# liupei101/VLSA

Measured on AMD Instinct MI355X. Metric: patches/sec per slide (50k x 512 CONCH bag), higher is better.
Workload: dtype bf16

## Files before the change

include/vlsa_hip.h:

```cpp
#ifndef VLSA_HIP_H
#define VLSA_HIP_H

#include <stddef.h>
#include <stdint.h>

#ifdef __cplusplus
extern "C" {
#endif

#define VLSA_ABI_VERSION 1
#define VLSA_MAX_P 16
#define VLSA_MAX_K 64
#define VLSA_MAX_D 1024

#define VLSA_DT_F32 0
#define VLSA_DT_BF16 1

#define VLSA_OK 0
#define VLSA_EINVAL (-1)
#define VLSA_EUNSUPPORTED (-2)
#define VLSA_ELAUNCH (-3)

#define VLSA_KERNEL_AUTO 0
#define VLSA_KERNEL_GENERIC 1
#define VLSA_KERNEL_MFMA 2
#define VLSA_KERNEL_DMA 3

#define VLSA_POOL_MEAN 0
#define VLSA_POOL_MAX 1
#define VLSA_POOL_WEIGHT 2
#define VLSA_POOL_GIVEN 3

int vlsa_abi_version(void);
const char* vlsa_error_string(int code);

int vlsa_num_partials(int64_t N);

size_t vlsa_qprep_bytes(int D);

int vlsa_prepare_queries(const float* Q, int nq, int D, int gated, float coattn_scale, void* qprep, void* stream);
int vlsa_prepare_queries_and_text(const float* Q, int nq, int D, int gated, float coattn_scale, void* qprep,
                                  const float* T, int K, float* That, float* tnorm, void* stream);
const float* vlsa_qprep_qeff(const void* qprep, int D);
const float* vlsa_qprep_qhat(const void* qprep, int D);
const float* vlsa_qprep_qnorm(const void* qprep, int D);

int vlsa_vlfan_partial(const void* X, int x_dtype, int64_t N, int64_t ldx, int D, const void* qprep, int P,
                       int kernel, float* pm, float* pl, float* pacc, float* scores, void* stream);

int vlsa_vlfan_merge(const float* pm, const float* pl, const float* pacc, int G, int P, int D, int normalise,
                     float* m2, float* l, float* out, void* stream);
int vlsa_vlfan_merge_strided(const float* pm, int64_t pm_stride, const float* pl, int64_t pl_stride, const float* pacc,
                             int64_t pacc_stride, int G, int P, int D, int normalise, float* m2, float* l, float* out,
                             void* stream);

size_t vlsa_bwd_prep_bytes(int D);
int vlsa_vlfan_backward(const void* X, int x_dtype, int64_t N, int64_t ldx, int D, const void* qprep, int P,
                        float coattn_scale, const float* dout, const float* out, const float* m2, const float* l,
                        void* bwd_prep, float* pm, float* pl, float* pacc, void* stream);

int vlsa_attn_normalise(const float* scores, int P, int64_t N, const float* m2, const float* l, float* A,
                        void* stream);

int vlsa_normalize_rows(const float* in, int rows, int D, float* out, float* norms, void* stream);

int vlsa_vlfan_merge_head(const float* pm, const float* pl, const float* pacc, int G, int P, int D, int pool_mode,
                          const float* pool_w, const float* W, const float* b, const float* That, int K,
                          const float* logit_scale, void* head_ws, float* m2, float* l, float* out, float* pooled, float* v,
                          float* vhat, float* vnorm, float* logits, float* incidence, void* stream);

size_t vlsa_head_workspace_bytes(int D);

int vlsa_head_forward(const float* rows, int P, int D, int pool_mode, const float* pool_w, const float* W,
                      const float* b, const float* That, int K, const float* logit_scale, void* workspace,
                      float* pooled, float* v, float* vhat, float* vnorm, float* logits, float* incidence,
                      void* stream);

int vlsa_vlfan_forward_bag(const void* X, int x_dtype, int64_t N, int64_t ldx, int D, const float* Q, int nq, int gated,
                           float coattn_scale, const float* T, int K, const float* logit_scale, int pool_mode, const float* pool_w,
                           const float* W, const float* b, int kernel, void* qprep, float* That, float* tnorm, float* pm, float* pl,
                           float* pacc, int G, float* m2, float* l, float* out, float* scores, float* A, void* head_ws,
                           float* pooled, float* v, float* vhat, float* vnorm, float* logits, float* incidence, void* stream);

int vlsa_query_chain(const float* dE, const void* qprep, int nq, int gated, int D, float* dQ, void* stream);

int vlsa_vlfan_backward_bag(const void* X, int x_dtype, int64_t N, int64_t ldx, int D, const void* qprep, int nq, int gated,
                            float coattn_scale, const float* dlogits, const float* g_vhat, const float* g_That,
                            const float* pooled, const float* vhat, const float* vnorm, const float* That, const float* tnorm,
                            const float* logits, const float* W, const float* logit_scale, const float* out, const float* m2,
                            const float* l, int K, float* head_ws, float* drows, float* dW, float* db, float* dT, float* dls,
                            void* bwd_prep, float* pm, float* pl, float* pacc, int G, float* dE, float* dQ, void* stream);


typedef struct vlsa_bag_desc {
    const void* X;
    int64_t N;
    int64_t ldx;
} vlsa_bag_desc;

typedef struct vlsa_rows_desc {
    float* ptr;
    int64_t ld;
} vlsa_rows_desc;

int vlsa_batch_max_bags(void);
int vlsa_batch_forward_max_bags(void);
int vlsa_batch_partials_per_bag(int B);
size_t vlsa_batch_workspace_bytes(int B, int P, int D);

int vlsa_vlfan_partial_batch(const void* bag_desc, int B, int x_dtype, int D, const void* qprep, int P, void* workspace,
                             void* stream);
int vlsa_batch_groups(const int64_t* rows_host, int B, int reserved_cus);
int vlsa_batch_partials_per_bag_ex(int B, int reserved_cus, int groups);
int vlsa_vlfan_partial_batch_ex(const void* bag_desc, int B, int x_dtype, int D, const void* qprep, int P, void* workspace,
                                int reserved_cus, int groups, void* stream);
int vlsa_vlfan_forward_batch(const void* bag_desc, int B, int x_dtype, int D, const void* qprep, int P, int pool_mode,
                             const float* pool_w, const float* W, const float* b, const float* That, int K,
                             const float* logit_scale, void* workspace, float* m2, float* l, float* out, float* pooled,
                             float* v, float* vhat, float* vnorm, float* logits, float* incidence, int reserved_cus,
                             int groups, void* stream);
int vlsa_vlfan_partial_batch_scores(const void* bag_desc, int B, int x_dtype, int D, const void* qprep, int P, void* workspace,
                                    int reserved_cus, int groups, const void* scores_desc, void* stream);
int vlsa_attn_normalise_batch(const void* bag_desc, int B, int P, int64_t max_N, const void* scores_desc, const float* m2,
                              const float* l, const void* attn_desc, void* stream);
int vlsa_vlfan_forward_batch_attn(const void* bag_desc, int B, int x_dtype, int D, const void* qprep, int P, int pool_mode,
                                  const float* pool_w, const float* W, const float* b, const float* That, int K,
                                  const float* logit_scale, void* workspace, float* m2, float* l, float* out, float* pooled,
                                  float* v, float* vhat, float* vnorm, float* logits, float* incidence, int reserved_cus,
                                  int groups, const void* scores_desc, const void* attn_desc, int64_t max_N, void* stream);

int vlsa_bwd_batch_partials(void);
size_t vlsa_bwd_batch_prep_bytes(int B, int D);
int vlsa_vlfan_backward_batch(const void* bag_desc, int B, int x_dtype, int D, const void* qprep, int P,
                              float coattn_scale, const float* dout, const float* out, const float* m2, const float* l,
                              void* bwd_prep, float* pm, float* pl, float* pacc, int groups, void* stream);

int vlsa_vlfan_backward_bags(const void* bag_desc, int B, int x_dtype, int D, const void* qprep, int P, float coattn_scale,
                             const float* dout, const float* out, const float* m2, const float* l, void* bwd_prep, float* pm,
                             float* pl, float* pacc, int G, void* stream);

int vlsa_vlfan_merge_batch_strided(const float* pm, const float* pl, const float* pacc, int B, int G, int P, int D,
                                   int normalise, const int64_t* strides9, float* m2, float* l, float* out, void* stream);

int vlsa_vlfan_merge_head_batch_strided(const float* pm, const float* pl, const float* pacc, int B, int G, int P, int D,
                                        const int64_t* strides9, int pool_mode, const float* pool_w, const float* W,
                                        const float* b, const float* That, int K, const float* logit_scale, float* m2,
                                        float* l, float* out, float* pooled, float* v, float* vhat, float* vnorm,
                                        float* logits, float* incidence, void* stream);

int vlsa_head_forward_batch(const float* rows, int B, int P, int D, int pool_mode, const float* pool_w, const float* W,
                            const float* b, const float* That, int K, const float* logit_scale, void* counters,
                            float* pooled, float* v, float* vhat, float* vnorm, float* logits, float* incidence,
                            void* stream);

int vlsa_head_forward_batch_text(const float* rows, int B, int P, int D, int pool_mode, const float* pool_w, const float* W,
                                 const float* b, const float* T, int K, const float* logit_scale, float* That, float* tnorm,
                                 float* pooled, float* v, float* vhat, float* vnorm, float* logits, float* incidence, void* stream);

int vlsa_head_backward_batch(const float* dlogits, const float* g_vhat, const float* g_That, const float* pooled, const float* vhat,
                             const float* vnorm, const float* That, const float* tnorm, const float* logits, const float* W,
                             const float* logit_scale, int B, int P, int D, int K, float* workspace, float* drows, float* dW,
                             float* db, float* dT, float* dls, void* stream);


int vlsa_pool_num_partials(int64_t N);

int vlsa_scored_pool_partial(const void* X, int x_dtype, int64_t N, int64_t ldx, int D, const float* scores,
                             float* pm, float* pl, float* pacc, void* stream);

int vlsa_colmax(const void* X, int x_dtype, int64_t N, int64_t ldx, int D, float* partials, float* out, void* stream);

int vlsa_colmax_part_rows(void);
int vlsa_colmax_parts(int64_t N);
size_t vlsa_colmax_workspace_bytes(int n_parts);
int vlsa_colmax_batch(const void* bag_desc, int B, int x_dtype, int D, const int* part_start, int n_parts, void* workspace, float* out,
                      int* idx, void* stream);
int vlsa_pool_dx_tile_rows(void);
int vlsa_pool_dx_batch(const void* dx_desc, const void* bag_desc, int B, int mode, const int* idx, const float* dpooled,
                       const int* tile_start, int n_tiles, void* stream);
int vlsa_gather_rows_batch(const void* bag_desc, int B, int x_dtype, const int* idx, float* out, void* stream);

int vlsa_attn_scores(const float* H, const float* Hg, int64_t N, int hid, const float* b1, const float* bg,
                     const float* w2, const float* b2, float* a, void* stream);

int vlsa_gated_scores_tiling(int x_dtype, int gated, int* max_rows, int* round_tiles);
int vlsa_gated_scores_big_tile(int x_dtype, int gated, int* rows, int64_t* min_total_rows);
int64_t vlsa_gated_scores_pool_ws_floats(int64_t N);
int vlsa_gated_scores_pool(const void* X, int x_dtype, int64_t N, int64_t ldx, int D, const void* prep, int gated, float* a, float* ws,
                           float* pooled, void* stream);
int vlsa_gated_scores_pool_adapter(const void* X, int x_dtype, int64_t N, int64_t ldx, int D, const void* prep, int gated, float* a,
                                   float* ws, float* pooled, const float* W1, int R, const float* W2, float keep_ratio, float* logit,
                                   void* stream);
int vlsa_gated_scores_pool_batch(const void* bag_desc, int B, int x_dtype, int D, const void* prep, int gated, const int* tile_start,
                                 int n_tiles, int rows_per_tile, float* a, const int64_t* a_off, float* ws, float* pooled,
                                 void* stream);
int vlsa_gated_scores_batch(const void* bag_desc, int B, int x_dtype, int D, const void* prep, int gated, const int* tile_start,
                            int n_tiles, int rows_per_tile, float* a, const int64_t* a_off, int64_t a_floats, void* stream);
int vlsa_scored_pool_partial_batch(const void* bag_desc, int B, int x_dtype, int D, const float* scores, const int64_t* a_off,
                                   int G, float* pm, float* pl, float* pacc, void* stream);

int vlsa_prompt_sentences(const float* templ, const float* context, int ctx_per_rank, const float* rank, const float* interp,
                          int n_base, const int* order, int R, int L, int S, int C, int T, int dim, float* out, void* stream);
int vlsa_prompt_sentences_backward(const float* dout, const int* pos, int ctx_per_rank, const float* interp, int n_base,
                                   int n_rank_rows, int R, int L, int S, int C, int T, int dim, float* dcontext, float* drank,
                                   void* stream);

int vlsa_prototype_shapley(const float* sim, int P, int K, float logit_scale, float* values, float* shap, void* stream);

size_t vlsa_featproj_prep_bytes(void);
int vlsa_prepare_featproj(const float* W, const float* b, const float* gamma, const float* beta, int dim_in, int dim_out,
                          void* prep, void* stream);
int vlsa_feat_project(const void* X, int x_dtype, int64_t N, int64_t ldx, int D, const void* prep, float eps, float* Y,
                      int64_t ldy, void* stream);

int vlsa_query_pool_attention(const float* rows, int B, int P, int D, const float* Wa, const float* ba, const float* Wg,
                              const float* bg, const float* w2, const float* c, int hid, int want_raw, void* workspace,
                              float* pooled, float* scores, void* stream);

int vlsa_rowdot(const void* X, int x_dtype, int64_t N, int64_t ldx, int D, const float* v, float* out, void* stream);
int vlsa_scored_pool_backward(const void* X, int x_dtype, int64_t N, int64_t ldx, int D, const float* a, const float* m2,
                              const float* l, const float* pooled, const float* dpooled, float* da, void* stream);

int vlsa_topk_mean(const float* S, int C, int64_t N, int k, float out_scale, float* out, void* stream);
int vlsa_topk_chunks(int64_t N);
size_t vlsa_topk_workspace_bytes(int C, int64_t N, int k);
int vlsa_topk_mean_ws(const float* S, int C, int64_t N, int k, float out_scale, void* workspace, float* out, void* stream);

int vlsa_topk_values(const float* S, int C, int64_t N, int k, void* workspace, float* vals, void* stream);

int vlsa_topk_mean_batch(const void* bag_desc, const void* scores_desc, int B, int C, int k, const float* logit_scale, float* out,
                         void* stream);

int vlsa_topk_select_batch(const void* bag_desc, const void* scores_desc, int B, int C, int k, const float* logit_scale, float* out,
                           int* idx, void* stream);

size_t vlsa_unit_mean_workspace_bytes(int B);
int vlsa_unit_mean_batch(const void* bag_desc, int B, int x_dtype, int D, void* workspace, float* u, void* stream);

int vlsa_zeroshot_backward_batch(const void* bag_desc, int B, int x_dtype, int D, int C, int k, const int* idx, const float* u,
                                 const float* G, const float* logits, const float* That, const float* tnorm, const float* logit_scale,
                                 float* dT, float* dls, void* stream);

int vlsa_normalize_many(const void* X, int x_dtype, int64_t N, int64_t ldx, int D, float* out, void* stream);

size_t vlsa_gated_prep_bytes(int gated);
int vlsa_prepare_gated_weights(const float* Wa, const float* ba, const float* Wg, const float* bg, const float* w2,
                               const float* c, int dim_in, int dim_hid, int gated, void* prep, void* stream);
int vlsa_gated_scores(const void* X, int x_dtype, int64_t N, int64_t ldx, int D, const void* prep, int gated, float* a,
                      void* stream);

int vlsa_adapter_head(const float* f, int D, const float* W1, int R, const float* W2, float keep_ratio, float* hidden,
                      float* out, void* stream);

int vlsa_pack_rows_bf16(const void* src, int src_dtype, int64_t N, int64_t lds, int D, void* dst, int64_t ldd,
                        void* stream);

int vlsa_surv_loss(const float* x, const int64_t* t, const float* e, int B, int K, int from_logits,
                   const float* logit_scale_exp, float alpha, float eps, int p, int raw_distance, float w_ifmle,
                   float w_emd, float* out_ifmle, float* out_emd, float* grad, void* stream);
int vlsa_surv_objective(const float* x, const int64_t* t, const float* e, int B, int K, int from_logits, const float* logit_scale,
                        int ls_is_log, float alpha, float eps, int p, int raw_distance, float w_ifmle, float w_emd,
                        float* objective, float* grad, void* stream);

#define VLSA_EVAL_INCIDENCE 0
#define VLSA_EVAL_HAZARD 1
#define VLSA_EVAL_RAW 0
#define VLSA_EVAL_CONVERTED 1
#define VLSA_EVAL_MAX_M 65536
#define VLSA_EVAL_RESULT_WORDS 16
#define VLSA_EVAL_SUM_MLE 0
#define VLSA_EVAL_SUM_MLE_ORG 1
#define VLSA_EVAL_SUM_IFMLE 2
#define VLSA_EVAL_SUM_EMD 3
#define VLSA_EVAL_EVENTS 4
#define VLSA_EVAL_NONFINITE 5
#define VLSA_EVAL_M 6
#define VLSA_EVAL_CONCORDANT 8
#define VLSA_EVAL_DISCORDANT 9
#define VLSA_EVAL_TIED_RISK 10
#define VLSA_EVAL_TIED_TIME 11
#define VLSA_EVAL_COMPARABLE 12
int vlsa_surv_eval_rows(const float* x, int x_kind, int pred_type, const int64_t* t, const float* e, int M, int K, double alpha,
                        double eps, const float* logit_scale, double logit_scale_value, int ls_is_log, int ext_mask, double ext_alpha,
                        double ext_eps, int p, int raw_distance, double w_ifmle, double w_emd, double* est, double* time, float* surv,
                        double* result, void* stream);
int vlsa_concordance_pairs(const double* time, const float* e, const double* est, int M, double tied_tol, uint64_t* counters,
                           int zero_first, void* stream);

// ... 168 lines not shown
```

vlsa_amd/csrc/launch.h:

```cpp
#pragma once
#include "vlsa_common.h"

namespace vlsa {

inline int launch_status() { return hipGetLastError() == hipSuccess ? VLSA_OK : VLSA_ELAUNCH; }

struct LdsGrant {
    int granted[64];
    LdsGrant() { for (int& g : granted) g = -1; }
    bool covers(int bytes) {
        int d = 0;
        if (hipGetDevice(&d) != hipSuccess || d < 0 || d >= 64) return false;
        if (granted[d] >= bytes) return true;
        granted[d] = bytes;
        return false;
    }
};

template <auto Kernel>
inline LdsGrant& lds_grant() {
    static LdsGrant grant;
    return grant;
}
template <auto Kernel, typename... Args>
inline void launch_lds(dim3 grid, dim3 block, size_t lds_bytes, hipStream_t stream, Args... args) {
    if (!lds_grant<Kernel>().covers((int)lds_bytes))
        (void)hipFuncSetAttribute(reinterpret_cast<const void*>(Kernel), hipFuncAttributeMaxDynamicSharedMemorySize, (int)lds_bytes);
    hipLaunchKernelGGL(Kernel, grid, block, lds_bytes, stream, args...);
}

struct DropSpec {
    unsigned int thr = 0u;
    float scale = 1.f;
};
inline bool drop_spec(float p, DropSpec* out) {
    *out = DropSpec{};
    if (p <= 0.f) return true;
    if (!(p < 1.f)) return false;
    out->thr = (unsigned int)((double)p * 4294967296.0);
    if (out->thr == 0u) out->thr = 1u;
    out->scale = 1.f / (1.f - p);
    return true;
}

inline bool bag_table_ok(const void* bag_desc, int B, const void* table, long long n_table) {
    return bag_desc && table && B >= 1 && B <= 64 && n_table >= B;
}

}
```

vlsa_amd/csrc/vlfan_backward_batch.hip:

```cpp
#ifndef VLSA_DMA_NT
#define VLSA_DMA_NT "nt"
#endif
#define VLSA_STREAM_NT VLSA_DMA_NT
#include "vlfan_stream.h"
#include "launch.h"

namespace vlsa {

namespace bb {
constexpr int kTile = 32;
constexpr int kSlot = kTile * 256;
constexpr int kWaveRing = 2 * kSlot;
constexpr int kRingBytes = 4 * kWaveRing;
constexpr int kMaxP = 12;
constexpr int kTileBytes = 2 * 4 * kMaxP * 16;
constexpr int kExchWave = 2 * kTileBytes + 128;
constexpr int kExchGroup = 4 * kExchWave;
constexpr int kTabOff = kRingBytes + kExchGroup;
constexpr int kTabInts = 8;
constexpr int kMaxBags = 64;
constexpr int kLdsBytes = kTabOff + kMaxBags * kTabInts * 4;
}

__global__ __launch_bounds__(256) void k_prepare_backward_batch(const float* __restrict__ dout, const float* __restrict__ out,
                                                                 int P, int D, __bf16* __restrict__ dsplit,
                                                                 float* __restrict__ delta) {
    __shared__ float red[4];
    const int p = blockIdx.x, bag = blockIdx.y, tid = threadIdx.x;
    dout += (size_t)bag * P * D;
    out += (size_t)bag * P * D;
    dsplit += (size_t)bag * 3 * 16 * D;
    float acc = 0.f;
    for (int d = tid; d < D; d += 256) {
        const float x = p < P ? dout[(size_t)p * D + d] : 0.f;
        if (p < P) acc += x * out[(size_t)p * D + d];
        const __bf16 h0 = (__bf16)x;
        const float r1 = x - (float)h0;
        const __bf16 h1 = (__bf16)r1;
        dsplit[((size_t)0 * 16 + p) * D + d] = h0;
        dsplit[((size_t)1 * 16 + p) * D + d] = h1;
        dsplit[((size_t)2 * 16 + p) * D + d] = (__bf16)(r1 - (float)h1);
    }
    acc = block_sum_256(acc, red);
    if (tid == 0) delta[(size_t)bag * kPStride + p] = acc;
}

__global__ __launch_bounds__(256, 2) void k_vlfan_backward_dma_batch(const vlsa_bag_desc* __restrict__ bags, int B,
                                                                     const __bf16* __restrict__ qsplit,
                                                                     const __bf16* __restrict__ dsplit, int P,
                                                                     const float* __restrict__ m2, const float* __restrict__ l,
                                                                     const float* __restrict__ delta, float scale,
                                                                     float* __restrict__ pm, float* __restrict__ pl,
                                                                     float* __restrict__ pacc, int S) {
    using namespace bb;
    constexpr int D = 512;
    extern __shared__ __attribute__((aligned(16))) unsigned char smem[];
    const int tid = threadIdx.x, lane = tid & 63;
    const int w = __builtin_amdgcn_readfirstlane(tid >> 6);
    const int cw = w;
    const int g = lane >> 4, i16 = lane & 15;
    const int Gb = gridDim.x / S;
    const int grp = blockIdx.x / Gb, b = blockIdx.x % Gb, G = Gb;

    unsigned char* ring = smem + w * kWaveRing;
    unsigned char* exch = smem + kRingBytes;
    const StreamTab<kTabInts> tab{reinterpret_cast<int_ma*>(smem + kTabOff)};
    const bool pok = i16 < P;
    const int xslot = i16 < bb::kMaxP ? (i16 + 4 * g) % bb::kMaxP : (4 * g) % bb::kMaxP;

    if (tid < B) {
        const vlsa_bag_desc d = bags[tid];
        const unsigned int vb = (unsigned int)((b + (tid / S) * 37) % G);
        stream_split<5, 2, kTile>(d, G, vb, (tid % S) == grp, tab.entry(tid));
    }
    bf16x8 qf[3][4];
#pragma unroll
    for (int t = 0; t < 3; ++t)
#pragma unroll
        for (int kk = 0; kk < 4; ++kk)
            qf[t][kk] = *reinterpret_cast<const bf16x8*>(qsplit + ((size_t)t * 16 + i16) * D + cw * 128 + kk * 32 + g * 8);
#pragma unroll
    for (int t = 0; t < 3; ++t)
#pragma unroll
        for (int kk = 0; kk < 4; ++kk) asm volatile("" : "+v"(qf[t][kk]));
    asm volatile("s_waitcnt vmcnt(0)" ::: "memory");
    __syncthreads();

    DmaRingBf16 dma(ring, lane, cw);

    int kown = 0;
    {
        const int fb = stream_first_bag(tab, 0, B, 0);
        if (fb < B) {
            dma.bind(tab.entry(fb), fb);
            dma.issue(0, 0);
        }
    }

    
    f32x4 acc[8];
#pragma unroll
    for (int ct = 0; ct < 8; ++ct) acc[ct] = f32x4{0.f, 0.f, 0.f, 0.f};

    for (int bag = 0; bag < B; ++bag) {
        if (tab.get(bag, kEntMine) == 0) continue;
        const int nrows = tab.get(bag, kEntRows), ntiles = tab.get(bag, kEntTiles);
        const int niter = ntiles;
        if (niter == 0) continue;
        bf16x8 df[2][4];
#pragma unroll
        for (int t = 0; t < 2; ++t)
#pragma unroll
            for (int kk = 0; kk < 4; ++kk)
                df[t][kk] = *reinterpret_cast<const bf16x8*>(dsplit + (((size_t)bag * 3 + t) * 16 + i16) * D + cw * 128 + kk * 32 + g * 8);
        float m2p = pok ? m2[(size_t)bag * kPStride + i16] : 0.f;
        float rlp = pok ? 1.f / l[(size_t)bag * kPStride + i16] : 0.f;
        float dlt = pok ? delta[(size_t)bag * kPStride + i16] : 0.f;
#pragma unroll
        for (int t = 0; t < 2; ++t)
#pragma unroll
            for (int kk = 0; kk < 4; ++kk) asm volatile("" : "+v"(df[t][kk]));
        asm volatile("" : "+v"(m2p), "+v"(rlp), "+v"(dlt));

        for (int it = 0; it < niter; ++it) {
            const int tile = it;
            constexpr bool have = true;
            const int slot = kown & 1;
            const unsigned char* xs = ring + slot * kSlot;
            const int row0 = tile * kTile;
            f32x4 S[2], Nd[2], Dd[2];
#pragma unroll
            for (int h = 0; h < 2; ++h) {
                S[h] = f32x4{0.f, 0.f, 0.f, 0.f};
                Nd[h] = f32x4{0.f, 0.f, 0.f, 0.f};
                Dd[h] = f32x4{0.f, 0.f, 0.f, 0.f};
            }
            if (have) {
                int nb, nt;
                stream_next<1>(tab, bag, tile, ntiles, B, 0, nb, nt);
                asm volatile("s_waitcnt lgkmcnt(0)" ::: "memory");
                if (nb < B) {
                    dma.bind(tab.entry(nb), nb);
                    dma.issue(nt, slot ^ 1);
                    asm volatile("s_waitcnt vmcnt(8)" ::: "memory");
                } else {
                    asm volatile("s_waitcnt vmcnt(0)" ::: "memory");
                }
                bf16x8 xa[2][4];
#pragma unroll
                for (int h = 0; h < 2; ++h)
#pragma unroll
                    for (int kk = 0; kk < 4; ++kk)
                        xa[h][kk] = *reinterpret_cast<const bf16x8_ma*>(xs + swz(16 * h + i16, kk * 64 + g * 16));
                __builtin_amdgcn_sched_barrier(0);
                f32x4 Sb[2], Db[2];
                Sb[0] = f32x4{0.f, 0.f, 0.f, 0.f};
                Sb[1] = Sb[0];
                Db[0] = Sb[0];
                Db[1] = Sb[0];
#pragma unroll
                for (int kk = 0; kk < 4; ++kk)
#pragma unroll
                    for (int h = 0; h < 2; ++h) {
                        S[h] = __builtin_amdgcn_mfma_f32_16x16x32_bf16(xa[h][kk], qf[0][kk], S[h], 0, 0, 0);
                        Sb[h] = __builtin_amdgcn_mfma_f32_16x16x32_bf16(xa[h][kk], qf[1][kk], Sb[h], 0, 0, 0);
                        Nd[h] = __builtin_amdgcn_mfma_f32_16x16x32_bf16(xa[h][kk], xa[h][kk], Nd[h], 0, 0, 0);
                        Sb[h] = __builtin_amdgcn_mfma_f32_16x16x32_bf16(xa[h][kk], qf[2][kk], Sb[h], 0, 0, 0);
                        Dd[h] = __builtin_amdgcn_mfma_f32_16x16x32_bf16(xa[h][kk], df[0][kk], Dd[h], 0, 0, 0);
                        Db[h] = __builtin_amdgcn_mfma_f32_16x16x32_bf16(xa[h][kk], df[1][kk], Db[h], 0, 0, 0);
                    }
                S[0] += Sb[0];
                S[1] += Sb[1];
                Dd[0] += Db[0];
                Dd[1] += Db[1];
            }

            VLSA_LDS_BARRIER();
            {
                unsigned char* mine = exch + cw * kExchWave;
                if (i16 < kMaxP) {
                    *reinterpret_cast<f32x4_ma*>(mine + ((0 * 4 + g) * kMaxP + xslot) * 16) = S[0];
                    *reinterpret_cast<f32x4_ma*>(mine + ((1 * 4 + g) * kMaxP + xslot) * 16) = S[1];
                    *reinterpret_cast<f32x4_ma*>(mine + kTileBytes + ((0 * 4 + g) * kMaxP + xslot) * 16) = Dd[0];
                    *reinterpret_cast<f32x4_ma*>(mine + kTileBytes + ((1 * 4 + g) * kMaxP + xslot) * 16) = Dd[1];
                }
                if (g == (i16 >> 2)) {
                    const int r = i16 & 3;
                    const float d0 = r == 0 ? Nd[0][0] : r == 1 ? Nd[0][1] : r == 2 ? Nd[0][2] : Nd[0][3];
                    const float d1 = r == 0 ? Nd[1][0] : r == 1 ? Nd[1][1] : r == 2 ? Nd[1][2] : Nd[1][3];
                    reinterpret_cast<float_ma*>(mine + 2 * kTileBytes)[i16] = d0;
                    reinterpret_cast<float_ma*>(mine + 2 * kTileBytes)[16 + i16] = d1;
                }
            }
            VLSA_LDS_BARRIER();
            if (have) {
                f32x4 T[2], DA[2], R2[2];
                {
                    f32x4 tv[2][4], dv[2][4], rv[2][4];
                    const int pidx = xslot;
#pragma unroll
                    for (int h = 0; h < 2; ++h)
#pragma unroll
                        for (int ww = 0; ww < 4; ++ww) {
                            const unsigned char* o = exch + ww * kExchWave;
                            tv[h][ww] = *reinterpret_cast<const f32x4_ma*>(o + ((h * 4 + g) * kMaxP + pidx) * 16);
                            dv[h][ww] = *reinterpret_cast<const f32x4_ma*>(o + kTileBytes + ((h * 4 + g) * kMaxP + pidx) * 16);
                            rv[h][ww] = *reinterpret_cast<const f32x4_ma*>(o + 2 * kTileBytes + (16 * h + 4 * g) * 4);
                        }
#pragma unroll
                    for (int h = 0; h < 2; ++h) {
                        T[h] = (tv[h][0] + tv[h][1]) + (tv[h][2] + tv[h][3]);
                        DA[h] = (dv[h][0] + dv[h][1]) + (dv[h][2] + dv[h][3]);
                        R2[h] = (rv[h][0] + rv[h][1]) + (rv[h][2] + rv[h][3]);
                    }
                }
                bf16x8 ahi, alo;
#pragma unroll
                for (int h = 0; h < 2; ++h)
#pragma unroll
                    for (int r = 0; r < 4; ++r) {
                        const bool valid = pok && (row0 + 16 * h + 4 * g + r < nrows);
                        const float inv = fminf(__builtin_amdgcn_rsqf(R2[h][r]), 1e12f);
                        const float A = fast_exp2(T[h][r] * inv - m2p) * rlp;
                        const float u = valid ? A * (DA[h][r] - dlt) * (scale * inv) : 0.f;
                        const __bf16 hi = (__bf16)u;
                        ahi[4 * h + r] = hi;
                        alo[4 * h + r] = (__bf16)(u - (float)hi);
                    }
#pragma unroll
                for (int ct = 0; ct < 8; ++ct) {
                    const int c_off = ct * 32 + (i16 & 3) * 8;
                    const int rr = 4 * g + (i16 >> 2);
                    const bf16x4 b0 = __builtin_amdgcn_ds_read_tr16_b64_v4bf16((lds_bf16x4_ptr)(xs + swz(rr, c_off)));
                    const bf16x4 b1 = __builtin_amdgcn_ds_read_tr16_b64_v4bf16((lds_bf16x4_ptr)(xs + swz(16 + rr, c_off)));
                    const bf16x8 bh = __builtin_shufflevector(b0, b1, 0, 1, 2, 3, 4, 5, 6, 7);
                    acc[ct] = __builtin_amdgcn_mfma_f32_16x16x32_bf16(ahi, bh, acc[ct], 0, 0, 0);
                    acc[ct] = __builtin_amdgcn_mfma_f32_16x16x32_bf16(alo, bh, acc[ct], 0, 0, 0);
                }
                ++kown;
            }
        }
    }

    asm volatile("s_waitcnt vmcnt(0)" ::: "memory");
    {
        const size_t slotg = blockIdx.x;
        if (cw == 0 && g == 0 && i16 < P) {
            pm[slotg * kPStride + i16] = 0.f;
            pl[slotg * kPStride + i16] = 1.f;
        }
#pragma unroll
        for (int ct = 0; ct < 8; ++ct)
#pragma unroll
            for (int r = 0; r < 4; ++r) {
                const int p = 4 * g + r;
                if (p < P) pacc[(slotg * P + p) * D + cw * 128 + ct * 16 + i16] = acc[ct][r];
            }
    }
}

}

using namespace vlsa;

static inline int bwd_groups(int B) { return B >= 8 ? 8 : (B >= 4 ? 4 : (B >= 2 ? 2 : 1)); }

int vlsa_launch_backward_f32_batch(const void* bag_desc, int B, const __bf16* qsplit, const __bf16* dsplit, int P,
                                   const float* m2, const float* l, const float* delta, float scale, float* pm, float* pl,
                                   float* pacc, int S, hipStream_t s);

extern "C" int vlsa_bwd_batch_partials(void) { return 512; }

extern "C" size_t vlsa_bwd_batch_prep_bytes(int B, int D) { return (size_t)B * 3 * 16 * D * 2 + (size_t)B * kPStride * 4; }

static int backward_prepare(const void* bag_desc, int B, int x_dtype, int D, const void* qprep, int P, int bf16_max_p, const float* dout,
                            const float* out, const float* m2, const float* l, void* bwd_prep, const float* pm, const float* pl,
                            const float* pacc, hipStream_t s, const __bf16** qsplit, const __bf16** dsplit, const float** delta) {
    if (!bag_desc || !qprep || !dout || !out || !m2 || !l || !bwd_prep || !pm || !pl || !pacc) return VLSA_EINVAL;
    if (B < 1 || B > bb::kMaxBags || P < 1 || P > VLSA_MAX_P) return VLSA_EINVAL;
    if (D != 512 || (x_dtype != VLSA_DT_BF16 && x_dtype != VLSA_DT_F32)) return VLSA_EUNSUPPORTED;
    if (x_dtype == VLSA_DT_BF16 && P > bf16_max_p) return VLSA_EUNSUPPORTED;
    __bf16* ds = static_cast<__bf16*>(bwd_prep);
    float* dl = reinterpret_cast<float*>(static_cast<unsigned char*>(bwd_prep) + (size_t)B * 3 * 16 * D * 2);
    hipLaunchKernelGGL(k_prepare_backward_batch, dim3(16, B), dim3(256), 0, s, dout, out, P, D, ds, dl);
    *qsplit = reinterpret_cast<const __bf16*>(static_cast<const unsigned char*>(qprep) + QPrepLayout(D).qsplit);
    *dsplit = ds;
    *delta = dl;
    return VLSA_OK;
}

extern "C" int vlsa_vlfan_backward_batch(const void* bag_desc, int B, int x_dtype, int D, const void* qprep, int P,
                                         float coattn_scale, const float* dout, const float* out, const float* m2,
                                         const float* l, void* bwd_prep, float* pm, float* pl, float* pacc, int groups,
                                         void* stream) {
    hipStream_t s = (hipStream_t)stream;
    const __bf16 *qsplit, *dsplit;
    const float* delta;
    const int rc = backward_prepare(bag_desc, B, x_dtype, D, qprep, P, bb::kMaxP, dout, out, m2, l, bwd_prep, pm, pl, pacc, s, &qsplit, &dsplit,
                                    &delta);
    if (rc != VLSA_OK) return rc;
    int S = groups > 0 ? groups : bwd_groups(B);
    {
        int p2 = 1;
        while (p2 * 2 <= S && p2 * 2 <= B && p2 * 2 <= 64) p2 *= 2;
        S = p2;
    }
    if (x_dtype == VLSA_DT_F32)
        return vlsa_launch_backward_f32_batch(bag_desc, B, qsplit, dsplit, P, m2, l, delta, coattn_scale, pm, pl, pacc, S, s);
    launch_lds<k_vlfan_backward_dma_batch>(dim3(512), dim3(256), bb::kLdsBytes, s, static_cast<const vlsa_bag_desc*>(bag_desc), B,
                                           qsplit, dsplit, P, m2, l, delta, coattn_scale, pm, pl, pacc, S);
    return launch_status();
}

int vlsa_launch_backward_mfma_bags(const void* bag_desc, int B, int x_dtype, const __bf16* qsplit, const __bf16* dsplit, int P,
                                   const float* m2, const float* l, const float* delta, float scale, float* pm, float* pl,
                                   float* pacc, int G, hipStream_t s);

extern "C" int vlsa_vlfan_backward_bags(const void* bag_desc, int B, int x_dtype, int D, const void* qprep, int P,
                                        float coattn_scale, const float* dout, const float* out, const float* m2, const float* l,
                                        void* bwd_prep, float* pm, float* pl, float* pacc, int G, void* stream) {
    if (G < 1) return VLSA_EINVAL;
    hipStream_t s = (hipStream_t)stream;
    const __bf16 *qsplit, *dsplit;
    const float* delta;
    const int rc = backward_prepare(bag_desc, B, x_dtype, D, qprep, P, VLSA_MAX_P, dout, out, m2, l, bwd_prep, pm, pl, pacc, s, &qsplit, &dsplit,
                                    &delta);
    if (rc != VLSA_OK) return rc;
    return vlsa_launch_backward_mfma_bags(bag_desc, B, x_dtype, qsplit, dsplit, P, m2, l, delta, coattn_scale, pm, pl, pacc, G, s);
}
```

vlsa_amd/csrc/vlfan_backward_batch_f32.hip:

```cpp
#define VLSA_STREAM_NT "nt"
#include "vlfan_stream.h"
#include "launch.h"

namespace vlsa {

namespace bbf {
constexpr int kTile = 16;
constexpr int kSlot = kTile * 512;
constexpr int kWaveRing = 2 * kSlot;
constexpr int kRingBytes = 4 * kWaveRing;
constexpr int kExchWave = 2 * 1024 + 64;
constexpr int kExchBytes = 4 * kExchWave;
constexpr int kTabOff = kRingBytes + kExchBytes;
constexpr int kTabInts = 8;
constexpr int kMaxBags = 64;
constexpr int kLdsBytes = kTabOff + kMaxBags * kTabInts * 4;
}

__global__ __launch_bounds__(256, 2) void k_vlfan_backward_f32_batch(const vlsa_bag_desc* __restrict__ bags, int B,
                                                                     const __bf16* __restrict__ qsplit,
                                                                     const __bf16* __restrict__ dsplit, int P,
                                                                     const float* __restrict__ m2, const float* __restrict__ l,
                                                                     const float* __restrict__ delta, float scale,
                                                                     float* __restrict__ pm, float* __restrict__ pl,
                                                                     float* __restrict__ pacc, int S) {
    using namespace bbf;
    constexpr int D = 512;
    extern __shared__ __attribute__((aligned(16))) unsigned char smem[];
    const int tid = threadIdx.x, lane = tid & 63;
    const int cw = __builtin_amdgcn_readfirstlane(tid >> 6);
    const int g = lane >> 4, i16 = lane & 15;
    const int Gb = gridDim.x / S;
    const int grp = blockIdx.x / Gb, b = blockIdx.x % Gb, G = Gb;

    unsigned char* ring = smem + cw * kWaveRing;
    unsigned char* exch = smem + kRingBytes;
    const StreamTab<kTabInts> tab{reinterpret_cast<int_ma*>(smem + kTabOff)};
    const bool pok = i16 < P;

    if (tid < B) {
        const vlsa_bag_desc d = bags[tid];
        const unsigned int vb = (unsigned int)((b + (tid / S) * 37) % G);
        stream_split<4, 4, kTile>(d, G, vb, (tid % S) == grp, tab.entry(tid));
    }
    bf16x8 qs[3][4];
#pragma unroll
    for (int t = 0; t < 3; ++t)
#pragma unroll
        for (int s4 = 0; s4 < 4; ++s4) {
            const __bf16* src = qsplit + ((size_t)t * 16 + i16) * D + cw * 128 + 32 * s4 + 4 * g;
            const bf16x4 lo4 = *reinterpret_cast<const bf16x4*>(src), hi4 = *reinterpret_cast<const bf16x4*>(src + 16);
            qs[t][s4] = __builtin_shufflevector(lo4, hi4, 0, 1, 2, 3, 4, 5, 6, 7);
        }
#pragma unroll
    for (int t = 0; t < 3; ++t)
#pragma unroll
        for (int s4 = 0; s4 < 4; ++s4) asm volatile("" : "+v"(qs[t][s4]));
    asm volatile("s_waitcnt vmcnt(0)" ::: "memory");
    __syncthreads();

    DmaRingF32 dma(ring, lane, cw);

    int kown = 0;
    {
        const int fb = stream_first_bag(tab, 0, B, 0);
        if (fb < B) {
            dma.bind(tab.entry(fb), fb);
            dma.issue(0, 0);
        }
    }

    f32x4 acc[8];
#pragma unroll
    for (int ct = 0; ct < 8; ++ct) acc[ct] = f32x4{0.f, 0.f, 0.f, 0.f};

    for (int bag = 0; bag < B; ++bag) {
        if (tab.get(bag, kEntMine) == 0) continue;
        const int nrows = tab.get(bag, kEntRows), ntiles = tab.get(bag, kEntTiles);
        if (ntiles == 0) continue;
        bf16x8 df[2][4];
#pragma unroll
        for (int t = 0; t < 2; ++t)
#pragma unroll
            for (int s4 = 0; s4 < 4; ++s4) {
                const __bf16* src = dsplit + (((size_t)bag * 3 + t) * 16 + i16) * D + cw * 128 + 32 * s4 + 4 * g;
                const bf16x4 lo4 = *reinterpret_cast<const bf16x4*>(src), hi4 = *reinterpret_cast<const bf16x4*>(src + 16);
                df[t][s4] = __builtin_shufflevector(lo4, hi4, 0, 1, 2, 3, 4, 5, 6, 7);
            }
        float m2p = pok ? m2[(size_t)bag * kPStride + i16] : 0.f;
        float rlp = pok ? 1.f / l[(size_t)bag * kPStride + i16] : 0.f;
        float dlt = pok ? delta[(size_t)bag * kPStride + i16] : 0.f;
#pragma unroll
        for (int t = 0; t < 2; ++t)
#pragma unroll
            for (int s4 = 0; s4 < 4; ++s4) asm volatile("" : "+v"(df[t][s4]));
        asm volatile("" : "+v"(m2p), "+v"(rlp), "+v"(dlt));

        for (int tile = 0; tile < ntiles; ++tile) {
            const int slot = kown & 1;
            const unsigned char* xs = ring + slot * kSlot;
            const int row0 = tile * kTile;
            f32x4 Sv = {0.f, 0.f, 0.f, 0.f}, Dv = {0.f, 0.f, 0.f, 0.f};
            float ss = 0.f;
            {
                int nb, nt;
                stream_next<1>(tab, bag, tile, ntiles, B, 0, nb, nt);
                asm volatile("s_waitcnt lgkmcnt(0)" ::: "memory");
                if (nb < B) {
                    dma.bind(tab.entry(nb), nb);
                    dma.issue(nt, slot ^ 1);
                    asm volatile("s_waitcnt vmcnt(8)" ::: "memory");
                } else {
                    asm volatile("s_waitcnt vmcnt(0)" ::: "memory");
                }
                float xa[32];
#pragma unroll
                for (int j = 0; j < 8; ++j) {
                    const f32x4 v = *reinterpret_cast<const f32x4_ma*>(xs + fswz(i16, 16 * j + 4 * g));
                    xa[4 * j] = v[0];
                    xa[4 * j + 1] = v[1];
                    xa[4 * j + 2] = v[2];
                    xa[4 * j + 3] = v[3];
                }
                float s0 = 0.f, s1 = 0.f;
#pragma unroll
                for (int kk = 0; kk < 32; kk += 2) {
                    s0 = fmaf(xa[kk], xa[kk], s0);
                    s1 = fmaf(xa[kk + 1], xa[kk + 1], s1);
                }
                ss = quad_rows_sum(s0 + s1);
                f32x4 Db = {0.f, 0.f, 0.f, 0.f}, Sb = {0.f, 0.f, 0.f, 0.f};
#pragma unroll
                for (int s4 = 0; s4 < 4; ++s4) {
                    bf16x8 xh, xl;
#pragma unroll
                    for (int e = 0; e < 8; ++e) {
                        const float v = xa[8 * s4 + e];
                        const __bf16 h = (__bf16)v;
                        xh[e] = h;
                        xl[e] = (__bf16)(v - (float)h);
                    }
                    Sv = __builtin_amdgcn_mfma_f32_16x16x32_bf16(xh, qs[0][s4], Sv, 0, 0, 0);
                    Dv = __builtin_amdgcn_mfma_f32_16x16x32_bf16(xh, df[0][s4], Dv, 0, 0, 0);
                    Sb = __builtin_amdgcn_mfma_f32_16x16x32_bf16(xh, qs[1][s4], Sb, 0, 0, 0);
                    Db = __builtin_amdgcn_mfma_f32_16x16x32_bf16(xh, df[1][s4], Db, 0, 0, 0);
                    Sb = __builtin_amdgcn_mfma_f32_16x16x32_bf16(xl, qs[0][s4], Sb, 0, 0, 0);
                    Db = __builtin_amdgcn_mfma_f32_16x16x32_bf16(xl, df[0][s4], Db, 0, 0, 0);
                    Sb = __builtin_amdgcn_mfma_f32_16x16x32_bf16(xh, qs[2][s4], Sb, 0, 0, 0);
                    Sb = __builtin_amdgcn_mfma_f32_16x16x32_bf16(xl, qs[1][s4], Sb, 0, 0, 0);
                }
                Sv += Sb;
                Dv += Db;
            }

            VLSA_LDS_BARRIER();
            {
                unsigned char* mine = exch + cw * kExchWave;
                *reinterpret_cast<f32x4_ma*>(mine + lane * 16) = Sv;
                *reinterpret_cast<f32x4_ma*>(mine + 1024 + lane * 16) = Dv;
                if (g == 0) reinterpret_cast<float_ma*>(mine + 2048)[i16] = ss;
            }
            VLSA_LDS_BARRIER();
            {
                f32x4 T, DA, R2;
                {
                    f32x4 tv[4], dv[4], rv[4];
#pragma unroll
                    for (int ww = 0; ww < 4; ++ww) {
                        const unsigned char* o = exch + ww * kExchWave;
                        tv[ww] = *reinterpret_cast<const f32x4_ma*>(o + lane * 16);
                        dv[ww] = *reinterpret_cast<const f32x4_ma*>(o + 1024 + lane * 16);
                        rv[ww] = *reinterpret_cast<const f32x4_ma*>(o + 2048 + 16 * g);
                    }
                    T = (tv[0] + tv[1]) + (tv[2] + tv[3]);
                    DA = (dv[0] + dv[1]) + (dv[2] + dv[3]);
                    R2 = (rv[0] + rv[1]) + (rv[2] + rv[3]);
                }
                float uv[4];
#pragma unroll
                for (int r = 0; r < 4; ++r) {
                    const bool valid = pok && (row0 + 4 * g + r < nrows);
                    const float inv = fminf(__builtin_amdgcn_rsqf(R2[r]), 1e12f);
                    const float A = fast_exp2(T[r] * inv - m2p) * rlp;
                    uv[r] = valid ? A * (DA[r] - dlt) * (scale * inv) : 0.f;
                }
                float xb[4][8];
#pragma unroll
                for (int rs = 0; rs < 4; ++rs)
#pragma unroll
                    for (int ct = 0; ct < 8; ++ct) xb[rs][ct] = *reinterpret_cast<const float_ma*>(xs + fswz(4 * g + rs, 16 * ct + i16));
                bf16x4 uhi, ulo;
#pragma unroll
                for (int r = 0; r < 4; ++r) {
                    uhi[r] = (__bf16)uv[r];
                    ulo[r] = (__bf16)(uv[r] - (float)uhi[r]);
                }
#pragma unroll
                for (int ct = 0; ct < 8; ++ct) {
                    bf16x4 xh, xl;
#pragma unroll
                    for (int r = 0; r < 4; ++r) {
                        xh[r] = (__bf16)xb[r][ct];
                        xl[r] = (__bf16)(xb[r][ct] - (float)xh[r]);
                    }
                    acc[ct] = __builtin_amdgcn_mfma_f32_16x16x16bf16_1k(uhi, xh, acc[ct], 0, 0, 0);
                    acc[ct] = __builtin_amdgcn_mfma_f32_16x16x16bf16_1k(ulo, xh, acc[ct], 0, 0, 0);
                    acc[ct] = __builtin_amdgcn_mfma_f32_16x16x16bf16_1k(uhi, xl, acc[ct], 0, 0, 0);
                }
                ++kown;
            }
        }
    }

    asm volatile("s_waitcnt vmcnt(0)" ::: "memory");
    {
        const size_t slotg = blockIdx.x;
        if (cw == 0 && g == 0 && i16 < P) {
            pm[slotg * kPStride + i16] = 0.f;
            pl[slotg * kPStride + i16] = 1.f;
        }
#pragma unroll
        for (int ct = 0; ct < 8; ++ct)
#pragma unroll
            for (int r = 0; r < 4; ++r) {
                const int p = 4 * g + r;
                if (p < P) pacc[(slotg * P + p) * D + cw * 128 + ct * 16 + i16] = acc[ct][r];
            }
    }
}

}

using namespace vlsa;

int vlsa_launch_backward_f32_batch(const void* bag_desc, int B, const __bf16* qsplit, const __bf16* dsplit, int P,
                                   const float* m2, const float* l, const float* delta, float scale, float* pm, float* pl,
                                   float* pacc, int S, hipStream_t s) {
    launch_lds<k_vlfan_backward_f32_batch>(dim3(512), dim3(256), bbf::kLdsBytes, s, static_cast<const vlsa_bag_desc*>(bag_desc), B,
                                           qsplit, dsplit, P, m2, l, delta, scale, pm, pl, pacc, S);
    return launch_status();
}
```

vlsa_amd/csrc/vlfan_batch.hip:

```cpp
#ifndef VLSA_DMA_NT
#define VLSA_DMA_NT "nt"
#endif
#define VLSA_STREAM_NT VLSA_DMA_NT
#include "vlfan_stream.h"
#include "launch.h"

namespace vlsa {

#ifdef VLSA_TIMING
__device__ long long vlsa_dbg_batch[64];
#define BSTAMP(k)                                                                                            \
    do {                                                                                                     \
        const int k_ = (k);                                                                                  \
        if (blockIdx.x == 3 && threadIdx.x == 0 && k_ < 40) vlsa_dbg_batch[k_] = __builtin_readcyclecounter(); \
        if (blockIdx.x == 3 && threadIdx.x == 0 && (k_ == 1 || k_ == 39)) vlsa_dbg_batch[k_ == 1 ? 62 : 63] = __builtin_amdgcn_s_memrealtime(); \
    } while (0)
#define ISTAMP(k, dep)                                                                                                   \
    do {                                                                                                                 \
        if (kown == 12) {                                                                                                 \
            float sink_ = (dep);                                                                                          \
            asm volatile("v_mov_b32 %0, %0" : "+v"(sink_));                                                              \
            if (blockIdx.x == 3 && (threadIdx.x & 255) == 0)                                                             \
                vlsa_dbg_batch[40 + 8 * rg + (k)] = __builtin_readcyclecounter();                                        \
        }                                                                                                                \
    } while (0)
#else
#define BSTAMP(k) do {} while (0)
#define ISTAMP(k, dep) do {} while (0)
#endif

namespace bt {
constexpr int kTile = 32;
constexpr int kSlot = kTile * 256;
constexpr int kWaveRing = 2 * kSlot;
constexpr int kRingBytes = 8 * kWaveRing;
constexpr int kExchWave = 2048 + 128;
constexpr int kExchGroup = 4 * kExchWave;
constexpr int kTabOff = kRingBytes + 2 * kExchGroup;
constexpr int kTabInts = 12;
constexpr int kMaxLocal = 64;
constexpr int kMaxBags = 256;
constexpr int kMlOff = kTabOff + kMaxLocal * kTabInts * 4;
constexpr int kLdsBytes = kMlOff + 8 * 32 * 4;
constexpr float kThr = 16.0f;
}

template <bool kScores>
__global__ __launch_bounds__(512, 2) void k_vlfan_partial_dma_batch(const vlsa_bag_desc* __restrict__ bags, int B,
                                                                     const __bf16* __restrict__ qsplit, int P,
                                                                     float* __restrict__ pm, float* __restrict__ pl,
                                                                     float* __restrict__ pacc, int S,
                                                                     const vlsa_rows_desc* __restrict__ sdesc) {
    using namespace bt;
    constexpr int D = 512;
    extern __shared__ __attribute__((aligned(16))) unsigned char smem[];
    const int tid = threadIdx.x, lane = tid & 63;
    const int w = __builtin_amdgcn_readfirstlane(tid >> 6);
    const int rg = w >> 2, cw = w & 3;
    const int g = lane >> 4, i16 = lane & 15;
#ifdef VLSA_TIMING
    const int xmode = S >> 8;
    S &= 255;
#else
    constexpr int xmode = 0;
#endif
    const int Gb = gridDim.x / S;
    const int grp = blockIdx.x / Gb, b = blockIdx.x % Gb, G = Gb;

    unsigned char* ring = smem + w * kWaveRing;
    unsigned char* exch = smem + kRingBytes + rg * kExchGroup;
    const StreamTab<kTabInts> tab{reinterpret_cast<int_ma*>(smem + kTabOff)};

    const int nloc = grp < B ? (B - grp + S - 1) / S : 0;
    if (tid < nloc) {
        const int bag_id = grp + tid * S;
        const vlsa_bag_desc d = bags[bag_id];
        const unsigned int vb = (unsigned int)((b + tid * 37) % G);
        int_ma* e = tab.entry(tid);
        const long long rbeg = stream_split<6, 2, kTile>(d, G, vb, true, e);
        if constexpr (kScores) {
            const vlsa_rows_desc sd = sdesc[bag_id];
            const unsigned long long sp = sd.ptr ? reinterpret_cast<unsigned long long>(sd.ptr + rbeg) : 0ull;
            e[kEntScoreLo] = (int)(unsigned int)sp;
            e[kEntScoreHi] = (int)(sp >> 32);
            e[kEntScorePitch] = (int)sd.ld;
        }
    }
    bf16x8 qf[3][4];
#pragma unroll
    for (int t = 0; t < 3; ++t)
#pragma unroll
        for (int kk = 0; kk < 4; ++kk)
            qf[t][kk] = *reinterpret_cast<const bf16x8*>(qsplit + ((size_t)t * 16 + i16) * D + cw * 128 + kk * 32 + g * 8);
#pragma unroll
    for (int t = 0; t < 3; ++t)
#pragma unroll
        for (int kk = 0; kk < 4; ++kk) asm volatile("" : "+v"(qf[t][kk]));
    asm volatile("s_waitcnt vmcnt(0)" ::: "memory");
    __syncthreads();

    DmaRingBf16 dma(ring, lane, cw);

    int kown = 0;
    int k0 = 0, k1 = 0;
    {
        const int fb = stream_first_bag(tab, 0, nloc, rg);
        if (fb < nloc) {
            dma.bind(tab.entry(fb), fb);
            dma.issue(rg, 0);
        }
    }

    int stamp = 0;
    BSTAMP(stamp++);
    for (int bag = 0; bag < nloc; ++bag) {
        const int nrows = tab.get(bag, kEntRows), ntiles = tab.get(bag, kEntTiles);
        const int niter = (ntiles + 1) >> 1;
        f32x4 acc[8];
#pragma unroll
        for (int ct = 0; ct < 8; ++ct) acc[ct] = f32x4{0.f, 0.f, 0.f, 0.f};
        float M = -INFINITY, lsum = 0.f;
        float* srow = nullptr;
        bool has_scores = false;
        if constexpr (kScores) {
            const unsigned long long sp = (unsigned long long)(unsigned int)tab.get(bag, kEntScoreLo) |
                                          ((unsigned long long)(unsigned int)tab.get(bag, kEntScoreHi) << 32);
            const int sp_q = 8 * cw + (lane >> 3);
            has_scores = sp != 0 && cw < 2 && 8 * cw < P;
            if (has_scores && sp_q < P) srow = reinterpret_cast<float*>(sp) + (size_t)sp_q * tab.get(bag, kEntScorePitch) + 4 * (lane & 7);
        }

        if (rg == 1 && !(xmode & 2)) VLSA_LDS_BARRIER();
        for (int it = 0; it < niter; ++it) {
            const int tile = 2 * it + rg;
            const bool have = tile < ntiles;
            const int slot = kown & 1;
            const unsigned char* xs = ring + slot * kSlot;
            const int row0 = tile * kTile;
            f32x4 S[2], Nd[2];
#pragma unroll
            for (int h = 0; h < 2; ++h) {
                S[h] = f32x4{0.f, 0.f, 0.f, 0.f};
                Nd[h] = f32x4{0.f, 0.f, 0.f, 0.f};
            }
            if (!(xmode & 2)) VLSA_LDS_BARRIER();
            if (have) {
                int nb, nt;
                stream_next<2>(tab, bag, tile, ntiles, nloc, rg, nb, nt);
                ISTAMP(0, 0.f);
                asm volatile("s_waitcnt lgkmcnt(0)" ::: "memory");
                if (nb < nloc) {
                    dma.bind(tab.entry(nb), nb);
                    dma.issue(nt, slot ^ 1);
                    asm volatile("s_waitcnt vmcnt(8)" ::: "memory");
                } else {
                    asm volatile("s_waitcnt vmcnt(0)" ::: "memory");
                }
                ISTAMP(1, 0.f);
                bf16x8 xa[2][4];
#pragma unroll
                for (int h = 0; h < 2; ++h)
#pragma unroll
                    for (int kk = 0; kk < 4; ++kk)
                        xa[h][kk] = *reinterpret_cast<const bf16x8_ma*>(xs + swz(16 * h + i16, kk * 64 + g * 16));
                __builtin_amdgcn_sched_barrier(0);
                f32x4 Sb[2];
                Sb[0] = f32x4{0.f, 0.f, 0.f, 0.f};
                Sb[1] = Sb[0];
                if (!(xmode & 1))
#pragma unroll
                for (int kk = 0; kk < 4; ++kk)
#pragma unroll
                    for (int h = 0; h < 2; ++h) {
                        S[h] = __builtin_amdgcn_mfma_f32_16x16x32_bf16(xa[h][kk], qf[0][kk], S[h], 0, 0, 0);
                        Sb[h] = __builtin_amdgcn_mfma_f32_16x16x32_bf16(xa[h][kk], qf[1][kk], Sb[h], 0, 0, 0);
                        Nd[h] = __builtin_amdgcn_mfma_f32_16x16x32_bf16(xa[h][kk], xa[h][kk], Nd[h], 0, 0, 0);
                        Sb[h] = __builtin_amdgcn_mfma_f32_16x16x32_bf16(xa[h][kk], qf[2][kk], Sb[h], 0, 0, 0);
                    }
                S[0] += Sb[0];
                S[1] += Sb[1];
                ISTAMP(2, S[0][0] + S[1][0] + Nd[0][0] + Nd[1][0]);
            }

            {
                unsigned char* mine = exch + cw * kExchWave;
                *reinterpret_cast<f32x4_ma*>(mine + (0 * 64 + lane) * 16) = S[0];
                *reinterpret_cast<f32x4_ma*>(mine + (1 * 64 + lane) * 16) = S[1];
                if (g == (i16 >> 2)) {
                    const int r = i16 & 3;
                    const float d0 = r == 0 ? Nd[0][0] : r == 1 ? Nd[0][1] : r == 2 ? Nd[0][2] : Nd[0][3];
                    const float d1 = r == 0 ? Nd[1][0] : r == 1 ? Nd[1][1] : r == 2 ? Nd[1][2] : Nd[1][3];
                    reinterpret_cast<float_ma*>(mine + 2048)[i16] = d0;
                    reinterpret_cast<float_ma*>(mine + 2048)[16 + i16] = d1;
                }
            }
            if (have) ISTAMP(3, 0.f);
            if (!(xmode & 2)) VLSA_LDS_BARRIER();
            if (have) {
                ISTAMP(4, 0.f);
                f32x4 T[2], R2[2];
                {
                    f32x4 tv[2][4], rv[2][4];
#pragma unroll
                    for (int h = 0; h < 2; ++h)
#pragma unroll
                        for (int ww = 0; ww < 4; ++ww) {
                            const unsigned char* o = exch + ww * kExchWave;
                            tv[h][ww] = *reinterpret_cast<const f32x4_ma*>(o + (h * 64 + lane) * 16);
                            rv[h][ww] = *reinterpret_cast<const f32x4_ma*>(o + 2048 + (16 * h + 4 * g) * 4);
                        }
#pragma unroll
                    for (int h = 0; h < 2; ++h) {
                        T[h] = (tv[h][0] + tv[h][1]) + (tv[h][2] + tv[h][3]);
                        R2[h] = (rv[h][0] + rv[h][1]) + (rv[h][2] + rv[h][3]);
                    }
                }
#pragma unroll
                for (int h = 0; h < 2; ++h)
#pragma unroll
                    for (int r = 0; r < 4; ++r) T[h][r] *= fminf(__builtin_amdgcn_rsqf(R2[h][r]), 1e12f);
                if (row0 + kTile > nrows) {
#pragma unroll
                    for (int h = 0; h < 2; ++h)
#pragma unroll
                        for (int r = 0; r < 4; ++r)
                            if (row0 + 16 * h + 4 * g + r >= nrows) T[h][r] = -INFINITY;
                }
                if constexpr (kScores) {
                    if (has_scores) {
                        const int c = lane & 7;
                        const int src = (16 * (c & 3) + ((8 * cw + (lane >> 3)) & 15)) << 2;
                        f32x4 v;
#pragma unroll
                        for (int r = 0; r < 4; ++r) {
                            const float t0 = T[0][r], t1 = T[1][r];
                            const float a0 = __int_as_float(__builtin_amdgcn_ds_bpermute(src, __float_as_int(t0)));
                            const float a1 = __int_as_float(__builtin_amdgcn_ds_bpermute(src, __float_as_int(t1)));
                            v[r] = (c & 4) ? a1 : a0;
                        }
                        if (srow != nullptr) *reinterpret_cast<f32x4*>(srow + row0) = v;
                    }
                }
                ISTAMP(5, T[0][0] + T[1][0]);
                const float tmax = fmaxf(fmaxf(fmaxf(T[0][0], T[0][1]), fmaxf(T[0][2], T[0][3])),
                                         fmaxf(fmaxf(T[1][0], T[1][1]), fmaxf(T[1][2], T[1][3])));
                if (__builtin_amdgcn_ballot_w64(tmax > M + kThr) != 0) {
                    const float newM = fmaxf(M, quad_rows_max(tmax));
                    const float f = (M == -INFINITY) ? 0.f : fast_exp2(M - newM);
                    lsum *= f;
#pragma unroll
                    for (int r = 0; r < 4; ++r) {
                        const float fr = __shfl(f, 4 * g + r);
#pragma unroll
                        for (int ct = 0; ct < 8; ++ct) acc[ct][r] *= fr;
                    }
                    M = newM;
                }
                bf16x8 ahi, alo;
#pragma unroll
                for (int h = 0; h < 2; ++h)
#pragma unroll
                    for (int r = 0; r < 4; ++r) {
                        const float wv = (xmode & 4) ? T[h][r] : fast_exp2(T[h][r] - M);
                        lsum += wv;
                        const __bf16 hi = (__bf16)wv;
                        ahi[4 * h + r] = hi;
                        alo[4 * h + r] = (__bf16)(wv - (float)hi);
                    }
                ISTAMP(6, lsum);
                if (!(xmode & 8))
#pragma unroll
                for (int ct = 0; ct < 8; ++ct) {
                    const int c_off = ct * 32 + (i16 & 3) * 8;
                    const int rr = 4 * g + (i16 >> 2);
                    const bf16x4 b0 = __builtin_amdgcn_ds_read_tr16_b64_v4bf16((lds_bf16x4_ptr)(xs + swz(rr, c_off)));
                    const bf16x4 b1 = __builtin_amdgcn_ds_read_tr16_b64_v4bf16((lds_bf16x4_ptr)(xs + swz(16 + rr, c_off)));
                    const bf16x8 bh = __builtin_shufflevector(b0, b1, 0, 1, 2, 3, 4, 5, 6, 7);
                    acc[ct] = __builtin_amdgcn_mfma_f32_16x16x32_bf16(ahi, bh, acc[ct], 0, 0, 0);
                    acc[ct] = __builtin_amdgcn_mfma_f32_16x16x32_bf16(alo, bh, acc[ct], 0, 0, 0);
                }
                ISTAMP(7, acc[0][0] + acc[7][0]);
                ++kown;
            }
            BSTAMP(stamp++);
        }
        if (rg == 0 && !(xmode & 2)) VLSA_LDS_BARRIER();
        k0 += (ntiles + 1) >> 1;
        k1 += ntiles >> 1;

        lsum = quad_rows_sum(lsum);
        const int kmine = rg == 0 ? k0 : k1, kother = rg == 0 ? k1 : k0;
        unsigned char* myslot = ring + (((kmine - 1) & 1) * kSlot);
        const unsigned char* otherslot = smem + ((rg ^ 1) * 4 + cw) * kWaveRing + (((kother - 1) & 1) * kSlot);
        float_ma* mlw = reinterpret_cast<float_ma*>(smem + kMlOff);
#pragma unroll
        for (int j = 0; j < 4; ++j) *reinterpret_cast<f32x4_ma*>(myslot + (j * 64 + lane) * 16) = rg == 0 ? acc[4 + j] : acc[j];
        if (g == 0) {
            mlw[w * 32 + i16] = M;
            mlw[w * 32 + 16 + i16] = lsum;
        }
        VLSA_LDS_BARRIER();
        {
            const int wo = (rg ^ 1) * 4 + cw;
            const f32x4 Mm4 = *reinterpret_cast<const f32x4_ma*>(&mlw[w * 32 + 4 * g]);
            const f32x4 Mo4 = *reinterpret_cast<const f32x4_ma*>(&mlw[wo * 32 + 4 * g]);
            const float Mo = mlw[wo * 32 + i16], lo = mlw[wo * 32 + 16 + i16];
            f32x4 oth[4];
#pragma unroll
            for (int j = 0; j < 4; ++j) oth[j] = *reinterpret_cast<const f32x4_ma*>(otherslot + (j * 64 + lane) * 16);
            float am[4], ao[4];
#pragma unroll
            for (int r = 0; r < 4; ++r) {
                const float mn = fmaxf(Mm4[r], Mo4[r]);
                am[r] = (Mm4[r] == -INFINITY) ? 0.f : fast_exp2(Mm4[r] - mn);
                ao[r] = (Mo4[r] == -INFINITY) ? 0.f : fast_exp2(Mo4[r] - mn);
            }
            const size_t slotg = (size_t)(grp + bag * S) * G + tab.get(bag, kEntSlot);
            if (w == 0 && g == 0 && i16 < P) {
                const float Mn = fmaxf(M, Mo);
                const float fm = (M == -INFINITY) ? 0.f : fast_exp2(M - Mn);
                const float fo = (Mo == -INFINITY) ? 0.f : fast_exp2(Mo - Mn);
                pm[slotg * kPStride + i16] = Mn;
                pl[slotg * kPStride + i16] = lsum * fm + lo * fo;
            }
            float_ma* tp = reinterpret_cast<float_ma*>(myslot + 4096);
#pragma unroll
            for (int j = 0; j < 4; ++j) {
                const f32x4 mine = rg == 0 ? acc[j] : acc[4 + j];
#pragma unroll
                for (int r = 0; r < 4; ++r) tp[(4 * g + r) * 64 + j * 16 + i16] = mine[r] * am[r] + oth[j][r] * ao[r];
            }
            asm volatile("s_waitcnt lgkmcnt(0)" ::: "memory");
            float* dstp = pacc + slotg * P * D + cw * 128 + rg * 64 + (lane & 15) * 4;
#pragma unroll
            for (int k = 0; k < 4; ++k) {
                const int p = 4 * k + (lane >> 4);
                const f32x4 v = *reinterpret_cast<const f32x4_ma*>(reinterpret_cast<unsigned char*>(tp) + (p * 64 + (lane & 15) * 4) * 4);
                if (p < P) *reinterpret_cast<f32x4*>(dstp + (size_t)p * D) = v;
            }
        }
        VLSA_LDS_BARRIER();
        BSTAMP(stamp++);
    }
}

struct MergeStrides {
    int64_t sm, sl, sa;
    int64_t bm, bl, ba;
    int64_t om, ol, oo;
};

__global__ __launch_bounds__(256, 5) void k_vlfan_merge_batch(const float* __restrict__ pm, const float* __restrict__ pl,
                                                            const float* __restrict__ pacc, int G, int P, int D,
                                                            int normalise, float* __restrict__ m2, float* __restrict__ l,
                                                            float* __restrict__ out, MergeStrides st) {
    __shared__ float red[4];
    __shared__ __attribute__((aligned(16))) float4 sacc[128];
    __shared__ float sl;
    __builtin_amdgcn_s_setprio(VLSA_TAIL_PRIO);
    const int tid = threadIdx.x, lane = tid & 63, wv = tid >> 6;
    const int p = blockIdx.y, c0 = blockIdx.x * 512, bag = blockIdx.z;
    pm += (size_t)bag * st.bm;
    pl += (size_t)bag * st.bl;
    pacc += (size_t)bag * st.ba;
    const int c4 = tid & 127, gs = __builtin_amdgcn_readfirstlane(tid >> 7);
    const int col = c0 + c4 * 4;
    const bool incol = col < D;
    constexpr int U = 16;
    float mx = -INFINITY;
    for (int gI = tid; gI < G; gI += 256) mx = fmaxf(mx, pm[(size_t)gI * st.sm + p]);
    mx = wave_max(mx);
    if (lane == 0) red[wv] = mx;
    __syncthreads();
    mx = fmaxf(fmaxf(red[0], red[1]), fmaxf(red[2], red[3]));
    float4 a = make_float4(0.f, 0.f, 0.f, 0.f);
    float lt = 0.f;
    for (int g0 = gs; g0 < G; g0 += 2 * U) {
        float mg[U], lg[U];
        float4 v[U];
#pragma unroll
        for (int u = 0; u < U; ++u) {
            const int gI = g0 + 2 * u;
            const bool ok = gI < G;
            mg[u] = ok ? pm[(size_t)gI * st.sm + p] : -INFINITY;
            lg[u] = ok ? pl[(size_t)gI * st.sl + p] : 0.f;
            v[u] = (ok && incol) ? *reinterpret_cast<const float4*>(pacc + (size_t)gI * st.sa + (size_t)p * D + col)
                                 : make_float4(0.f, 0.f, 0.f, 0.f);
        }
#pragma unroll
        for (int u = 0; u < U; ++u) {
            const float f = (mg[u] == -INFINITY) ? 0.f : fast_exp2(mg[u] - mx);
            lt += lg[u] * f;
            a.x += v[u].x * f; a.y += v[u].y * f; a.z += v[u].z * f; a.w += v[u].w * f;
        }
    }
    if (gs == 1) {
        sacc[c4] = a;
        if (c4 == 0) sl = lt;
    }
    __syncthreads();
    if (gs == 0) {
        const float4 o = sacc[c4];
        a.x += o.x; a.y += o.y; a.z += o.z; a.w += o.w;
        const float ls = lt + sl;
        if (normalise) {
            const float inv = 1.f / ls;
            a.x *= inv; a.y *= inv; a.z *= inv; a.w *= inv;
        }
        if (incol) *reinterpret_cast<float4*>(out + (size_t)bag * st.oo + (size_t)p * D + col) = a;
        if (c4 == 0 && blockIdx.x == 0) {
            m2[(size_t)bag * st.om + p] = mx;
            l[(size_t)bag * st.ol + p] = ls;
        }
    }
}

__global__ __launch_bounds__(512, 4) void k_vlfan_merge_pool_batch(const float* __restrict__ pm, const float* __restrict__ pl,
                                                                    const float* __restrict__ pacc, int G, int P, int D,
                                                                    float* __restrict__ m2, float* __restrict__ l,
                                                                    float* __restrict__ out, MergeStrides st, int pool_mode,
                                                                    const float* __restrict__ pool_w,
                                                                    float* __restrict__ pooled) {
    __shared__ __attribute__((aligned(16))) float4 sacc[VLSA_MAX_P][16];
    __shared__ float slt[VLSA_MAX_P][16];
    __shared__ float spw[VLSA_MAX_P];
    __builtin_amdgcn_s_setprio(VLSA_TAIL_PRIO);
    const int tid = threadIdx.x;
    const int gs = tid >> 8, p = (tid >> 4) & 15, c4 = tid & 15, bag = blockIdx.y;
    const int col = blockIdx.x * 64 + c4 * 4;
    const bool live = p < P && col < D;
    pm += (size_t)bag * st.bm + p;
    pl += (size_t)bag * st.bl + p;
    pacc += (size_t)bag * st.ba + (size_t)p * D + col;
    if (pool_mode == VLSA_POOL_WEIGHT && tid == 0) {
        float mx = -INFINITY, sum = 0.f;
        for (int q = 0; q < P; ++q) mx = fmaxf(mx, pool_w[q]);
        for (int q = 0; q < P; ++q) { spw[q] = expf(pool_w[q] - mx); sum += spw[q]; }
        for (int q = 0; q < P; ++q) spw[q] /= sum;
    }
    constexpr int U = 8;
    float mx = -INFINITY;
    if (p < P)
        for (int g = 0; g < G; ++g) mx = fmaxf(mx, pm[(size_t)g * st.sm]);
    float4 a = make_float4(0.f, 0.f, 0.f, 0.f);
    float lt = 0.f;
    for (int g0 = gs; g0 < G; g0 += 2 * U) {
        float mg[U], lg[U];
        float4 v[U];
#pragma unroll
        for (int u = 0; u < U; ++u) {
            const int g = g0 + 2 * u;
            const bool ok = live && g < G;
            mg[u] = ok ? pm[(size_t)g * st.sm] : -INFINITY;
            lg[u] = ok ? pl[(size_t)g * st.sl] : 0.f;
            v[u] = ok ? *reinterpret_cast<const float4*>(pacc + (size_t)g * st.sa) : make_float4(0.f, 0.f, 0.f, 0.f);
        }
#pragma unroll
        for (int u = 0; u < U; ++u) {
            const float f = (mg[u] == -INFINITY) ? 0.f : fast_exp2(mg[u] - mx);
            lt += lg[u] * f;
            a.x += v[u].x * f; a.y += v[u].y * f; a.z += v[u].z * f; a.w += v[u].w * f;
        }
    }
    if (gs == 1) {
        sacc[p][c4] = a;
        slt[p][c4] = lt;
    }
    __syncthreads();
    if (gs == 0) {
        const float4 o = sacc[p][c4];
// ... 56 lines not shown
    if (tid < 8 * VLSA_MAX_P) {
        const int g = tid >> 4, p = tid & 15;
        const bool ok = g < G && p < P;
        sm_[g][p] = ok ? pm[(size_t)g * st.sm + p] : -INFINITY;
        sl_[g][p] = ok ? pl[(size_t)g * st.sl + p] : 0.f;
    }
    if (pool_mode == VLSA_POOL_WEIGHT && tid == 255) {
        float mx = -INFINITY, sum = 0.f;
        for (int q = 0; q < P; ++q) mx = fmaxf(mx, pool_w[q]);
        for (int q = 0; q < P; ++q) { spw[q] = expf(pool_w[q] - mx); sum += spw[q]; }
        for (int q = 0; q < P; ++q) spw[q] /= sum;
    }
    __syncthreads();
    if (tid < VLSA_MAX_P) {
        const int p = tid;
        float mx = -INFINITY;
#pragma unroll
        for (int g = 0; g < 8; ++g) mx = fmaxf(mx, sm_[g][p]);
        float ls = 0.f;
#pragma unroll
        for (int g = 0; g < 8; ++g) {
            const float f = sm_[g][p] == -INFINITY ? 0.f : fast_exp2(sm_[g][p] - mx);
            ls += sl_[g][p] * f;
            sm_[g][p] = f;
        }
        sinv[p] = 1.f / ls;
        if (p < P) {
            m2[(size_t)bag * st.om + p] = mx;
            l[(size_t)bag * st.ol + p] = ls;
        }
    }
    __syncthreads();
    for (int c = tid; c < D; c += 256) {
        float acc[VLSA_MAX_P];
#pragma unroll
        for (int p = 0; p < VLSA_MAX_P; ++p) acc[p] = 0.f;
        for (int g = 0; g < G; ++g) {
            float x[VLSA_MAX_P];
#pragma unroll
            for (int p = 0; p < VLSA_MAX_P; ++p) x[p] = p < P ? pacc[(size_t)g * st.sa + (size_t)p * D + c] : 0.f;
#pragma unroll
            for (int p = 0; p < VLSA_MAX_P; ++p) acc[p] += x[p] * sm_[g][p];
        }
        float r = pool_mode == VLSA_POOL_MAX ? -INFINITY : 0.f;
#pragma unroll
        for (int p = 0; p < VLSA_MAX_P; ++p)
            if (p < P) {
                const float o = acc[p] * sinv[p];
                out[(size_t)bag * st.oo + (size_t)p * D + c] = o;
                if (pool_mode == VLSA_POOL_MAX) r = fmaxf(r, o);
                else if (pool_mode == VLSA_POOL_WEIGHT) r += spw[p] * o;
                else r += o;
            }
        if (pool_mode == VLSA_POOL_MEAN) r /= (float)P;
        if (pooled != nullptr) pooled[(size_t)bag * D + c] = r;
    }
}

__global__ __launch_bounds__(256) void k_attn_normalise_batch(const vlsa_bag_desc* __restrict__ bags, const vlsa_rows_desc* __restrict__ sdesc,
                                                             const vlsa_rows_desc* __restrict__ adesc, const float* __restrict__ m2,
                                                             const float* __restrict__ l, int m_stride) {
    const int bag = blockIdx.z, p = blockIdx.y;
    const int64_t n = ((int64_t)blockIdx.x * 256 + threadIdx.x) * 4;
    const int64_t N = bags[bag].N;
    const vlsa_rows_desc sd = sdesc[bag], ad = adesc[bag];
    if (n >= N || sd.ptr == nullptr || ad.ptr == nullptr) return;
    const float m = m2[(size_t)bag * m_stride + p], inv = 1.f / l[(size_t)bag * m_stride + p];
    const f32x4 t = *reinterpret_cast<const f32x4*>(sd.ptr + (size_t)p * sd.ld + n);
    f32x4 a;
#pragma unroll
    for (int r = 0; r < 4; ++r) a[r] = fast_exp2(t[r] - m) * inv;
    *reinterpret_cast<f32x4*>(ad.ptr + (size_t)p * ad.ld + n) = a;
}

}

using namespace vlsa;

int vlsa_launch_head_batch(const float* rows, int B, int P, int D, int pool_mode, const float* pool_w, const float* W,
                           const float* b, const float* That, int K, const float* logit_scale, unsigned int* counters,
                           float* pooled, float* v, float* vhat, float* vnorm, float* logits, float* incidence,
                           hipStream_t s);
int vlsa_launch_head_pooled_batch(const float* pooled, int B, int D, const float* W, const float* b, const float* That, int K,
                                  const float* logit_scale, float* v, float* vhat, float* vnorm, float* logits,
                                  float* incidence, hipStream_t s);
int vlsa_launch_head_rows_batch(const float* rows, int B, int P, int D, int pool_mode, const float* pool_w, const float* W,
                                const float* b, const float* That, int K, const float* logit_scale, float* pooled, float* v,
                                float* vhat, float* vnorm, float* logits, float* incidence, hipStream_t s);

static int launch_merge_pool(const float* pm, const float* pl, const float* pacc, int B, int G, int P, int D, float* m2, float* l,
                             float* out, const MergeStrides& st, int pool_mode, const float* pool_w, float* pooled, hipStream_t s) {
    if (G <= 8)
        hipLaunchKernelGGL(k_vlfan_merge_pool_small, dim3(B), dim3(256), 0, s, pm, pl, pacc, G, P, D, m2, l, out, st, pool_mode, pool_w,
                           pooled);
    else
        hipLaunchKernelGGL(k_vlfan_merge_pool_batch, dim3((D + 63) / 64, B), dim3(512), 0, s, pm, pl, pacc, G, P, D, m2, l, out, st,
                           pool_mode, pool_w, pooled);
    return launch_status();
}

#ifdef VLSA_TIMING
extern "C" int vlsa_debug_read_batch_cycles(long long* host_out) {
    return hipMemcpyFromSymbol(host_out, HIP_SYMBOL(vlsa::vlsa_dbg_batch), sizeof(long long) * 64) == hipSuccess ? 0 : -3;
}
#endif

static inline int batch_groups(int B) { return B >= 8 ? 8 : (B >= 4 ? 4 : (B >= 2 ? 2 : 1)); }
static inline int min_groups(int B) {
    int m = 1;
    while (m * bt::kMaxLocal < B) m *= 2;
    return m;
}
static inline int resolve_groups(int B, int groups) {
    int S = groups > 0 ? groups : batch_groups(B);
    int p2 = 1;
    while (p2 * 2 <= S && p2 * 2 <= B && p2 * 2 <= 256) p2 *= 2;
    const int m = min_groups(B);
    return p2 < m ? m : p2;
}
static inline int batch_workgroups(int S, int reserved_cus) {
    int r = reserved_cus < 0 ? 0 : reserved_cus;
    r = (r + S - 1) / S * S;
    if (r > 256 - S) r = 256 - S;
    return 256 - r;
}
extern "C" int vlsa_batch_partials_per_bag(int B) { return 256 / batch_groups(B); }
extern "C" int vlsa_batch_partials_per_bag_ex(int B, int reserved_cus, int groups) {
    const int S = resolve_groups(B, groups);
    return batch_workgroups(S, reserved_cus) / S;
}
extern "C" int vlsa_batch_groups(const int64_t* rows_host, int B, int reserved_cus) {
    if (!rows_host || B < 1) return 1;
    int best = 1;
    double best_cost = 1e300;
    for (int S = min_groups(B); S <= 256 && S <= B; S *= 2) {
        const int Gb = batch_workgroups(S, reserved_cus) / S;
        double worst = 0.0;
        for (int g = 0; g < S; ++g) {
            double c = 0.0;
            for (int t = g; t < B; t += S) {
                const int64_t units = (rows_host[t] + 63) / 64;
                c += (double)((units + Gb - 1) / Gb) + 0.7;
            }
            if (c > worst) worst = c;
        }
        if (worst < best_cost * 0.999) {
            best_cost = worst;
            best = S;
        }
    }
    return best;
}

extern "C" int vlsa_batch_max_bags(void) { return 64; }
extern "C" int vlsa_batch_forward_max_bags(void) { return bt::kMaxBags; }

extern "C" size_t vlsa_batch_workspace_bytes(int B, int P, int D) {
    const size_t recs = (size_t)(B < bt::kMaxLocal ? B : bt::kMaxLocal) * 256;
    return (recs * kPStride * 2 + recs * P * D) * sizeof(float) + (size_t)B * 64;
}

int vlsa_launch_partial_f32_batch(const void* bag_desc, int B, const float* qeff, const float* qmeta, int P, float* pm,
                                  float* pl, float* pacc, int S, int workgroups, const void* scores_desc, hipStream_t s);

extern "C" int vlsa_vlfan_partial_batch_scores(const void* bag_desc, int B, int x_dtype, int D, const void* qprep, int P,
                                               void* workspace, int reserved_cus, int groups, const void* scores_desc,
                                               void* stream) {
    if (!bag_desc || !qprep || !workspace) return VLSA_EINVAL;
    if (B < 1 || B > bt::kMaxBags || P < 1 || P > VLSA_MAX_P) return VLSA_EINVAL;
    if (x_dtype != VLSA_DT_BF16 && x_dtype != VLSA_DT_F32) return VLSA_EINVAL;
    if (D != 512) return VLSA_EUNSUPPORTED;
    const int S = resolve_groups(B, groups);
    const int WG = batch_workgroups(S, reserved_cus);
    const int G = WG / S;
    float* pm = static_cast<float*>(workspace);
    float* pl = pm + (size_t)B * G * kPStride;
    float* pacc = pl + (size_t)B * G * kPStride;
    const QPrepLayout L(D);
    if (x_dtype == VLSA_DT_F32) {
        const unsigned char* qp = static_cast<const unsigned char*>(qprep);
        return vlsa_launch_partial_f32_batch(bag_desc, B, reinterpret_cast<const float*>(qp + L.qeff),
                                             reinterpret_cast<const float*>(qp + L.qnorm), P, pm, pl, pacc, S, WG, scores_desc,
                                             (hipStream_t)stream);
    }
    const __bf16* qsplit = reinterpret_cast<const __bf16*>(static_cast<const unsigned char*>(qprep) + L.qsplit);
#ifdef VLSA_TIMING
    static const int xm = VLSA_ENV("VLSA_EXP") ? atoi(VLSA_ENV("VLSA_EXP")) : 0;
#else
    constexpr int xm = 0;
#endif
    if (!scores_desc)
        launch_lds<k_vlfan_partial_dma_batch<false>>(dim3(WG), dim3(512), bt::kLdsBytes, (hipStream_t)stream,
                                                     static_cast<const vlsa_bag_desc*>(bag_desc), B, qsplit, P, pm, pl, pacc, S | (xm << 8),
                                                     static_cast<const vlsa_rows_desc*>(nullptr));
    else
        launch_lds<k_vlfan_partial_dma_batch<true>>(dim3(WG), dim3(512), bt::kLdsBytes, (hipStream_t)stream,
                                                    static_cast<const vlsa_bag_desc*>(bag_desc), B, qsplit, P, pm, pl, pacc, S,
                                                    static_cast<const vlsa_rows_desc*>(scores_desc));
    return launch_status();
}

extern "C" int vlsa_vlfan_partial_batch_ex(const void* bag_desc, int B, int x_dtype, int D, const void* qprep, int P,
                                           void* workspace, int reserved_cus, int groups, void* stream) {
    return vlsa_vlfan_partial_batch_scores(bag_desc, B, x_dtype, D, qprep, P, workspace, reserved_cus, groups, nullptr, stream);
}

extern "C" int vlsa_attn_normalise_batch(const void* bag_desc, int B, int P, int64_t max_N, const void* scores_desc,
                                         const float* m2, const float* l, const void* attn_desc, void* stream) {
    if (!bag_desc || !scores_desc || !attn_desc || !m2 || !l) return VLSA_EINVAL;
    if (B < 1 || B > bt::kMaxBags || P < 1 || P > VLSA_MAX_P || max_N < 0) return VLSA_EINVAL;
    if (max_N == 0) return VLSA_OK;
    const unsigned int chunks = (unsigned int)((max_N + 1023) / 1024);
    hipLaunchKernelGGL(k_attn_normalise_batch, dim3(chunks, P, B), dim3(256), 0, (hipStream_t)stream,
                       static_cast<const vlsa_bag_desc*>(bag_desc), static_cast<const vlsa_rows_desc*>(scores_desc),
                       static_cast<const vlsa_rows_desc*>(attn_desc), m2, l, (int)kPStride);
    return launch_status();
}

extern "C" int vlsa_vlfan_partial_batch(const void* bag_desc, int B, int x_dtype, int D, const void* qprep, int P,
                                        void* workspace, void* stream) {
    return vlsa_vlfan_partial_batch_ex(bag_desc, B, x_dtype, D, qprep, P, workspace, 0, 0, stream);
}

extern "C" int vlsa_vlfan_forward_batch_attn(const void* bag_desc, int B, int x_dtype, int D, const void* qprep, int P,
                                             int pool_mode, const float* pool_w, const float* W, const float* b,
                                             const float* That, int K, const float* logit_scale, void* workspace, float* m2,
                                             float* l, float* out, float* pooled, float* v, float* vhat, float* vnorm,
                                             float* logits, float* incidence, int reserved_cus, int groups,
                                             const void* scores_desc, const void* attn_desc, int64_t max_N, void* stream) {
    if (!That || !logit_scale || !m2 || !l || !out || !pooled || !v || !vhat || !vnorm || !logits) return VLSA_EINVAL;
    if (K < 1 || K > VLSA_MAX_K) return VLSA_EINVAL;
    if ((scores_desc == nullptr) != (attn_desc == nullptr)) return VLSA_EINVAL;
    if (pool_mode < VLSA_POOL_MEAN || pool_mode > VLSA_POOL_WEIGHT) return VLSA_EINVAL;
    if (pool_mode == VLSA_POOL_WEIGHT && !pool_w) return VLSA_EINVAL;
    const int rc = vlsa_vlfan_partial_batch_scores(bag_desc, B, x_dtype, D, qprep, P, workspace, reserved_cus, groups, scores_desc,
                                                   stream);
    if (rc != VLSA_OK) return rc;
    hipStream_t s = (hipStream_t)stream;
    const int G = vlsa_batch_partials_per_bag_ex(B, reserved_cus, groups);
    float* pm = static_cast<float*>(workspace);
    float* pl = pm + (size_t)B * G * kPStride;
    float* pacc = pl + (size_t)B * G * kPStride;
    unsigned int* counters = reinterpret_cast<unsigned int*>(static_cast<unsigned char*>(workspace) +
                                                             vlsa_batch_workspace_bytes(B, P, D) - (size_t)B * 64);
    const MergeStrides st{kPStride, kPStride, (int64_t)P * D, (int64_t)G * kPStride, (int64_t)G * kPStride,
                          (int64_t)G * P * D, kPStride, kPStride, (int64_t)P * D};
    if (launch_merge_pool(pm, pl, pacc, B, G, P, D, m2, l, out, st, pool_mode, pool_w, pooled, s) != VLSA_OK) return VLSA_ELAUNCH;
    (void)counters;
    const int rh = vlsa_launch_head_pooled_batch(pooled, B, D, W, b, That, K, logit_scale, v, vhat, vnorm, logits, incidence, s);
    if (rh != VLSA_OK || !scores_desc) return rh;
    return vlsa_attn_normalise_batch(bag_desc, B, P, max_N, scores_desc, m2, l, attn_desc, stream);
}

extern "C" int vlsa_vlfan_forward_batch(const void* bag_desc, int B, int x_dtype, int D, const void* qprep, int P,
                                        int pool_mode, const float* pool_w, const float* W, const float* b,
                                        const float* That, int K, const float* logit_scale, void* workspace, float* m2,
                                        float* l, float* out, float* pooled, float* v, float* vhat, float* vnorm,
                                        float* logits, float* incidence, int reserved_cus, int groups, void* stream) {
    return vlsa_vlfan_forward_batch_attn(bag_desc, B, x_dtype, D, qprep, P, pool_mode, pool_w, W, b, That, K, logit_scale,
                                         workspace, m2, l, out, pooled, v, vhat, vnorm, logits, incidence, reserved_cus, groups,
                                         nullptr, nullptr, 0, stream);
}

extern "C" int vlsa_vlfan_merge_batch_strided(const float* pm, const float* pl, const float* pacc, int B, int G, int P, int D,
                                              int normalise, const int64_t* strides9, float* m2, float* l, float* out,
                                              void* stream) {
    if (!pm || !pl || !pacc || !strides9 || !m2 || !l || !out) return VLSA_EINVAL;
    if (B < 1 || G < 1 || P < 1 || P > VLSA_MAX_P || D < 4 || (D % 4) != 0 || D > VLSA_MAX_D) return VLSA_EINVAL;
    MergeStrides st{strides9[0], strides9[1], strides9[2], strides9[3], strides9[4], strides9[5], strides9[6], strides9[7], strides9[8]};
    if ((st.sa % 4) || (st.ba % 4) || (st.oo % 4) || (reinterpret_cast<uintptr_t>(pacc) & 15) || (reinterpret_cast<uintptr_t>(out) & 15))
        return VLSA_EINVAL;
    hipLaunchKernelGGL(k_vlfan_merge_batch, dim3((D + 511) / 512, P, B), dim3(256), 0, (hipStream_t)stream, pm, pl, pacc, G, P, D,
                       normalise, m2, l, out, st);
    return launch_status();
}

extern "C" int vlsa_vlfan_merge_head_batch_strided(const float* pm, const float* pl, const float* pacc, int B, int G, int P, int D,
                                                   const int64_t* strides9, int pool_mode, const float* pool_w, const float* W,
                                                   const float* b, const float* That, int K, const float* logit_scale, float* m2,
                                                   float* l, float* out, float* pooled, float* v, float* vhat, float* vnorm,
                                                   float* logits, float* incidence, void* stream) {
    if (!pm || !pl || !pacc || !strides9 || !m2 || !l || !out || !pooled || !v || !vhat || !vnorm || !logits || !That || !logit_scale)
        return VLSA_EINVAL;
    if (B < 1 || G < 1 || P < 1 || P > VLSA_MAX_P || D < 4 || (D % 4) != 0 || D > VLSA_MAX_D || K < 1 || K > VLSA_MAX_K) return VLSA_EINVAL;
    if (pool_mode < VLSA_POOL_MEAN || pool_mode > VLSA_POOL_WEIGHT || (pool_mode == VLSA_POOL_WEIGHT && !pool_w)) return VLSA_EINVAL;
    MergeStrides st{strides9[0], strides9[1], strides9[2], strides9[3], strides9[4], strides9[5], strides9[6], strides9[7], strides9[8]};
    if ((st.sa % 4) || (st.ba % 4) || (st.oo % 4) || (reinterpret_cast<uintptr_t>(pacc) & 15) || (reinterpret_cast<uintptr_t>(out) & 15))
        return VLSA_EINVAL;
    hipStream_t s = (hipStream_t)stream;
    if (launch_merge_pool(pm, pl, pacc, B, G, P, D, m2, l, out, st, pool_mode, pool_w, pooled, s) != VLSA_OK) return VLSA_ELAUNCH;
    return vlsa_launch_head_pooled_batch(pooled, B, D, W, b, That, K, logit_scale, v, vhat, vnorm, logits, incidence, s);
}

extern "C" int vlsa_head_forward_batch(const float* rows, int B, int P, int D, int pool_mode, const float* pool_w, const float* W,
                                       const float* b, const float* That, int K, const float* logit_scale, void* counters,
                                       float* pooled, float* v, float* vhat, float* vnorm, float* logits, float* incidence,
                                       void* stream) {
    if (!rows || !That || !logit_scale || !counters || !pooled || !v || !vhat || !vnorm || !logits) return VLSA_EINVAL;
    if (B < 1 || P < 1 || P > VLSA_MAX_P || K < 1 || K > VLSA_MAX_K || D <= 0 || D > VLSA_MAX_D || (D % 4) != 0) return VLSA_EINVAL;
    if (B > 1 && pool_mode >= VLSA_POOL_MEAN && pool_mode <= VLSA_POOL_WEIGHT && pooled != rows)
        return vlsa_launch_head_rows_batch(rows, B, P, D, pool_mode, pool_w, W, b, That, K, logit_scale, pooled, v, vhat, vnorm, logits,
                                           incidence, (hipStream_t)stream);
    return vlsa_launch_head_batch(rows, B, P, D, pool_mode, pool_w, W, b, That, K, logit_scale, static_cast<unsigned int*>(counters),
                                  pooled, v, vhat, vnorm, logits, incidence, (hipStream_t)stream);
}
```

vlsa_amd/csrc/vlfan_batch_f32.hip:

```cpp
#define VLSA_STREAM_NT "nt"
#include "vlfan_stream.h"
#include "launch.h"
#ifndef VLSA_F32_ABL
#define VLSA_F32_ABL 0
#endif

namespace vlsa {

namespace bf {
constexpr int kTile = 16;
constexpr int kSlot = kTile * 512;
constexpr int kWaveRing = 2 * kSlot;
constexpr int kRingBytes = 8 * kWaveRing;
constexpr int kExchWave = 1024 + 64;
constexpr int kExchGroup = 4 * kExchWave;
constexpr int kTabOff = kRingBytes + 2 * kExchGroup;
constexpr int kTabInts = 12;
constexpr int kMaxLocal = 64;
constexpr int kMlOff = kTabOff + kMaxLocal * kTabInts * 4;
constexpr int kLdsBytes = kMlOff + 8 * 32 * 4;
constexpr float kThr = 16.0f;
}

template <bool kScores>
__global__ __launch_bounds__(512, 2) void k_vlfan_partial_f32_batch(const vlsa_bag_desc* __restrict__ bags, int B,
                                                                     const float* __restrict__ qeff, const float* __restrict__ qmeta, int P,
                                                                     float* __restrict__ pm, float* __restrict__ pl,
                                                                     float* __restrict__ pacc, int S,
                                                                     const vlsa_rows_desc* __restrict__ sdesc, const vlsa_bag_desc one) {
    using namespace bf;
    constexpr int D = 512;
    extern __shared__ __attribute__((aligned(16))) unsigned char smem[];
    const int tid = threadIdx.x, lane = tid & 63;
    const int w = __builtin_amdgcn_readfirstlane(tid >> 6);
    const int rg = w >> 2, cw = w & 3;
    const int g = lane >> 4, i16 = lane & 15;
    const int Gb = gridDim.x / S;
    const int grp = blockIdx.x / Gb, b = blockIdx.x % Gb, G = Gb;

    unsigned char* ring = smem + w * kWaveRing;
    unsigned char* exch = smem + kRingBytes + rg * kExchGroup;
    const StreamTab<kTabInts> tab{reinterpret_cast<int_ma*>(smem + kTabOff)};

    const int nloc = grp < B ? (B - grp + S - 1) / S : 0;
    if (tid < nloc) {
        const int bag_id = grp + tid * S;
        const vlsa_bag_desc d = bags ? bags[bag_id] : one;
        const unsigned int vb = (unsigned int)((b + tid * 37) % G);
        int_ma* e = tab.entry(tid);
        const long long rbeg = stream_split<5, 4, kTile>(d, G, vb, true, e);
        if constexpr (kScores) {
            const vlsa_rows_desc sd = sdesc[bag_id];
            const unsigned long long sp = sd.ptr ? reinterpret_cast<unsigned long long>(sd.ptr + rbeg) : 0ull;
            e[kEntScoreLo] = (int)(unsigned int)sp;
            e[kEntScoreHi] = (int)(sp >> 32);
            e[kEntScorePitch] = (int)sd.ld;
        }
    }
    float qf[32];
    {
        const float sc = qmeta[31];
#pragma unroll
        for (int kk = 0; kk < 32; ++kk)
            qf[kk] = qeff[(size_t)i16 * D + cw * 128 + 16 * (kk >> 2) + 4 * g + (kk & 3)] * sc;
#pragma unroll
        for (int kk = 0; kk < 32; ++kk) asm volatile("" : "+v"(qf[kk]));
    }
    asm volatile("s_waitcnt vmcnt(0)" ::: "memory");
    __syncthreads();

    DmaRingF32 dma(ring, lane, cw);

    int kown = 0;
    int k0 = 0, k1 = 0;
    {
        const int fb = stream_first_bag(tab, 0, nloc, rg);
        if (fb < nloc) {
            dma.bind(tab.entry(fb), fb);
            dma.issue(rg, 0);
        }
    }

    
    for (int bag = 0; bag < nloc; ++bag) {
        const int nrows = tab.get(bag, kEntRows), ntiles = tab.get(bag, kEntTiles);
        const int niter = (ntiles + 1) >> 1;
        f32x4 acc[8];
#pragma unroll
        for (int ct = 0; ct < 8; ++ct) acc[ct] = f32x4{0.f, 0.f, 0.f, 0.f};
        float M = -INFINITY, lsum = 0.f;
        float* srow = nullptr;
        if constexpr (kScores) {
            const unsigned long long sp = (unsigned long long)(unsigned int)tab.get(bag, kEntScoreLo) |
                                          ((unsigned long long)(unsigned int)tab.get(bag, kEntScoreHi) << 32);
            if (sp != 0 && cw == 0 && i16 < P) srow = reinterpret_cast<float*>(sp) + (size_t)i16 * tab.get(bag, kEntScorePitch) + 4 * g;
        }

        for (int it = 0; it < niter; ++it) {
            const int tile = 2 * it + rg;
            const bool have = tile < ntiles;
            const int slot = kown & 1;
            const unsigned char* xs = ring + slot * kSlot;
            const int row0 = tile * kTile;
            f32x4 S = {0.f, 0.f, 0.f, 0.f};
            float ss = 0.f;
            if (have) {
                int nb, nt;
                stream_next<2>(tab, bag, tile, ntiles, nloc, rg, nb, nt);
                asm volatile("s_waitcnt lgkmcnt(0)" ::: "memory");
                if (nb < nloc) {
                    dma.bind(tab.entry(nb), nb);
                    dma.issue(nt, slot ^ 1);
                    asm volatile("s_waitcnt vmcnt(8)" ::: "memory");
                } else {
                    asm volatile("s_waitcnt vmcnt(0)" ::: "memory");
                }
                float xa[32];
#pragma unroll
                for (int j = 0; j < 8; ++j) {
                    const f32x4 v = *reinterpret_cast<const f32x4_ma*>(xs + fswz(i16, 16 * j + 4 * g));
                    xa[4 * j] = v[0];
                    xa[4 * j + 1] = v[1];
                    xa[4 * j + 2] = v[2];
                    xa[4 * j + 3] = v[3];
                }
                f32x4 Sb = {0.f, 0.f, 0.f, 0.f};
#if (VLSA_F32_ABL & 4)
                S[0] = xa[0] + xa[31];
#elif (VLSA_F32_ABL & 32)
                f32x4 Sc = {0.f, 0.f, 0.f, 0.f}, Sd = {0.f, 0.f, 0.f, 0.f};
#pragma unroll
                for (int kk = 0; kk < 32; kk += 4) {
                    S = __builtin_amdgcn_mfma_f32_16x16x4f32(xa[kk], qf[kk], S, 0, 0, 0);
                    Sb = __builtin_amdgcn_mfma_f32_16x16x4f32(xa[kk + 1], qf[kk + 1], Sb, 0, 0, 0);
                    Sc = __builtin_amdgcn_mfma_f32_16x16x4f32(xa[kk + 2], qf[kk + 2], Sc, 0, 0, 0);
                    Sd = __builtin_amdgcn_mfma_f32_16x16x4f32(xa[kk + 3], qf[kk + 3], Sd, 0, 0, 0);
                }
                S = (S + Sb) + (Sc + Sd);
#else
#pragma unroll
                for (int kk = 0; kk < 32; kk += 2) {
                    S = __builtin_amdgcn_mfma_f32_16x16x4f32(xa[kk], qf[kk], S, 0, 0, 0);
                    Sb = __builtin_amdgcn_mfma_f32_16x16x4f32(xa[kk + 1], qf[kk + 1], Sb, 0, 0, 0);
                }
                S += Sb;
#endif
                float s0 = 0.f, s1 = 0.f;
#pragma unroll
                for (int kk = 0; kk < 32; kk += 2) {
                    s0 = fmaf(xa[kk], xa[kk], s0);
                    s1 = fmaf(xa[kk + 1], xa[kk + 1], s1);
                }
                ss = quad_rows_sum(s0 + s1);
            }

            VLSA_LDS_BARRIER();
            {
                unsigned char* mine = exch + cw * kExchWave;
                *reinterpret_cast<f32x4_ma*>(mine + lane * 16) = S;
                if (g == 0) reinterpret_cast<float_ma*>(mine + 1024)[i16] = ss;
            }
            VLSA_LDS_BARRIER();
            if (have) {
                f32x4 T, R2;
                {
                    f32x4 tv[4], rv[4];
#pragma unroll
                    for (int ww = 0; ww < 4; ++ww) {
                        const unsigned char* o = exch + ww * kExchWave;
                        tv[ww] = *reinterpret_cast<const f32x4_ma*>(o + lane * 16);
                        rv[ww] = *reinterpret_cast<const f32x4_ma*>(o + 1024 + 16 * g);
                    }
                    T = (tv[0] + tv[1]) + (tv[2] + tv[3]);
                    R2 = (rv[0] + rv[1]) + (rv[2] + rv[3]);
                }
#pragma unroll
                for (int r = 0; r < 4; ++r) T[r] *= fminf(__builtin_amdgcn_rsqf(R2[r]), 1e12f);
                if (row0 + kTile > nrows) {
#pragma unroll
                    for (int r = 0; r < 4; ++r)
                        if (row0 + 4 * g + r >= nrows) T[r] = -INFINITY;
                }
                if constexpr (kScores) {
                    if (srow != nullptr) *reinterpret_cast<f32x4*>(srow + row0) = T;
                }
                const float tmax = fmaxf(fmaxf(T[0], T[1]), fmaxf(T[2], T[3]));
                if (__builtin_amdgcn_ballot_w64(tmax > M + kThr) != 0) {
                    const float newM = fmaxf(M, quad_rows_max(tmax));
                    const float f = (M == -INFINITY) ? 0.f : fast_exp2(M - newM);
                    lsum *= f;
#pragma unroll
                    for (int r = 0; r < 4; ++r) {
                        const float fr = __shfl(f, 4 * g + r);
#pragma unroll
                        for (int ct = 0; ct < 8; ++ct) acc[ct][r] *= fr;
                    }
                    M = newM;
                }
                float wv[4];
#pragma unroll
                for (int r = 0; r < 4; ++r) {
                    wv[r] = fast_exp2(T[r] - M);
                    lsum += wv[r];
                }
                float xb[4][8];
#pragma unroll
                for (int rs = 0; rs < 4; ++rs)
#pragma unroll
                    for (int ct = 0; ct < 8; ++ct) xb[rs][ct] = *reinterpret_cast<const float_ma*>(xs + fswz(4 * g + rs, 16 * ct + i16));
                bf16x4 whi, wlo;
#pragma unroll
                for (int r = 0; r < 4; ++r) {
                    whi[r] = (__bf16)wv[r];
                    wlo[r] = (__bf16)(wv[r] - (float)whi[r]);
                }
#if (VLSA_F32_ABL & 2)
#pragma unroll
                for (int ct = 0; ct < 8; ++ct) acc[ct][0] += xb[0][ct] + xb[1][ct] + xb[2][ct] + xb[3][ct];
#elif (VLSA_F32_ABL & 16)
                bf16x4 xh[8], xl[8];
#pragma unroll
                for (int ct = 0; ct < 8; ++ct)
#pragma unroll
                    for (int r = 0; r < 4; ++r) {
                        xh[ct][r] = (__bf16)xb[r][ct];
                        xl[ct][r] = (__bf16)(xb[r][ct] - (float)xh[ct][r]);
                    }
#pragma unroll
                for (int ct = 0; ct < 8; ++ct) acc[ct] = __builtin_amdgcn_mfma_f32_16x16x16bf16_1k(whi, xh[ct], acc[ct], 0, 0, 0);
#pragma unroll
                for (int ct = 0; ct < 8; ++ct) acc[ct] = __builtin_amdgcn_mfma_f32_16x16x16bf16_1k(wlo, xh[ct], acc[ct], 0, 0, 0);
#pragma unroll
                for (int ct = 0; ct < 8; ++ct) acc[ct] = __builtin_amdgcn_mfma_f32_16x16x16bf16_1k(whi, xl[ct], acc[ct], 0, 0, 0);
#else
#pragma unroll
                for (int ct = 0; ct < 8; ++ct) {
                    bf16x4 xh, xl;
#pragma unroll
                    for (int r = 0; r < 4; ++r) {
                        xh[r] = (__bf16)xb[r][ct];
                        xl[r] = (__bf16)(xb[r][ct] - (float)xh[r]);
                    }
#if (VLSA_F32_ABL & 1)
                    acc[ct][0] += (float)xh[0] + (float)xl[1] + (float)xh[2] + (float)xl[3] + (float)xl[0] + (float)xh[1] + (float)xl[2] + (float)xh[3];
#else
                    acc[ct] = __builtin_amdgcn_mfma_f32_16x16x16bf16_1k(whi, xh, acc[ct], 0, 0, 0);
                    acc[ct] = __builtin_amdgcn_mfma_f32_16x16x16bf16_1k(wlo, xh, acc[ct], 0, 0, 0);
                    acc[ct] = __builtin_amdgcn_mfma_f32_16x16x16bf16_1k(whi, xl, acc[ct], 0, 0, 0);
#endif
                }
#endif
                ++kown;
            }
            
        }
        k0 += (ntiles + 1) >> 1;
        k1 += ntiles >> 1;

        lsum = quad_rows_sum(lsum);
        const int kmine = rg == 0 ? k0 : k1, kother = rg == 0 ? k1 : k0;
        unsigned char* myslot = ring + (((kmine - 1) & 1) * kSlot);
        const unsigned char* otherslot = smem + ((rg ^ 1) * 4 + cw) * kWaveRing + (((kother - 1) & 1) * kSlot);
        float_ma* mlw = reinterpret_cast<float_ma*>(smem + kMlOff);
#pragma unroll
        for (int j = 0; j < 4; ++j) *reinterpret_cast<f32x4_ma*>(myslot + (j * 64 + lane) * 16) = rg == 0 ? acc[4 + j] : acc[j];
        if (g == 0) {
            mlw[w * 32 + i16] = M;
            mlw[w * 32 + 16 + i16] = lsum;
        }
        VLSA_LDS_BARRIER();
        {
            const int wo = (rg ^ 1) * 4 + cw;
            const f32x4 Mm4 = *reinterpret_cast<const f32x4_ma*>(&mlw[w * 32 + 4 * g]);
            const f32x4 Mo4 = *reinterpret_cast<const f32x4_ma*>(&mlw[wo * 32 + 4 * g]);
            const float Mo = mlw[wo * 32 + i16], lo = mlw[wo * 32 + 16 + i16];
            f32x4 oth[4];
#pragma unroll
            for (int j = 0; j < 4; ++j) oth[j] = *reinterpret_cast<const f32x4_ma*>(otherslot + (j * 64 + lane) * 16);
            float am[4], ao[4];
#pragma unroll
            for (int r = 0; r < 4; ++r) {
                const float mn = fmaxf(Mm4[r], Mo4[r]);
                am[r] = (Mm4[r] == -INFINITY) ? 0.f : fast_exp2(Mm4[r] - mn);
                ao[r] = (Mo4[r] == -INFINITY) ? 0.f : fast_exp2(Mo4[r] - mn);
            }
            const size_t slotg = (size_t)(grp + bag * S) * G + tab.get(bag, kEntSlot);
            if (w == 0 && g == 0 && i16 < P) {
                const float Mn = fmaxf(M, Mo);
                const float fm = (M == -INFINITY) ? 0.f : fast_exp2(M - Mn);
                const float fo = (Mo == -INFINITY) ? 0.f : fast_exp2(Mo - Mn);
                pm[slotg * kPStride + i16] = Mn;
                pl[slotg * kPStride + i16] = lsum * fm + lo * fo;
            }
            float_ma* tp = reinterpret_cast<float_ma*>(myslot + 4096);
#pragma unroll
            for (int j = 0; j < 4; ++j) {
                const f32x4 mine = rg == 0 ? acc[j] : acc[4 + j];
#pragma unroll
                for (int r = 0; r < 4; ++r) tp[(4 * g + r) * 64 + j * 16 + i16] = mine[r] * am[r] + oth[j][r] * ao[r];
            }
            asm volatile("s_waitcnt lgkmcnt(0)" ::: "memory");
            float* dstp = pacc + slotg * P * D + cw * 128 + rg * 64 + (lane & 15) * 4;
#pragma unroll
            for (int k = 0; k < 4; ++k) {
                const int p = 4 * k + (lane >> 4);
                const f32x4 v = *reinterpret_cast<const f32x4_ma*>(reinterpret_cast<unsigned char*>(tp) + (p * 64 + (lane & 15) * 4) * 4);
                if (p < P) *reinterpret_cast<f32x4*>(dstp + (size_t)p * D) = v;
            }
        }
        VLSA_LDS_BARRIER();
        
    }
}
#ifdef VLSA_TIMING
extern "C" __global__ void k_dummy_batch_dbg() {}
#endif

}

using namespace vlsa;

int vlsa_launch_partial_f32_batch(const void* bag_desc, int B, const float* qeff, const float* qmeta, int P, float* pm,
                                  float* pl, float* pacc, int S, int workgroups, const void* scores_desc, hipStream_t s) {
    if (!scores_desc)
        launch_lds<k_vlfan_partial_f32_batch<false>>(dim3(workgroups), dim3(512), bf::kLdsBytes, s,
                                                     static_cast<const vlsa_bag_desc*>(bag_desc), B, qeff, qmeta, P, pm, pl, pacc, S,
                                                     static_cast<const vlsa_rows_desc*>(nullptr), vlsa_bag_desc{nullptr, 0, 0});
    else
        launch_lds<k_vlfan_partial_f32_batch<true>>(dim3(workgroups), dim3(512), bf::kLdsBytes, s,
                                                    static_cast<const vlsa_bag_desc*>(bag_desc), B, qeff, qmeta, P, pm, pl, pacc, S,
                                                    static_cast<const vlsa_rows_desc*>(scores_desc), vlsa_bag_desc{nullptr, 0, 0});
    return launch_status();
}

int vlsa_launch_partial_f32_one(const float* X, int64_t N, int64_t ldx, const float* qeff, const float* qmeta, int P, float* pm,
                                float* pl, float* pacc, int G, hipStream_t s) {
    launch_lds<k_vlfan_partial_f32_batch<false>>(dim3(G), dim3(512), bf::kLdsBytes, s, static_cast<const vlsa_bag_desc*>(nullptr), 1,
                                                 qeff, qmeta, P, pm, pl, pacc, 1, static_cast<const vlsa_rows_desc*>(nullptr), vlsa_bag_desc{X, N, ldx});
    return launch_status();
}
```

vlsa_amd/csrc/vlfan_stream.h:

```cpp
#pragma once
#include "vlsa_common.h"

#ifndef VLSA_STREAM_NT
#error "define VLSA_STREAM_NT (\"nt\" or \"\") before including vlfan_stream.h"
#endif

#define VLSA_LDS_BARRIER()                                   \
    do {                                                     \
        asm volatile("s_waitcnt lgkmcnt(0)" ::: "memory");   \
        __builtin_amdgcn_s_barrier();                        \
        asm volatile("" ::: "memory");                       \
    } while (0)

namespace vlsa {

constexpr int kStreamD = 512;

__device__ __forceinline__ int fswz(int row, int col) { return row * 512 + ((((col >> 2) ^ (row & 15))) << 4) + ((col & 3) << 2); }

enum StreamEntry : int {
    kEntAddrLo = 0,
    kEntAddrHi,
    kEntSpan,
    kEntPitch,
    kEntRows,
    kEntTiles,
    kEntSlot,
    kEntMine,
    kEntScoreLo,
    kEntScoreHi,
    kEntScorePitch,
};

template <int kInts>
struct StreamTab {
    int_ma* t;
    __device__ __forceinline__ int_ma* entry(int bag) const { return t + bag * kInts; }
    __device__ __forceinline__ int get(int bag, int k) const { return __builtin_amdgcn_readfirstlane(t[bag * kInts + k]); }
};

template <int kUnitShift, int kElemBytes, int kTile>
__device__ __forceinline__ long long stream_split(const vlsa_bag_desc& d, int G, unsigned int vb, bool mine, int_ma* e) {
    const unsigned long long units = (unsigned long long)((d.N + ((1 << kUnitShift) - 1)) >> kUnitShift);
    const unsigned int uq = (unsigned int)(units / (unsigned int)G), ur = (unsigned int)(units % (unsigned int)G);
    const unsigned long long ubeg = (unsigned long long)vb * uq + (vb < ur ? vb : ur);
    const long long rbeg = (long long)(ubeg << kUnitShift);
    long long rend = (long long)((ubeg + uq + (vb < ur ? 1u : 0u)) << kUnitShift);
    if (rend > d.N) rend = d.N;
    const int nrows = (mine && rend > rbeg) ? (int)(rend - rbeg) : 0;
    const unsigned long long addr = reinterpret_cast<unsigned long long>(d.X) + (unsigned long long)rbeg * d.ldx * (unsigned long long)kElemBytes;
    e[kEntAddrLo] = (int)(unsigned int)addr;
    e[kEntAddrHi] = (int)((addr >> 32) & 0xffffu);
    e[kEntSpan] = nrows > 0 ? (int)(((long long)(nrows - 1) * d.ldx + kStreamD) * kElemBytes) : 0;
    e[kEntPitch] = (int)(d.ldx * kElemBytes);
    e[kEntRows] = nrows;
    e[kEntTiles] = (nrows + kTile - 1) / kTile;
    e[kEntSlot] = (int)vb;
    e[kEntMine] = mine ? 1 : 0;
    return rbeg;
}

template <int kInts>
__device__ __forceinline__ int stream_first_bag(const StreamTab<kInts>& tab, int bag, int nbags, int start) {
    while (bag < nbags && tab.get(bag, kEntTiles) <= start) ++bag;
    return bag;
}
template <int kStride, int kInts>
__device__ __forceinline__ void stream_next(const StreamTab<kInts>& tab, int bag, int tile, int ntiles_bag, int nbags, int start,
                                            int& nb, int& nt) {
    if (tile + kStride < ntiles_bag) {
        nb = bag;
        nt = tile + kStride;
        return;
    }
    nb = bag + 1;
    while (nb < nbags && tab.get(nb, kEntTiles) <= start) ++nb;
    nt = start;
}

#define VLSA_DMA_PIECE(lds_dst, voff, rsrc, soff)                         \
    do {                                                                  \
        unsigned int keep_;                                               \
        asm volatile(                                                     \
            "s_mov_b32 %0, m0\n\t"                                        \
            "s_mov_b32 m0, %1\n\t"                                        \
            "s_nop 0\n\t"                                                 \
            "buffer_load_dwordx4 %2, %3, %4 offen " VLSA_STREAM_NT " lds\n\t" \
            "s_mov_b32 m0, %0"                                            \
            : "=&s"(keep_)                                                \
            : "s"(lds_dst), "v"(voff), "s"(rsrc), "s"(soff)               \
            : "memory");                                                  \
    } while (0)

constexpr int kDmaSlot = 8192;

struct DmaRingBase {
    i32x4 rsrc = {0, 0, 0, 0x00020000};
    int ldb = 0;
    int bag = -1;
    unsigned int lds;
    int cw;

    __device__ __forceinline__ DmaRingBase(unsigned char* ring, int cw_) : lds((unsigned int)(uintptr_t)(lds_void_ptr)ring), cw(cw_) {}
    __device__ __forceinline__ void load(const int_ma* e) {
        const int4 v = *reinterpret_cast<const int4*>(e);
        rsrc[0] = __builtin_amdgcn_readfirstlane(v.x);
        rsrc[1] = __builtin_amdgcn_readfirstlane(v.y);
        rsrc[2] = __builtin_amdgcn_readfirstlane(v.z);
        ldb = __builtin_amdgcn_readfirstlane(v.w);
    }
};

struct DmaRingBf16 : DmaRingBase {
    static constexpr int kTile = 32;
    int lr, chunk_e, chunk_o;
    int voff_e = 0, voff_o = 0;

    __device__ __forceinline__ DmaRingBf16(unsigned char* ring, int lane, int cw_) : DmaRingBase(ring, cw_), lr(lane >> 4) {
        chunk_e = ((lane & 15) ^ (lr << 1)) << 4;
        chunk_o = ((lane & 15) ^ (lr << 1) ^ 8) << 4;
    }
    __device__ __forceinline__ void offsets() {
        voff_e = lr * ldb + cw * 256 + chunk_e;
        voff_o = lr * ldb + cw * 256 + chunk_o;
    }
    __device__ __forceinline__ void bind(int addr_lo, int addr_hi, int span, int pitch) {
        rsrc[0] = addr_lo;
        rsrc[1] = addr_hi;
        rsrc[2] = span;
        ldb = pitch;
        offsets();
    }
    __device__ __forceinline__ void bind(const int_ma* e, int b) {
        if (b != bag) {
            load(e);
            offsets();
            bag = b;
        }
    }
    __device__ __forceinline__ void issue(int tile, int slot) const {
        const int sbase = tile * kTile * ldb;
        const unsigned int dst = lds + slot * kDmaSlot;
#pragma unroll
        for (int i = 0; i < 8; ++i) VLSA_DMA_PIECE(dst + i * 1024, (i & 1) ? voff_o : voff_e, rsrc, sbase + i * 4 * ldb);
    }
};

struct DmaRingF32 : DmaRingBase {
    static constexpr int kTile = 16;
    int lr, lc;
    int voff[8] = {0, 0, 0, 0, 0, 0, 0, 0};

    __device__ __forceinline__ DmaRingF32(unsigned char* ring, int lane, int cw_) : DmaRingBase(ring, cw_), lr(lane >> 5), lc(lane & 31) {}
    __device__ __forceinline__ void bind(const int_ma* e, int b) {
        if (b != bag) {
            load(e);
#pragma unroll
            for (int q = 0; q < 8; ++q) voff[q] = lr * ldb + cw * 512 + ((lc ^ (2 * q + lr)) << 4);
            bag = b;
        }
    }
    __device__ __forceinline__ void issue(int tile, int slot) const {
        const int sbase = tile * kTile * ldb;
        const unsigned int dst = lds + slot * kDmaSlot;
#pragma unroll
        for (int i = 0; i < 8; ++i) VLSA_DMA_PIECE(dst + i * 1024, voff[i], rsrc, sbase + i * 2 * ldb);
    }
};

}
```

vlsa_amd/csrc/vlsa_common.h:

```cpp
#pragma once
#include <hip/hip_runtime.h>
#include <stdint.h>

#include "../../include/vlsa_hip.h"

#ifdef VLSA_EXPERIMENT
#include <cstdlib>
#define VLSA_ENV(name) getenv(name)
#else
#define VLSA_ENV(name) (static_cast<const char*>(nullptr))
#endif

#ifndef VLSA_TAIL_PRIO
#define VLSA_TAIL_PRIO 3
#endif

namespace vlsa {

typedef __bf16 bf16x2 __attribute__((ext_vector_type(2)));
typedef __bf16 bf16x4 __attribute__((ext_vector_type(4)));
typedef __bf16 bf16x8 __attribute__((ext_vector_type(8)));
typedef float f32x4 __attribute__((ext_vector_type(4)));
typedef int i32x4 __attribute__((ext_vector_type(4)));
typedef unsigned int u32x4 __attribute__((ext_vector_type(4)));
typedef __attribute__((address_space(3))) bf16x4* lds_bf16x4_ptr;
typedef __attribute__((address_space(3))) void* lds_void_ptr;
typedef u32x4 __attribute__((may_alias)) u32x4_ma;
typedef bf16x8 __attribute__((may_alias)) bf16x8_ma;
typedef bf16x4 __attribute__((may_alias)) bf16x4_ma;
typedef f32x4 __attribute__((may_alias)) f32x4_ma;
typedef float __attribute__((may_alias)) float_ma;
typedef int __attribute__((may_alias)) int_ma;

static_assert(sizeof(vlsa_bag_desc) == 24, "vlsa_bag_desc is part of the ABI");
static_assert(sizeof(vlsa_rows_desc) == 16, "vlsa_rows_desc is part of the ABI");

constexpr float kLog2e = 1.4426950408889634f;
constexpr float kNormEps = 1e-12f;
constexpr int kPStride = 16;

__device__ __forceinline__ float wave_sum(float v) {
#pragma unroll
    for (int o = 32; o > 0; o >>= 1) v += __shfl_xor(v, o);
    return v;
}
__device__ __forceinline__ float wave_max(float v) {
#pragma unroll
    for (int o = 32; o > 0; o >>= 1) v = fmaxf(v, __shfl_xor(v, o));
    return v;
}
__device__ __forceinline__ float quad_rows_sum(float v) {
    v += __shfl_xor(v, 16);
    v += __shfl_xor(v, 32);
    return v;
}
__device__ __forceinline__ float quad_rows_max(float v) {
    v = fmaxf(v, __shfl_xor(v, 16));
    v = fmaxf(v, __shfl_xor(v, 32));
    return v;
}
__device__ __forceinline__ float row16_sum(float v) {
    v += __builtin_bit_cast(float, __builtin_amdgcn_update_dpp(0, __builtin_bit_cast(int, v), 0x128, 0xf, 0xf, false));
    v += __builtin_bit_cast(float, __builtin_amdgcn_update_dpp(0, __builtin_bit_cast(int, v), 0x124, 0xf, 0xf, false));
    v += __builtin_bit_cast(float, __builtin_amdgcn_update_dpp(0, __builtin_bit_cast(int, v), 0x122, 0xf, 0xf, false));
    v += __builtin_bit_cast(float, __builtin_amdgcn_update_dpp(0, __builtin_bit_cast(int, v), 0x121, 0xf, 0xf, false));
    return v;
}
__device__ __forceinline__ float fast_exp2(float x) { return __builtin_amdgcn_exp2f(x); }

__device__ __forceinline__ int swz(int row, int byte_off) { return row * 256 + (byte_off ^ ((row & 7) << 5)); }

__host__ __device__ __forceinline__ unsigned int dropout_bits(unsigned int seed, unsigned int row, unsigned int unit) {
    unsigned int h = seed ^ (row * 0x9E3779B1u) ^ (unit * 0x85EBCA6Bu);
    h ^= h >> 16;
    h *= 0x85EBCA6Bu;
    h ^= h >> 13;
    h *= 0xC2B2AE35u;
    h ^= h >> 16;
    return h;
}

__host__ __device__ __forceinline__ unsigned int bag_drop_seed(unsigned int s, int b) {
    return b == 0 ? s : dropout_bits(s ^ 0x5BD1E995u, (unsigned int)b, 0xFFFFFFFFu);
}

__device__ __forceinline__ float load_as_float(const float* p) { return *p; }
__device__ __forceinline__ float load_as_float(const __bf16* p) { return (float)*p; }

__device__ __forceinline__ float block_sum_256(float v, float* red) {
    v = wave_sum(v);
    __syncthreads();
    if ((threadIdx.x & 63) == 0) red[threadIdx.x >> 6] = v;
    __syncthreads();
    return red[0] + red[1] + red[2] + red[3];
}

struct QPrepLayout {
    size_t qeff, qsplit, qhat, qnorm, total;
    __host__ __device__ explicit QPrepLayout(int D) {
        qeff = 0;
        qsplit = qeff + (size_t)16 * D * 4;
        qhat = qsplit + (size_t)3 * 16 * D * 2;
        qnorm = qhat + (size_t)17 * D * 4;
        total = qnorm + 32 * 4;
    }
};

}
```

vlsa_amd/functional.py:

```python
from __future__ import annotations

import ctypes
import os
from dataclasses import dataclass
from typing import Optional, Tuple

import numpy as np
import torch
from torch.autograd.function import once_differentiable

from . import _native as nat
from ._native import VlsaNativeError
from .bag_tables import (ChunkTables, _bag2d, _dt, _need_gpu, _p, _stage_table, _stream, bag_rows, checked_bags,
                         merge_strides)

COATTN_SCALE = 100.0


def _f32c(t: torch.Tensor) -> torch.Tensor:
    t = t.detach()
    if t.dtype != torch.float32:
        t = t.float()
    return t.contiguous()

# ... 429 lines not shown
                if name == "That":
                    continue
                k[name] = _p(t)
        nq = self.P + 1 if self.gated else self.P
        dt = _dt(X)
        nat.check(lib.vlsa_vlfan_forward_bag(_p(X), dt, N_, X.stride(0), self.D, None if reuse else _p(Q), nq, int(self.gated), self.scale, _p(T),
                                             self.K, _p(logit_scale), -1 if query_pool_module is not None else self.pool, _p(pool_w),
                                             None if self.identity_head else _p(W), None if self.identity_head else _p(b),
                                             self.kernel, k["qprep"], k["That"], k["tnorm"], k["pm"], k["pl"], k["pacc"], G_,
                                             k["m2"], k["l"], k["out"], k["scores"], k["A"], k["ws"], k["pooled"], k["v"], k["vhat"],
                                             k["vnorm"], k["logits"], k["incidence"], s), "vlsa_vlfan_forward_bag")
        self._params_key = params_key
        if query_pool_module is not None:
            pooled, self.pool_scores = query_pool_attention(self.out[None], query_pool_module)
            nat.check(lib.vlsa_head_forward(_p(pooled), 1, self.D, nat.POOL_GIVEN, None, None if self.identity_head else _p(W),
                                            None if self.identity_head else _p(b), k["That"], self.K, _p(logit_scale), k["ws"],
                                            k["pooled"], k["v"], k["vhat"], k["vnorm"], k["logits"], k["incidence"], s), "vlsa_head_forward")
        if outs and "That" in outs:
            if not reuse or getattr(self, "_That_out", None) is None:
                self._That_out = self.That.clone()
            outs["That"] = self._That_out
        return outs["logits"] if outs and "logits" in outs else self.logits

    def hot_call(self, T, logit_scale, W, b, pool_w, That_out):
        lib, k = self.lib, self._c
        keep = (T, logit_scale, W, b, pool_w, That_out)
        fn_c = lib.vlsa_vlfan_forward_bag
        dt_code = {torch.float32: nat.DT_F32, torch.bfloat16: nat.DT_BF16}
        N, D, K = self.N, self.D, self.K
        any_n = N is None
        nq = self.P + 1 if self.gated else self.P
        args = [None, 0, N or 0, 0, D, None, nq, int(self.gated), self.scale, _p(T), K, _p(logit_scale), self.pool, _p(pool_w),
                None if self.identity_head else _p(W), None if self.identity_head else _p(b), self.kernel, k["qprep"], k["That"],
                k["tnorm"], k["pm"], k["pl"], k["pacc"], self.G, k["m2"], k["l"], k["out"], k["scores"], k["A"], k["ws"], k["pooled"],
                k["v"], None, k["vnorm"], None, k["incidence"], None]
        I_X, I_DT, I_N, I_LD, I_G, I_VHAT, I_LOGITS, I_STREAM = 0, 1, 2, 3, 23, 32, 34, 36
        empty, cur = torch.empty, torch.cuda.current_stream
        partials = _partials_of

        def fn(X):
            dev = X.device
            logits = empty((1, K), dtype=torch.float32, device=dev)
            vhat = empty((1, D), dtype=torch.float32, device=dev)
            a = args
            if any_n:
                n = X.shape[1]
                a[I_N], a[I_G] = n, partials(n)
            a[I_X], a[I_DT], a[I_LD] = X.data_ptr(), dt_code[X.dtype], X.stride(1)
            a[I_VHAT], a[I_LOGITS], a[I_STREAM] = vhat.data_ptr(), logits.data_ptr(), cur(dev).cuda_stream
            rc = fn_c(*a)
            if rc != 0:
                nat.check(rc, "vlsa_vlfan_forward_bag")
            return logits, vhat, That_out
        fn.keep = keep
        return fn

    def run_partial_only(self, X: torch.Tensor):
        dt = _dt(X)
        nat.check(self.lib.vlsa_vlfan_partial(_p(X), dt, self.N if self.N is not None else X.shape[0], X.stride(0), self.D, _p(self.qprep), self.P,
                                              self.kernel, _p(self.pm), _p(self.pl), _p(self.pacc),
                                              _p(self.scores), _stream()), "vlfan_partial")


def _vlfan_dx(bags, qbuf, P: int, scale: float, dout: torch.Tensor, out: torch.Tensor, m2: torch.Tensor, l: torch.Tensor):
    lib = nat.load()
    dev = bags[0].device
    for x in bags:
        if x.dtype != torch.float32 or x.shape[1] != 512:
            raise VlsaNativeError("the HIP aggregation produces dX for fp32 bags with D == 512 only (the output of a trainable "
                                  "Feat_Projecter); detach the bag or use such a bag")
    dxs = list(torch.empty(sum(x.shape[0] for x in bags), 512, dtype=torch.float32, device=dev).split([x.shape[0] for x in bags]))
    B = len(bags)
    tables = ChunkTables.of_list(bags, 64, "vlsa_vlfan_backward_dx", extra=dxs)
    ts, n_tiles = tables.p_tile_start(64)
    delta = torch.empty(B, nat.P_STRIDE, dtype=torch.float32, device=dev)
    nat.check(lib.vlsa_vlfan_backward_dx(tables.p_desc, tables.p_desc2, B, 512, _p(qbuf), P, float(scale), ts, n_tiles, _p(_f32c(dout)), _p(out), _p(m2),
                                         _p(l), _p(delta), _stream()), "vlsa_vlfan_backward_dx")
    return dxs


class _VlfanAggregateFn(torch.autograd.Function):
    @staticmethod
    def forward(ctx, X, Q, gated, coattn_scale, kernel, want_attn):
        X2 = _bag2d(X)
        qp = prepare_queries(Q, gated, coattn_scale)
        pm, pl, pacc, scores = vlfan_partial(X2, qp, kernel, want_scores=want_attn)
        m2, l, out = vlfan_merge(pm, pl, pacc, normalise=True)
        A = attn_normalise(scores, m2, l) if want_attn else torch.empty(0, device=X2.device)
        ctx.save_for_backward(X2, out, m2, l, qp.buf)
        ctx.meta = (qp.nq, qp.P, qp.D, bool(gated), float(coattn_scale))
        ctx.xshape = tuple(X.shape)
        ctx.mark_non_differentiable(A)
        return out, A

    @staticmethod
    def backward(ctx, dout, _dA):
        X2, out, m2, l, qbuf = ctx.saved_tensors
        nq, P, D, gated, scale = ctx.meta
        lib = nat.load()
        N = X2.shape[0]
        dev = X2.device
        dout = _f32c(dout)
        G = num_partials(N)
        pm = torch.empty(G, nat.P_STRIDE, dtype=torch.float32, device=dev)
        pl = torch.empty(G, nat.P_STRIDE, dtype=torch.float32, device=dev)
        pacc = torch.empty(G, P, D, dtype=torch.float32, device=dev)
        prep = torch.empty(lib.vlsa_bwd_prep_bytes(D), dtype=torch.uint8, device=dev)
        dt = _dt(X2)
        if N == 0:
            dE = torch.zeros(P, D, dtype=torch.float32, device=dev)
        else:
            nat.check(lib.vlsa_vlfan_backward(_p(X2), dt, N, X2.stride(0), D, _p(qbuf), P, scale, _p(dout), _p(out),
                                              _p(m2), _p(l), _p(prep), _p(pm), _p(pl), _p(pacc), _stream()),
                      "vlsa_vlfan_backward")
            _, _, dE = vlfan_merge(pm, pl, pacc, normalise=False)
        qp = PreparedQueries(qbuf, nq, P, D, gated)
        qhat, qnorm = qp.qhat, qp.qnorm
        dqh = torch.cat([dE, -dE.sum(dim=0, keepdim=True)], dim=0) if gated else dE
        dQ = (dqh - qhat * (dqh * qhat).sum(dim=-1, keepdim=True)) / qnorm[:, None]
        dX = None
        if ctx.needs_input_grad[0] and N > 0:
            dX = _vlfan_dx([X2], qbuf, P, scale, dout[None], out[None], m2[None], l[None])[0].reshape(ctx.xshape)
        return dX, dQ, None, None, None, None


def vlfan_cross_attention(X: torch.Tensor, Q: torch.Tensor, gated: bool = False, coattn_scale: float = COATTN_SCALE,
                          kernel: int = nat.KERNEL_AUTO, want_attn: bool = False):
    _need_gpu(X, Q)
    if torch.is_grad_enabled() and X.requires_grad and not (X.dtype == torch.float32 and X.shape[-1] == 512):
        _no_bag_grad(X)
    out, A = _VlfanAggregateFn.apply(X, Q.float(), bool(gated), float(coattn_scale), int(kernel), bool(want_attn))
    return out, (A if want_attn else None)


_GROUPS_CACHE: dict = {}


def forward_max_bags() -> int:
    return int(nat.load().vlsa_batch_forward_max_bags())


def choose_groups(sizes, reserved_cus: int = 0) -> int:
    key = (tuple(sizes), int(reserved_cus))
    g = _GROUPS_CACHE.get(key)
    if g is None:
        arr = (ctypes.c_int64 * len(sizes))(*[int(n) for n in sizes])
        g = int(nat.load().vlsa_batch_groups(arr, len(sizes), int(reserved_cus)))
        if len(_GROUPS_CACHE) > 4096:
            _GROUPS_CACHE.clear()
        _GROUPS_CACHE[key] = g
    return g


class AttnBuffers:

    @staticmethod
    def _layout(n, P: int):
        ld = (n + 63) // 64 * 64
        end = (P * ld).cumsum(0)
        return ld, end - P * ld, end

    def __init__(self, sizes, P: int, device, bag_desc: Optional[torch.Tensor] = None):
        self.sizes, self.P = [int(n) for n in sizes], int(P)
        B = len(self.sizes)
        n = np.asarray(self.sizes, dtype=np.int64)
        lds, start, end = self._layout(n, P)
        offs = np.concatenate([start, end[-1:]]) if B else np.zeros(1, dtype=np.int64)
        self.buf = torch.empty(max(int(offs[B]), 4), dtype=torch.float32, device=device)
        base = self.buf.data_ptr()
        if bag_desc is not None and torch.cuda.is_current_stream_capturing():
            dn = bag_desc[:, 1]
            dld, dstart, _ = self._layout(dn, P)
            self.desc = torch.stack([torch.where(dn > 0, dstart * 4 + base, torch.zeros_like(dn)), dld], 1).contiguous()
            self.ndesc = None
        else:
            host = np.zeros(5 * B, dtype=np.int64)
            host[0:2 * B:2] = np.where(n > 0, base + 4 * offs[:B], 0)
            host[1:2 * B:2] = lds
            host[2 * B + 1::3] = n
            dev = _stage_table(host, device, "AttnBuffers")
            self.desc, self.ndesc = dev[:2 * B].view(B, 2), dev[2 * B:].view(B, 3)
        self._offs, self._lds = offs, lds
        self._views = None
        self.max_n = max(self.sizes) if self.sizes else 0

    @property
    def views(self):
        if self._views is None:
            P = self.P
            self._views = [self.buf[int(o):int(o) + P * int(ld)].view(P, int(ld))[:, :n]
                           for o, ld, n in zip(self._offs[:-1], self._lds, self.sizes)]
        return self._views


class BagSet(list):

    def __init__(self, bags=(), D: int = 512, _rows=None):
        if _rows is not None:
            super().__init__(bags)
            self.rows, self.D = _rows, D
        else:
            super().__init__(checked_bags(bags, D, "a BagSet holds non-empty bags with D == 512, one dtype (bf16 or fp32) and one device",
                                          non_empty=True, no_grad="a BagSet holds bags without a gradient of their own (data, not activations)"))
            self.rows, self.D = bag_rows(self), D
        self.sizes = tuple(int(n) for n in self.rows[:, 1])
        self.dt = _dt(self[0]) if len(self) else nat.DT_BF16
        self._chunks, self._groups, self._desc = {}, {}, None

    def take(self, indices) -> "BagSet":
        idx = [int(i) for i in indices]
        return BagSet([self[i] for i in idx], self.D, _rows=self.rows[idx])

    def chunk(self, start: int, n: int) -> "BagSet":
        if start == 0 and n >= len(self):
            return self
        c = self._chunks.get((start, n))
        if c is None:
            c = self._chunks[(start, n)] = BagSet(list.__getitem__(self, slice(start, start + n)), self.D, _rows=self.rows[start:start + n])
        return c

    def groups(self, reserved_cus: int = 0) -> int:
        g = self._groups.get(reserved_cus)
        if g is None:
            g = self._groups[reserved_cus] = choose_groups(self.sizes, reserved_cus)
        return g

    def desc(self) -> torch.Tensor:
        if self._desc is None:
            self._desc = _stage_table(self.rows, self[0].device, "a BagSet's descriptor table (not yet uploaded)")
        return self._desc


class BagSlots(BagSet):

    def __init__(self, source: BagSet, batch: int, groups: Optional[int] = None, t_all: Optional[torch.Tensor] = None,
                 e_all: Optional[torch.Tensor] = None):
        if not isinstance(source, BagSet):
            raise ValueError(f"BagSlots takes a BagSet as its source (checked, resident bags), got {type(source).__name__}")
        batch, M = int(batch), len(source)
        max_bags = int(nat.load().vlsa_batch_max_bags())
        if batch > max_bags:
            raise ValueError(f"BagSlots: batch {batch} is above the {max_bags} bags a batched launch takes")
        if not (1 <= batch <= M):
            raise ValueError(f"BagSlots: batch {batch} outside [1, {M}] (the source holds {M} bags)")
        dev = source[0].device
        for name, lab, dtype in (("t_all", t_all, torch.int64), ("e_all", e_all, torch.float32)):
            if lab is None:
                continue
            if lab.dim() != 1 or lab.shape[0] != M:
                raise ValueError(f"BagSlots: {name} has shape {tuple(lab.shape)}, the source holds {M} bags")
            if lab.device != dev:
                raise ValueError(f"BagSlots: {name} is on {lab.device}, the source's bags are on {dev}")
            if lab.dtype != dtype or not lab.is_contiguous():
                raise ValueError(f"BagSlots: {name} must be a contiguous {dtype} tensor")
        if groups is None:
            rep = sorted(source.sizes)[::max(1, M // batch)][:batch]
            groups = choose_groups(rep, 0)
        groups = int(groups)
        if groups < 1 or groups > batch or groups & (groups - 1):
            raise ValueError(f"BagSlots: groups = {groups} is no power of two in [1, {batch}]")
        first = list(range(batch))
        super().__init__([source[i] for i in first], source.D, _rows=source.rows[first])
        self.dt = source.dt
        self.source, self.batch, self._fixed_groups = source, batch, groups
        self.t_all = t_all if t_all is not None else torch.zeros(M, dtype=torch.int64, device=dev)
        self.e_all = e_all if e_all is not None else torch.zeros(M, dtype=torch.float32, device=dev)
        self._desc = _stage_table(self.rows, dev, "a BagSlots table (built outside a capture)")
        self.t, self.e = self.t_all[:batch].clone(), self.e_all[:batch].clone()

    def groups(self, reserved_cus: int = 0) -> int:
        return self._fixed_groups

    def follow(self, indices) -> None:
        idx = [int(i) for i in indices]
        if len(idx) != self.batch:
            raise ValueError(f"BagSlots.follow: {len(idx)} indices for {self.batch} slots")
        src = self.source
        self[:] = [src[i] for i in idx]
        self.rows = src.rows[idx]
        self.sizes = tuple(int(n) for n in self.rows[:, 1])
        self._chunks.clear()
        self._groups.clear()
        self.__dict__.pop("_plans", None)

    def gather(self, order: torch.Tensor, L: int, cursor: torch.Tensor, status: torch.Tensor) -> None:
        src = self.source
        nat.check(nat.load().vlsa_batch_gather(_p(src.desc()), _p(self.t_all), _p(self.e_all), len(src), _p(order), int(L), self.batch,
                                               _p(cursor), _p(self._desc), _p(self.t), _p(self.e), _p(status), _stream()),
                  "vlsa_batch_gather")


_BATCH_BAGS = "the batched path takes bags with D == 512, one dtype (bf16 or fp32) and one device per batch"


class _BagTable:

    def __init__(self, bags, D=512):
        lib = nat.load()
        B = len(bags)
        if not (1 <= B <= lib.vlsa_batch_max_bags()):
            raise ValueError(f"batch size {B} outside [1, {lib.vlsa_batch_max_bags()}]")
        if isinstance(bags, BagSet) and bags.D == D:
            self.bags, self.B, self.D, self.dt, self.desc = bags, B, D, bags.dt, bags.desc()
            self.sizes = bags.sizes
            return
        self.bags, self.B, self.D = checked_bags(bags, D, _BATCH_BAGS), B, D
        rows = bag_rows(self.bags, D)
        self.dt = _dt(self.bags[0])
        self.desc = _stage_table(rows, self.bags[0].device, "the batched path over a plain list of bags")
        self.sizes = tuple(rows[:, 1].tolist())

    def groups(self, reserved_cus: int = 0) -> int:
        return self.bags.groups(reserved_cus) if isinstance(self.bags, BagSet) else choose_groups(self.sizes, reserved_cus)


class _VlfanBatchAggregateFn(torch.autograd.Function):

    @staticmethod
    def forward(ctx, Q, gated, coattn_scale, table, attn, *bag_tensors):
        lib, s = nat.load(), _stream()
        B, D = table.B, table.D
        dev = table.desc.device
        qp = prepare_queries(Q, gated, coattn_scale)
        P = qp.P
        ws = torch.empty(lib.vlsa_batch_workspace_bytes(B, P, D), dtype=torch.uint8, device=dev)
        groups = table.groups(0)
        nat.check(lib.vlsa_vlfan_partial_batch_scores(_p(table.desc), B, table.dt, D, _p(qp.buf), P, _p(ws), 0, groups,
                                                      None if attn is None else _p(attn.desc), s),
                  "vlsa_vlfan_partial_batch")
        G = int(lib.vlsa_batch_partials_per_bag_ex(B, 0, groups))
        wf = ws.view(torch.float32)
        pm, pl, pacc = wf, wf[B * G * nat.P_STRIDE:], wf[2 * B * G * nat.P_STRIDE:]
        m2 = torch.empty(B, nat.P_STRIDE, dtype=torch.float32, device=dev)
        l = torch.empty(B, nat.P_STRIDE, dtype=torch.float32, device=dev)
        out = torch.empty(B, P, D, dtype=torch.float32, device=dev)
        nat.check(lib.vlsa_vlfan_merge_batch_strided(_p(pm), _p(pl), _p(pacc), B, G, P, D, 1, merge_strides(G, P, D), _p(m2), _p(l), _p(out), s),
                  "vlsa_vlfan_merge_batch_strided")
        if attn is not None:
            nat.check(lib.vlsa_attn_normalise_batch(_p(table.desc), B, P, attn.max_n, _p(attn.desc), _p(m2), _p(l), _p(attn.desc), s),
                      "vlsa_attn_normalise_batch")
        ctx.save_for_backward(out, m2, l, qp.buf)
        ctx.table = table
        ctx.xshapes = [tuple(x.shape) for x in bag_tensors]
        ctx.meta = (qp.nq, P, D, bool(gated), float(coattn_scale))
        return out

    @staticmethod
    def backward(ctx, dout):
        out, m2, l, qbuf = ctx.saved_tensors
        table = ctx.table
        nq, P, D, gated, scale = ctx.meta
        lib, s = nat.load(), _stream()
        B, dev = table.B, out.device
        dout = _f32c(dout)
        persistent = table.dt == nat.DT_F32 or P <= 12
        G = lib.vlsa_bwd_batch_partials() if persistent else B * max(num_partials(n) for n in table.sizes)
        pm = torch.empty(G, nat.P_STRIDE, dtype=torch.float32, device=dev)
        pl = torch.empty(G, nat.P_STRIDE, dtype=torch.float32, device=dev)
        pacc = torch.empty(G, P, D, dtype=torch.float32, device=dev)
        prep = torch.empty(lib.vlsa_bwd_batch_prep_bytes(B, D), dtype=torch.uint8, device=dev)
        if persistent:
            nat.check(lib.vlsa_vlfan_backward_batch(_p(table.desc), B, table.dt, D, _p(qbuf), P, scale, _p(dout), _p(out),
                                                    _p(m2), _p(l), _p(prep), _p(pm), _p(pl), _p(pacc),
                                                    table.groups(0), s),
                      "vlsa_vlfan_backward_batch")
        else:
            nat.check(lib.vlsa_vlfan_backward_bags(_p(table.desc), B, table.dt, D, _p(qbuf), P, scale, _p(dout), _p(out), _p(m2),
                                                   _p(l), _p(prep), _p(pm), _p(pl), _p(pacc), G // B, s), "vlsa_vlfan_backward_bags")
        _, _, dE = vlfan_merge(pm, pl, pacc, normalise=False)
        dQ = torch.empty(nq, D, dtype=torch.float32, device=dev)
        nat.check(lib.vlsa_query_chain(_p(dE.contiguous()), _p(qbuf), nq, int(gated), D, _p(dQ), s), "vlsa_query_chain")
        dxs = [None] * len(ctx.xshapes)
        if any(ctx.needs_input_grad[5:]):
            got = _vlfan_dx(table.bags, qbuf, P, scale, dout, out, m2, l)
            dxs = [g.reshape(shape) if need else None for g, shape, need in zip(got, ctx.xshapes, ctx.needs_input_grad[5:])]
        return (dQ, None, None, None, None, *dxs)


def vlfan_cross_attention_bags(bags, Q: torch.Tensor, gated: bool = False, coattn_scale: float = COATTN_SCALE,
                               want_attn: bool = False):
    if isinstance(bags, BagSet):
        table = _BagTable(bags)
        if not want_attn:
            return _VlfanBatchAggregateFn.apply(Q.float(), bool(gated), float(coattn_scale), table, None)
        attn = AttnBuffers(bags.sizes, Q.shape[0] - (1 if gated else 0), table.desc.device)
        return _VlfanBatchAggregateFn.apply(Q.float(), bool(gated), float(coattn_scale), table, attn), attn.views
    if torch.is_grad_enabled():
        _no_bag_grad(*[x for x in bags if not (x.dtype == torch.float32 and x.shape[-1] == 512)])
    table = _BagTable(bags)
    if 0 in table.sizes:
        raise VlsaNativeError("empty bag in a batch")
    if not want_attn:
        return _VlfanBatchAggregateFn.apply(Q.float(), bool(gated), float(coattn_scale), table, None, *bags)
    P = Q.shape[0] - (1 if gated else 0)
    attn = AttnBuffers(table.sizes, P, table.desc.device)
    out = _VlfanBatchAggregateFn.apply(Q.float(), bool(gated), float(coattn_scale), table, attn, *bags)
    return out, attn.views


def _scored_pool_raw(X2: torch.Tensor, scores: Optional[torch.Tensor]):
    lib = nat.load()
    N, D = X2.shape
    G = int(lib.vlsa_pool_num_partials(N))
    dev = X2.device
    pm = torch.empty(G, nat.P_STRIDE, dtype=torch.float32, device=dev)
    pl = torch.empty(G, nat.P_STRIDE, dtype=torch.float32, device=dev)
    pacc = torch.empty(G, 1, D, dtype=torch.float32, device=dev)
    nat.check(lib.vlsa_scored_pool_partial(_p(X2), _dt(X2), N, X2.stride(0), D, _p(scores), _p(pm), _p(pl), _p(pacc),
                                           _stream()), "vlsa_scored_pool_partial")
    return vlfan_merge(pm, pl, pacc, normalise=True)


def rowdot(X: torch.Tensor, v: torch.Tensor) -> torch.Tensor:
    _need_gpu(X, v)
    lib = nat.load()
    X2 = _bag2d(X)
    N, D = X2.shape
    out = torch.empty(N, dtype=torch.float32, device=X2.device)
    nat.check(lib.vlsa_rowdot(_p(X2), _dt(X2), N, X2.stride(0), D, _p(_f32c(v)), _p(out), _stream()), "vlsa_rowdot")
    return out


class _ScoredPoolFn(torch.autograd.Function):

    @staticmethod
    def forward(ctx, X2, a):
        a = _f32c(a).reshape(-1)
        m2, l, out = _scored_pool_raw(X2, a)
        ctx.save_for_backward(X2, a, m2, l, out)
        return out[0]

    @staticmethod
    def backward(ctx, dpooled):
        X2, a, m2, l, out = ctx.saved_tensors
        dp = _f32c(dpooled).reshape(-1)
        N, D = X2.shape
        da = torch.empty(N, dtype=torch.float32, device=X2.device)
        if D % (8 if X2.dtype == torch.bfloat16 else 4) == 0 and D <= nat.MAX_D:
            nat.check(nat.load().vlsa_scored_pool_backward(_p(X2), _dt(X2), N, X2.stride(0), D, _p(a), _p(m2), _p(l), _p(out), _p(dp),
                                                           _p(da), _stream()), "vlsa_scored_pool_backward")
            return None, da
        xd = rowdot(X2, dp)
        A = torch.exp2(a * 1.4426950408889634 - m2[0]) / l[0]
        return None, A * (xd - (out[0] * dp).sum())


def scored_pool(X: torch.Tensor, scores: Optional[torch.Tensor]) -> torch.Tensor:
    _need_gpu(X, scores)
    _no_bag_grad(X)
    X2 = _bag2d(X)
    if X2.shape[0] == 0:
        raise ValueError("empty bag")
    if scores is None:
        return _scored_pool_raw(X2, None)[2][0]
    return _ScoredPoolFn.apply(X2, scores)


def colmax(X: torch.Tensor) -> torch.Tensor:
    _need_gpu(X)
    lib = nat.load()
    X2 = _bag2d(X)
    N, D = X2.shape
    G = int(lib.vlsa_pool_num_partials(N))
    part = torch.empty(G, D, dtype=torch.float32, device=X2.device)
    out = torch.empty(D, dtype=torch.float32, device=X2.device)
    nat.check(lib.vlsa_colmax(_p(X2), _dt(X2), N, X2.stride(0), D, _p(part), _p(out), _stream()), "vlsa_colmax")
    return out


def adapter_head(f: torch.Tensor, W1: torch.Tensor, W2: torch.Tensor, keep_ratio: float) -> torch.Tensor:
    _need_gpu(f, W1, W2)
    lib = nat.load()
    f = _f32c(f).reshape(-1)
    R, D = W1.shape
    hid = torch.empty(R, dtype=torch.float32, device=f.device)
    out = torch.empty(D, dtype=torch.float32, device=f.device)
    nat.check(lib.vlsa_adapter_head(_p(f), D, _p(_f32c(W1)), R, _p(_f32c(W2)), float(keep_ratio), _p(hid), _p(out), _stream()),
              "vlsa_adapter_head")
    return out


def attn_scores(H: torch.Tensor, Hg: Optional[torch.Tensor], b1, bg, w2, b2) -> torch.Tensor:
    _need_gpu(H)
    lib = nat.load()
    H = _f32c(H)
    N, hid = H.shape
    a = torch.empty(N, dtype=torch.float32, device=H.device)
    Hg_ = _f32c(Hg) if Hg is not None else None
    nat.check(lib.vlsa_attn_scores(_p(H), _p(Hg_), N, hid, _p(_f32c(b1)), _p(_f32c(bg)) if bg is not None else None,
                                   _p(_f32c(w2).reshape(-1)), _p(_f32c(b2).reshape(-1)), _p(a), _stream()),
              "vlsa_attn_scores")
    return a


_SCORE_TILES = {}
_NO_FUSED_POOL = os.environ.get("VLSA_GS_NO_FUSED_POOL", "") == "1"


def _score_tiles(name: str, f32: bool, gated: bool, second=ctypes.c_int):
    t = _SCORE_TILES.get((name, f32, gated))
    if t is None:
        a, b = ctypes.c_int(0), second(0)
        nat.check(getattr(nat.load(), name)(nat.DT_F32 if f32 else nat.DT_BF16, int(gated), ctypes.addressof(a), ctypes.addressof(b)), name)
        t = _SCORE_TILES[(name, f32, gated)] = (a.value, b.value)
    return t


def _score_tiling(f32: bool, gated: bool):
    return _score_tiles("vlsa_gated_scores_tiling", f32, gated)


def _score_big_tile(f32: bool, gated: bool):
    return _score_tiles("vlsa_gated_scores_big_tile", f32, gated, ctypes.c_int64)


def score_tile_rows(sizes, f32: bool, gated: bool, allow_big: bool, tiling=None):
    max_rows, round_tiles, big_rows, big_min = tiling or (*_score_tiling(f32, gated), *_score_big_tile(f32, gated))
# ... 569 lines not shown
        plan = ctx.plan
        dev, B = Y.device, plan.B
        grads = []
        for g, n in zip(dys, plan.sizes):
            g = torch.zeros(n, 512, dtype=torch.float32, device=dev) if g is None else _f32c(g).reshape(n, 512)
            grads.append(g if g.data_ptr() % 16 == 0 else g.clone())
        if plan.on_device:
            base = grads[0].data_ptr()
            if any(g.data_ptr() != base + 2048 * o for g, o in zip(grads, plan.offs)):
                packed = torch.cat(grads)
                grads, base = [packed], packed.data_ptr()
            t, dy_desc = plan.tables, plan.tables.packed_desc(base)
            p_dy = dy_desc.data_ptr()
        else:
            t = ChunkTables.of_list(plan.bags, plan.tr, "the batched Feat_Projecter over a plain list of bags", extra=grads)
            p_dy = t.p_desc2
        ts, n_tiles = t.p_tile_start(plan.tr)
        nat.check(lib.vlsa_feat_project_rowstats_batch(p_dy, B, _p(Y), t.p_row_off, plan.total, _p(prep), _p(stats), s),
                  "vlsa_feat_project_rowstats_batch")
        ws = torch.empty(lib.vlsa_mlp_bwd_workspace_bytes(2, n_tiles), dtype=torch.uint8, device=dev)
        dW = torch.empty(512, 512, dtype=torch.float32, device=dev)
        dvec = torch.empty(3, 512, dtype=torch.float32, device=dev)
        nat.check(lib.vlsa_feat_project_backward(t.p_desc, p_dy, B, plan.dt, _p(prep), ts, n_tiles, _p(stats), t.p_row_off, _p(ws), _p(dW),
                                                 _p(dvec), s), "vlsa_feat_project_backward")
        hb, hg, hbt = ctx.has
        return None, None, dW, dvec[0] if hb else None, dvec[1] if hg else None, dvec[2] if hbt else None, None


def feat_project_bags(bags, fused: "FusedFeatProjecter", W, b, gamma, beta, eps: float) -> list:
    B = _chunk_len(bags)
    _need_gpu(bags[0])
    dev = bags[0].device
    if torch.cuda.is_current_stream_capturing():
        fused = FusedFeatProjecter()
    prep = fused.packed(dev, W, b, gamma, beta)
    plan = FeatProjBagsPlan.of(bags)
    if torch.is_grad_enabled() and any(t is not None and t.requires_grad for t in (W, b, gamma, beta)):
        _no_bag_grad(*bags)
        return ProjectedBags(_FeatProjectBagsFn.apply(plan, prep, W, b, gamma, beta, float(eps)), plan)
    Y, _ = _feat_project_bags_launch(plan, prep, eps, False)
    return ProjectedBags(Y.split(plan.sizes), plan)


class _ProjectMaxPoolFn(torch.autograd.Function):

    @staticmethod
    def forward(ctx, plan, prep, W, b, gamma, beta, eps):
        B = plan.B
        Y, stats = _feat_project_bags_launch(plan, prep, eps, True)
        if not hasattr(plan, "part_start"):
            lib = nat.load()
            plan.part_table(lib.vlsa_colmax_part_rows, lib.vlsa_colmax_parts)
        pooled, idx = _colmax_launch(plan.tables.packed_desc(Y.data_ptr()), B, nat.DT_F32, plan.part_start, plan.n_parts)
        rows = (plan.tables.row_off[:, None] + idx).reshape(-1)
        sel_stats = torch.zeros(B * 512, 4, dtype=torch.float32, device=Y.device)
        sel_stats[:, :2] = stats.index_select(0, rows)[:, :2]
        ctx.save_for_backward(gather_rows_bags(plan.desc, B, plan.dt, idx), Y.index_select(0, rows), sel_stats, prep)
        ctx.B = B
        ctx.has = (b is not None, gamma is not None, beta is not None)
        return pooled

    @staticmethod
    @once_differentiable
    def backward(ctx, dpooled):
        lib, s = nat.load(), _stream()
        Xsel, Ysel, stats, prep = ctx.saved_tensors
        dev, B = Xsel.device, ctx.B
        dY = torch.diag_embed(_f32c(dpooled)).reshape(B * 512, 512)
        n = torch.full((B,), 512, dtype=torch.int64, device=dev)
        first = torch.arange(B, dtype=torch.int64, device=dev) * (512 * 2048)
        t = ChunkTables.from_device(torch.stack([first + Xsel.data_ptr(), n, n], 1).contiguous(), [512] * B, nat.DT_F32)
        dy_desc = t.packed_desc(dY.data_ptr())
        tile_rows = int(lib.vlsa_mlp_bwd_tile_rows(nat.DT_F32))
        ts, n_tiles = t.p_tile_start(tile_rows)
        nat.check(lib.vlsa_feat_project_rowstats_batch(_p(dy_desc), B, _p(Ysel), t.p_row_off, B * 512, _p(prep), _p(stats), s),
                  "vlsa_feat_project_rowstats_batch")
        ws = torch.empty(lib.vlsa_mlp_bwd_workspace_bytes(2, n_tiles), dtype=torch.uint8, device=dev)
        dW = torch.empty(512, 512, dtype=torch.float32, device=dev)
        dvec = torch.empty(3, 512, dtype=torch.float32, device=dev)
        nat.check(lib.vlsa_feat_project_backward(t.p_desc, _p(dy_desc), B, nat.DT_F32, _p(prep), ts, n_tiles, _p(stats), t.p_row_off, _p(ws),
                                                 _p(dW), _p(dvec), s), "vlsa_feat_project_backward")
        hb, hg, hbt = ctx.has
        return None, None, dW, dvec[0] if hb else None, dvec[1] if hg else None, dvec[2] if hbt else None, None


def project_max_pool_bags(bags, fused: "FusedFeatProjecter", W, b, gamma, beta, eps: float) -> torch.Tensor:
    _chunk_len(bags)
    _need_gpu(bags[0])
    if not (torch.is_grad_enabled() and any(t is not None and t.requires_grad for t in (W, b, gamma, beta))):
        return max_pool_bags(feat_project_bags(bags, fused, W, b, gamma, beta, eps))
    _no_bag_grad(*bags)
    if torch.cuda.is_current_stream_capturing():
        fused = FusedFeatProjecter()
    prep = fused.packed(bags[0].device, W, b, gamma, beta)
    return _ProjectMaxPoolFn.apply(FeatProjBagsPlan.of(bags), prep, W, b, gamma, beta, float(eps))


def topk_mean(S: torch.Tensor, k: int, out_scale: float = 1.0) -> torch.Tensor:
    _need_gpu(S)
    lib = nat.load()
    S = _f32c(S)
    C, N = S.shape
    out = torch.empty(C, dtype=torch.float32, device=S.device)
    ws = torch.empty(max(4, lib.vlsa_topk_workspace_bytes(C, N, int(k))), dtype=torch.uint8, device=S.device)
    nat.check(lib.vlsa_topk_mean_ws(_p(S), C, N, int(k), float(out_scale), _p(ws), _p(out), _stream()), "vlsa_topk_mean_ws")
    return out


def normalize_many(X: torch.Tensor) -> torch.Tensor:
    _need_gpu(X)
    lib = nat.load()
    X2 = _bag2d(X)
    N, D = X2.shape
    out = torch.empty(N, D, dtype=torch.float32, device=X2.device)
    nat.check(lib.vlsa_normalize_many(_p(X2), _dt(X2), N, X2.stride(0), D, _p(out), _stream()), "vlsa_normalize_many")
    return out


def class_cosines(X: torch.Tensor, T: torch.Tensor) -> torch.Tensor:
    _need_gpu(X, T)
    K = T.shape[0]
    outs = []
    for k0 in range(0, K, nat.MAX_P):
        qp = prepare_queries(T[k0:k0 + nat.MAX_P], False, 1.0 / 1.4426950408889634)
        _, _, _, sc = vlfan_partial(X, qp, want_scores=True)
        outs.append(sc)
    return outs[0] if len(outs) == 1 else torch.cat(outs, dim=0)


class VlfanBatchPlan:

    def __init__(self, B: int, P: int, K: int, device, D: int = 512, gated: bool = False, pool: str = "mean",
                 identity_head: bool = False, coattn_scale: float = COATTN_SCALE, reserved_cus: int = 0,
                 want_attn: bool = False):
        lib = nat.load()
        self.reserved_cus = int(reserved_cus)
        if not (1 <= B <= lib.vlsa_batch_forward_max_bags()):
            raise ValueError(f"batch size {B} outside [1, {lib.vlsa_batch_forward_max_bags()}]")
        self.lib, self.B, self.D, self.P, self.K = lib, B, D, P, K
        self.gated, self.pool, self.identity_head, self.scale = gated, _POOL_CODES[pool], identity_head, float(coattn_scale)
        f = lambda *s: torch.empty(*s, dtype=torch.float32, device=device)
        self.desc_host = torch.zeros(B, 3, dtype=torch.int64).pin_memory() if torch.cuda.is_available() else torch.zeros(B, 3, dtype=torch.int64)
        self.desc = torch.zeros(B, 3, dtype=torch.int64, device=device)
        self.ws = torch.zeros(lib.vlsa_batch_workspace_bytes(B, P, D), dtype=torch.uint8, device=device)
        self.qprep = torch.empty(lib.vlsa_qprep_bytes(D), dtype=torch.uint8, device=device)
        self.That, self.tnorm = f(K, D), f(K)
        self.m2, self.l, self.out = f(B, nat.P_STRIDE), f(B, nat.P_STRIDE), f(B, P, D)
        self.pooled, self.v, self.vhat, self.vnorm = f(B, D), f(B, D), f(B, D), f(B)
        self.logits, self.incidence = f(B, K), f(B, K)
        self._bags = None
        self.want_attn, self.attn = bool(want_attn), None
        self.dt = nat.DT_BF16
        self.groups = 0
        self._desc_np = self.desc_host.numpy()
        self._desc_ev = None
        self._c = {k: _p(getattr(self, k)) for k in ("desc", "ws", "qprep", "That", "tnorm", "m2", "l", "out", "pooled", "v",
                                                     "vhat", "vnorm", "logits", "incidence")}

    def set_bags(self, bags, validated: bool = False):
        if len(bags) != self.B:
            raise ValueError(f"expected {self.B} bags, got {len(bags)}")
        if isinstance(bags, BagSet) and bags.D == self.D:
            keep, rows, sizes, self.dt, self.groups = bags, bags.rows, bags.sizes, bags.dt, bags.groups(self.reserved_cus)
        else:
            keep = list(bags) if validated else checked_bags(bags, self.D, _BATCH_BAGS)
            rows = bag_rows(keep, self.D)
            sizes = tuple(rows[:, 1].tolist())
            self.dt, self.groups = _dt(keep[0]), choose_groups(sizes, self.reserved_cus)
        if self._desc_ev is not None:
            self._desc_ev.synchronize()
        self._desc_np[:] = rows
        self._bags = keep
        if self.want_attn and (self.attn is None or tuple(self.attn.sizes) != sizes):
            self.attn = AttnBuffers(sizes, self.P, self.desc.device)
        self.desc.copy_(self.desc_host, non_blocking=True)
        if self.desc_host.is_pinned():
            self._desc_ev = torch.cuda.Event()
            self._desc_ev.record()

    def run(self, Q, T, logit_scale, W=None, b=None, pool_w=None, outs: Optional[dict] = None, params_key=None):
        lib, s, c, k = self.lib, _stream(), nat.check, self._c
        reuse = params_key is not None and params_key == getattr(self, "_params_key", None)
        self._params_key = None
        own_That = None
        if outs:
            k = dict(k)
            for name, t in outs.items():
                if name == "That" and params_key is not None:
                    own_That = t
                    continue
                k[name] = _p(t)
        nq = self.P + 1 if self.gated else self.P
        if not reuse:
            c(lib.vlsa_prepare_queries_and_text(_p(Q), nq, self.D, int(self.gated), self.scale, k["qprep"], _p(T), self.K,
                                                k["That"], k["tnorm"], s), "prepare_queries_and_text")
        self._params_key = params_key
        if own_That is not None:
            own_That.copy_(self.That)
        ad = _p(self.attn.desc) if self.want_attn else None
        c(lib.vlsa_vlfan_forward_batch_attn(k["desc"], self.B, self.dt, self.D, k["qprep"], self.P, self.pool,
                                            _p(pool_w), None if self.identity_head else _p(W),
                                            None if self.identity_head else _p(b), k["That"], self.K, _p(logit_scale),
                                            k["ws"], k["m2"], k["l"], k["out"], k["pooled"], k["v"], k["vhat"], k["vnorm"],
                                            k["logits"], k["incidence"], self.reserved_cus, self.groups, ad, ad,
                                            self.attn.max_n if self.want_attn else 0, s), "vlfan_forward_batch")
        return outs["logits"] if outs and "logits" in outs else self.logits

    def capture(self, Q, T, logit_scale, W=None, b=None, pool_w=None):
        side = torch.cuda.Stream(device=self.desc.device)
        side.wait_stream(torch.cuda.current_stream())
        with torch.cuda.stream(side):
            self.run(Q, T, logit_scale, W, b, pool_w)
        torch.cuda.current_stream().wait_stream(side)
        g = torch.cuda.CUDAGraph()
        with torch.cuda.graph(g):
            self.run(Q, T, logit_scale, W, b, pool_w)
        self._graph_keep = (Q, T, logit_scale, W, b, pool_w)
        return g

    def run_partial_only(self):
        nat.check(self.lib.vlsa_vlfan_partial_batch_scores(_p(self.desc), self.B, self.dt, self.D, _p(self.qprep), self.P,
                                                           _p(self.ws), self.reserved_cus, self.groups,
                                                           _p(self.attn.desc) if self.want_attn else None, _stream()),
                  "vlfan_partial_batch")


def _zeroshot_launches(table, T: torch.Tensor, ls: torch.Tensor, k: Optional[int], want_idx: bool):
    lib, s = nat.load(), _stream()
    K, B, dev = T.shape[0], table.B, table.desc.device
    kk = 0 if k is None else int(k)
    vals, idxs, qps = [], [], []
    for k0 in range(0, K, nat.MAX_P):
        qp = prepare_queries(T[k0:k0 + nat.MAX_P], False, 1.0 / 1.4426950408889634)
        Pk = qp.P
        sc = AttnBuffers(table.sizes, Pk, dev, bag_desc=table.desc)
        ws = torch.empty(lib.vlsa_batch_workspace_bytes(B, Pk, table.D), dtype=torch.uint8, device=dev)
        nat.check(lib.vlsa_vlfan_partial_batch_scores(_p(table.desc), B, table.dt, table.D, _p(qp.buf), Pk, _p(ws), 0,
                                                      table.groups(0), _p(sc.desc), s), "vlsa_vlfan_partial_batch_scores")
        part = torch.empty(B, Pk, dtype=torch.float32, device=dev)
        if want_idx:
            idx = torch.empty(B, Pk, kk, dtype=torch.int32, device=dev) if kk else None
            nat.check(lib.vlsa_topk_select_batch(_p(table.desc), _p(sc.desc), B, Pk, kk, _p(ls), _p(part), _p(idx), s),
                      "vlsa_topk_select_batch")
            idxs.append(idx)
        else:
            nat.check(lib.vlsa_topk_mean_batch(_p(table.desc), _p(sc.desc), B, Pk, kk, _p(ls), _p(part), s), "vlsa_topk_mean_batch")
        vals.append(part)
        qps.append(qp)
    one = len(vals) == 1
    idx = None if not (want_idx and kk) else (idxs[0] if one else torch.cat(idxs, 1))
    return (vals[0] if one else torch.cat(vals, 1)), idx, qps


class _ZeroshotPoolFn(torch.autograd.Function):

    @staticmethod
    def forward(ctx, T, logit_scale, k, table, *bag_tensors):
        lib = nat.load()
        B, dev = table.B, table.desc.device
        ls = _f32c(logit_scale).reshape(1)
        logits, sel, qps = _zeroshot_launches(table, _f32c(T), ls, k, True)
        That = qps[0].qhat if len(qps) == 1 else torch.cat([q.qhat for q in qps], 0)
        tnorm = qps[0].qnorm if len(qps) == 1 else torch.cat([q.qnorm for q in qps], 0)
        if k is None:
            sel = torch.empty(B, 512, dtype=torch.float32, device=dev)
            uws = torch.empty(lib.vlsa_unit_mean_workspace_bytes(B), dtype=torch.uint8, device=dev)
            nat.check(lib.vlsa_unit_mean_batch(_p(table.desc), B, table.dt, table.D, _p(uws), _p(sel), _stream()), "vlsa_unit_mean_batch")
        ctx.save_for_backward(sel, logits, That, tnorm, ls)
        ctx.table, ctx.k, ctx.bags = table, k, bag_tensors
        ctx.shapes, ctx.dtypes = (T.shape, logit_scale.shape), (T.dtype, logit_scale.dtype)
        ctx.set_materialize_grads(False)
        return logits, That

    @staticmethod
    @once_differentiable
    def backward(ctx, dlogits, g_That):
        sel, logits, That, tnorm, ls = ctx.saved_tensors
        table, k = ctx.table, ctx.k
        K = That.shape[0]
        dT = dls = None
        if dlogits is not None:
            g = _f32c(dlogits)
            dT = torch.empty(K, 512, dtype=torch.float32, device=That.device)
            dls = torch.empty(1, dtype=torch.float32, device=That.device)
            nat.check(nat.load().vlsa_zeroshot_backward_batch(_p(table.desc), table.B, table.dt, table.D, K, 0 if k is None else int(k),
                                                              None if k is None else _p(sel), _p(sel) if k is None else None, _p(g),
                                                              _p(logits), _p(That), _p(tnorm), _p(ls), _p(dT), _p(dls), _stream()),
                      "vlsa_zeroshot_backward_batch")
            dls = dls.reshape(ctx.shapes[1]).to(ctx.dtypes[1])
        if g_That is not None:
            gt = g_That.float()
            gt = (gt - (gt * That).sum(1, keepdim=True) * That) / tnorm[:, None]
            dT = gt if dT is None else dT + gt
        if dT is not None:
            dT = dT.reshape(ctx.shapes[0]).to(ctx.dtypes[0])
        return (dT, dls, None, None, *([None] * len(ctx.bags)))


def zeroshot_pool_bags(bags, T: torch.Tensor, logit_scale: torch.Tensor, k: Optional[int], return_text: bool = False):
    _need_gpu(T, logit_scale, *bags)
    if torch.is_grad_enabled() and (T.requires_grad or logit_scale.requires_grad):
        _no_bag_grad(*bags)
        table = _BagTable(bags)
        logits, That = _ZeroshotPoolFn.apply(T, logit_scale, k, table, *table.bags)
        return (logits, That) if return_text else logits
    out, _, _ = _zeroshot_launches(_BagTable(bags), T, _f32c(logit_scale).reshape(1), k, False)
    return (out, normalize_rows(T)[0]) if return_text else out


def query_pool_attention(rows: torch.Tensor, module) -> Tuple[torch.Tensor, torch.Tensor]:
    _need_gpu(rows)
    lib = nat.load()
    rows = _f32c(rows)
    B, P, D = rows.shape
    gated = hasattr(module, "fc1")
    if gated:
        la, lg, l2 = module.fc1[0], module.score[0], module.fc2
        Wg, bg = _f32c(lg.weight), _f32c(lg.bias)
    else:
        la, l2 = module.attention[0], module.attention[2]
        Wg = bg = None
    hid = la.weight.shape[0]
    ws = torch.empty(B * ((hid + 3) // 4) * nat.P_STRIDE, dtype=torch.float32, device=rows.device)
    pooled = torch.empty(B, D, dtype=torch.float32, device=rows.device)
    scores = torch.empty(B, P, dtype=torch.float32, device=rows.device)
    nat.check(lib.vlsa_query_pool_attention(_p(rows), B, P, D, _p(_f32c(la.weight)), _p(_f32c(la.bias)), _p(Wg), _p(bg),
                                            _p(_f32c(l2.weight).reshape(-1)), _p(_f32c(l2.bias).reshape(-1)), hid, int(not gated),
                                            _p(ws), _p(pooled), _p(scores), _stream()), "vlsa_query_pool_attention")
    return pooled, scores


class DsmilBagsPlan(_ChunkPlan):

    def __init__(self, bags):
        lib = nat.load()
        super().__init__(_chunk_tables(bags, "the batched DSMIL route over a plain list of bags"))
        self.part_table(lib.vlsa_dsmil_part_rows, lib.vlsa_dsmil_parts)


def dsmil_state_views(state: torch.Tensor, B: int, C: int) -> dict:
    names = ("crit", "cmax", "m2", "l", "xcrit", "qmax", "u", "z", "bm")
    off = (ctypes.c_int64 * len(names))()
    total = int(nat.load().vlsa_dsmil_state_floats(B, C, off))
    o = list(off) + [total]
    shapes = ((B, 16), (B, 16), (B, 16), (B, 16), (B, C, 512), (B, C, 256), (B, C, 512), (B, C, 512), (B, C, 256))
    out = {k: state[o[i]:o[i + 1]].view(*sh) for i, (k, sh) in enumerate(zip(names, shapes))}
    out["crit"] = out["crit"].view(torch.int32)
    return out


class _DsmilBagsFn(torch.autograd.Function):

    @staticmethod
    def forward(ctx, plan, drop_p, seed_word, want_attn, Wc, bc, Wq, bq, Wv, bv, Wf, bf, *bag_tensors):
        lib, s = nat.load(), _stream()
        dev, B, C = plan.desc.device, plan.B, Wc.shape[0]
        w = [_f32c(t) for t in (Wc, bc, Wq, bq, Wv, bv, Wf, bf)]
        ws = torch.empty(lib.vlsa_dsmil_workspace_bytes(plan.n_parts, C), dtype=torch.uint8, device=dev)
        state = torch.empty(lib.vlsa_dsmil_state_floats(B, C, None), dtype=torch.float32, device=dev)
        logits = torch.empty(B, C, dtype=torch.float32, device=dev)
        attn = torch.empty(plan.total, dtype=torch.float32, device=dev) if want_attn else None
        nat.check(lib.vlsa_dsmil_forward_batch(_p(plan.desc), B, plan.dt, Wc.shape[1], Wq.shape[0], C, _p(plan.part_start), plan.n_parts,
                                               *[_p(t) for t in w], float(drop_p), _p(seed_word), _p(ws), _p(state), _p(logits), _p(attn),
                                               _p(plan.a_off), s), "vlsa_dsmil_forward_batch")
        ctx.save_for_backward(state, seed_word, w[2], w[4], w[6])
        ctx.plan, ctx.drop_p, ctx.C = plan, float(drop_p), C
        ctx.shapes = [t.shape for t in (Wc, bc, Wq, bq, Wv, bv, Wf, bf)]
        ctx.bags = bag_tensors
        if attn is None:
            attn = logits.new_empty(0)
        crit = dsmil_state_views(state, B, C)["crit"][:, :C].clone()
        ctx.mark_non_differentiable(attn, crit)
        return logits, attn, crit

    @staticmethod
    def backward(ctx, dlogits, _dattn, _dcrit):
        lib, s = nat.load(), _stream()
        state, seed_word, Wq, Wv, Wf = ctx.saved_tensors
        plan, C = ctx.plan, ctx.C
        dev, B = state.device, plan.B
        g = _f32c(dlogits)
        ws = torch.empty(lib.vlsa_dsmil_workspace_bytes(plan.n_parts, C), dtype=torch.uint8, device=dev)
        grads = [torch.empty(sh, dtype=torch.float32, device=dev) for sh in ctx.shapes]
        nat.check(lib.vlsa_dsmil_backward_batch(_p(plan.desc), B, plan.dt, 512, 256, C, _p(plan.part_start), plan.n_parts, _p(Wq), _p(Wv),
                                                _p(Wf), _p(g), ctx.drop_p, _p(seed_word), _p(state), _p(ws), *[_p(t) for t in grads], s),
                  "vlsa_dsmil_backward_batch")
        return (None, None, None, None, *grads, *([None] * len(ctx.bags)))


def dsmil_bags(bags, Wc, bc, Wq, bq, Wv, bv, Wf, bf, drop_p: float = 0.0, seed_word: Optional[torch.Tensor] = None,
               want_attn: bool = False):
# ... 219 lines not shown
```

Baseline: 6.044 billion.

## Deal bags to workgroup groups by size to balance batched kernel load

Adds a host-side scheduler that reorders bags across workgroup groups, using snake or greedy dealing of size-sorted bags under a simple cost model, and picks the group count with the lowest estimated critical path. The forward, score and backward batch kernels take a permutation table and map slot indices to bag ids. The aim is to cut tail imbalance when bag sizes differ. For a single bag or equal-size bags the order stays the identity, so this benchmark likely sees no effect beyond a small per-bag indirection cost.

Result: no change. 6.081 billion, median of 6 (+0.6%).

```diff
diff --git a/include/vlsa_hip.h b/include/vlsa_hip.h
--- a/include/vlsa_hip.h
+++ b/include/vlsa_hip.h
@@ -121,6 +121,19 @@
                              int groups, void* stream);
 int vlsa_vlfan_partial_batch_scores(const void* bag_desc, int B, int x_dtype, int D, const void* qprep, int P, void* workspace,
                                     int reserved_cus, int groups, const void* scores_desc, void* stream);
+
+int vlsa_batch_deal(const int64_t* rows_host, int B, int reserved_cus, int unit_rows, int workgroups, unsigned char* order_out);
+double vlsa_batch_deal_cost(const int64_t* rows_host, int B, int reserved_cus, int unit_rows, int workgroups, int groups,
+                            const unsigned char* order);
+int vlsa_vlfan_partial_batch_scores_dealt(const void* bag_desc, int B, int x_dtype, int D, const void* qprep, int P, void* workspace,
+                                          int reserved_cus, int groups, const unsigned char* order, const void* scores_desc,
+                                          void* stream);
+int vlsa_vlfan_forward_batch_attn_dealt(const void* bag_desc, int B, int x_dtype, int D, const void* qprep, int P, int pool_mode,
+                                        const float* pool_w, const float* W, const float* b, const float* That, int K,
+                                        const float* logit_scale, void* workspace, float* m2, float* l, float* out, float* pooled,
+                                        float* v, float* vhat, float* vnorm, float* logits, float* incidence, int reserved_cus,
+                                        int groups, const unsigned char* order, const void* scores_desc, const void* attn_desc,
+                                        int64_t max_N, void* stream);
 int vlsa_attn_normalise_batch(const void* bag_desc, int B, int P, int64_t max_N, const void* scores_desc, const float* m2,
                               const float* l, const void* attn_desc, void* stream);
 int vlsa_vlfan_forward_batch_attn(const void* bag_desc, int B, int x_dtype, int D, const void* qprep, int P, int pool_mode,
@@ -134,6 +147,10 @@
 int vlsa_vlfan_backward_batch(const void* bag_desc, int B, int x_dtype, int D, const void* qprep, int P,
                               float coattn_scale, const float* dout, const float* out, const float* m2, const float* l,
                               void* bwd_prep, float* pm, float* pl, float* pacc, int groups, void* stream);
+int vlsa_vlfan_backward_batch_dealt(const void* bag_desc, int B, int x_dtype, int D, const void* qprep, int P,
+                                    float coattn_scale, const float* dout, const float* out, const float* m2, const float* l,
+                                    void* bwd_prep, float* pm, float* pl, float* pacc, int groups, const unsigned char* order,
+                                    void* stream);
 
 int vlsa_vlfan_backward_bags(const void* bag_desc, int B, int x_dtype, int D, const void* qprep, int P, float coattn_scale,
                              const float* dout, const float* out, const float* m2, const float* l, void* bwd_prep, float* pm,
diff --git a/vlsa_amd/csrc/launch.h b/vlsa_amd/csrc/launch.h
--- a/vlsa_amd/csrc/launch.h
+++ b/vlsa_amd/csrc/launch.h
@@ -29,6 +29,20 @@
     hipLaunchKernelGGL(Kernel, grid, block, lds_bytes, stream, args...);
 }
 
+inline bool deal_order(const unsigned char* order, int B, DealOrder* out) {
+    if (B < 1 || B > 256) return false;
+    bool seen[256] = {};
+    for (int t = 0; t < 256; ++t) out->at[t] = (unsigned char)(t < B ? t : 0);
+    if (!order) return true;
+    for (int t = 0; t < B; ++t) {
+        const int bag = order[t];
+        if (bag >= B || seen[bag]) return false;
+        seen[bag] = true;
+        out->at[t] = (unsigned char)bag;
+    }
+    return true;
+}
+
 struct DropSpec {
     unsigned int thr = 0u;
     float scale = 1.f;
diff --git a/vlsa_amd/csrc/vlfan_backward_batch.hip b/vlsa_amd/csrc/vlfan_backward_batch.hip
--- a/vlsa_amd/csrc/vlfan_backward_batch.hip
+++ b/vlsa_amd/csrc/vlfan_backward_batch.hip
@@ -51,7 +51,7 @@
                                                                      const float* __restrict__ m2, const float* __restrict__ l,
                                                                      const float* __restrict__ delta, float scale,
                                                                      float* __restrict__ pm, float* __restrict__ pl,
-                                                                     float* __restrict__ pacc, int S) {
+                                                                     float* __restrict__ pacc, int S, const DealOrder order) {
     using namespace bb;
     constexpr int D = 512;
     extern __shared__ __attribute__((aligned(16))) unsigned char smem[];
@@ -69,9 +69,10 @@
     const int xslot = i16 < bb::kMaxP ? (i16 + 4 * g) % bb::kMaxP : (4 * g) % bb::kMaxP;
 
     if (tid < B) {
-        const vlsa_bag_desc d = bags[tid];
+        const int bag_id = deal_at<bb::kMaxBags / 4>(order, tid);
+        const vlsa_bag_desc d = bags[bag_id];
         const unsigned int vb = (unsigned int)((b + (tid / S) * 37) % G);
-        stream_split<5, 2, kTile>(d, G, vb, (tid % S) == grp, tab.entry(tid));
+        stream_split<5, 2, kTile>(d, G, vb, (tid % S) == grp, tab.entry(bag_id));
     }
     bf16x8 qf[3][4];
 #pragma unroll
@@ -267,7 +268,7 @@
 
 int vlsa_launch_backward_f32_batch(const void* bag_desc, int B, const __bf16* qsplit, const __bf16* dsplit, int P,
                                    const float* m2, const float* l, const float* delta, float scale, float* pm, float* pl,
-                                   float* pacc, int S, hipStream_t s);
+                                   float* pacc, int S, const DealOrder& order, hipStream_t s);
 
 extern "C" int vlsa_bwd_batch_partials(void) { return 512; }
 
@@ -289,11 +290,13 @@
     return VLSA_OK;
 }
 
-extern "C" int vlsa_vlfan_backward_batch(const void* bag_desc, int B, int x_dtype, int D, const void* qprep, int P,
-                                         float coattn_scale, const float* dout, const float* out, const float* m2,
-                                         const float* l, void* bwd_prep, float* pm, float* pl, float* pacc, int groups,
-                                         void* stream) {
+extern "C" int vlsa_vlfan_backward_batch_dealt(const void* bag_desc, int B, int x_dtype, int D, const void* qprep, int P,
+                                               float coattn_scale, const float* dout, const float* out, const float* m2,
+                                               const float* l, void* bwd_prep, float* pm, float* pl, float* pacc, int groups,
+                                               const unsigned char* order, void* stream) {
     hipStream_t s = (hipStream_t)stream;
+    DealOrder dealt;
+    if (B < 1 || B > bb::kMaxBags || !deal_order(order, B, &dealt)) return VLSA_EINVAL;
     const __bf16 *qsplit, *dsplit;
     const float* delta;
     const int rc = backward_prepare(bag_desc, B, x_dtype, D, qprep, P, bb::kMaxP, dout, out, m2, l, bwd_prep, pm, pl, pacc, s, &qsplit, &dsplit,
@@ -306,10 +309,18 @@
         S = p2;
     }
     if (x_dtype == VLSA_DT_F32)
-        return vlsa_launch_backward_f32_batch(bag_desc, B, qsplit, dsplit, P, m2, l, delta, coattn_scale, pm, pl, pacc, S, s);
+        return vlsa_launch_backward_f32_batch(bag_desc, B, qsplit, dsplit, P, m2, l, delta, coattn_scale, pm, pl, pacc, S, dealt, s);
     launch_lds<k_vlfan_backward_dma_batch>(dim3(512), dim3(256), bb::kLdsBytes, s, static_cast<const vlsa_bag_desc*>(bag_desc), B,
-                                           qsplit, dsplit, P, m2, l, delta, coattn_scale, pm, pl, pacc, S);
+                                           qsplit, dsplit, P, m2, l, delta, coattn_scale, pm, pl, pacc, S, dealt);
     return launch_status();
+}
+
+extern "C" int vlsa_vlfan_backward_batch(const void* bag_desc, int B, int x_dtype, int D, const void* qprep, int P,
+                                         float coattn_scale, const float* dout, const float* out, const float* m2,
+                                         const float* l, void* bwd_prep, float* pm, float* pl, float* pacc, int groups,
+                                         void* stream) {
+    return vlsa_vlfan_backward_batch_dealt(bag_desc, B, x_dtype, D, qprep, P, coattn_scale, dout, out, m2, l, bwd_prep, pm, pl, pacc,
+                                           groups, nullptr, stream);
 }
 
 int vlsa_launch_backward_mfma_bags(const void* bag_desc, int B, int x_dtype, const __bf16* qsplit, const __bf16* dsplit, int P,
diff --git a/vlsa_amd/csrc/vlfan_backward_batch_f32.hip b/vlsa_amd/csrc/vlfan_backward_batch_f32.hip
--- a/vlsa_amd/csrc/vlfan_backward_batch_f32.hip
+++ b/vlsa_amd/csrc/vlfan_backward_batch_f32.hip
@@ -23,7 +23,7 @@
                                                                      const float* __restrict__ m2, const float* __restrict__ l,
                                                                      const float* __restrict__ delta, float scale,
                                                                      float* __restrict__ pm, float* __restrict__ pl,
-                                                                     float* __restrict__ pacc, int S) {
+                                                                     float* __restrict__ pacc, int S, const DealOrder order) {
     using namespace bbf;
     constexpr int D = 512;
     extern __shared__ __attribute__((aligned(16))) unsigned char smem[];
@@ -39,9 +39,10 @@
     const bool pok = i16 < P;
 
     if (tid < B) {
-        const vlsa_bag_desc d = bags[tid];
+        const int bag_id = deal_at<bbf::kMaxBags / 4>(order, tid);
+        const vlsa_bag_desc d = bags[bag_id];
         const unsigned int vb = (unsigned int)((b + (tid / S) * 37) % G);
-        stream_split<4, 4, kTile>(d, G, vb, (tid % S) == grp, tab.entry(tid));
+        stream_split<4, 4, kTile>(d, G, vb, (tid % S) == grp, tab.entry(bag_id));
     }
     bf16x8 qs[3][4];
 #pragma unroll
@@ -235,8 +236,8 @@
 
 int vlsa_launch_backward_f32_batch(const void* bag_desc, int B, const __bf16* qsplit, const __bf16* dsplit, int P,
                                    const float* m2, const float* l, const float* delta, float scale, float* pm, float* pl,
-                                   float* pacc, int S, hipStream_t s) {
+                                   float* pacc, int S, const DealOrder& order, hipStream_t s) {
     launch_lds<k_vlfan_backward_f32_batch>(dim3(512), dim3(256), bbf::kLdsBytes, s, static_cast<const vlsa_bag_desc*>(bag_desc), B,
-                                           qsplit, dsplit, P, m2, l, delta, scale, pm, pl, pacc, S);
+                                           qsplit, dsplit, P, m2, l, delta, scale, pm, pl, pacc, S, order);
     return launch_status();
 }
diff --git a/vlsa_amd/csrc/vlfan_batch.hip b/vlsa_amd/csrc/vlfan_batch.hip
--- a/vlsa_amd/csrc/vlfan_batch.hip
+++ b/vlsa_amd/csrc/vlfan_batch.hip
@@ -50,7 +50,7 @@
                                                                      const __bf16* __restrict__ qsplit, int P,
                                                                      float* __restrict__ pm, float* __restrict__ pl,
                                                                      float* __restrict__ pacc, int S,
-                                                                     const vlsa_rows_desc* __restrict__ sdesc) {
+                                                                     const vlsa_rows_desc* __restrict__ sdesc, const DealOrder order) {
     using namespace bt;
     constexpr int D = 512;
     extern __shared__ __attribute__((aligned(16))) unsigned char smem[];
@@ -73,11 +73,12 @@
 
     const int nloc = grp < B ? (B - grp + S - 1) / S : 0;
     if (tid < nloc) {
-        const int bag_id = grp + tid * S;
+        const int bag_id = deal_at<64>(order, grp + tid * S);
         const vlsa_bag_desc d = bags[bag_id];
         const unsigned int vb = (unsigned int)((b + tid * 37) % G);
         int_ma* e = tab.entry(tid);
         const long long rbeg = stream_split<6, 2, kTile>(d, G, vb, true, e);
+        e[kEntBag] = bag_id;
         if constexpr (kScores) {
             const vlsa_rows_desc sd = sdesc[bag_id];
             const unsigned long long sp = sd.ptr ? reinterpret_cast<unsigned long long>(sd.ptr + rbeg) : 0ull;
@@ -315,7 +316,7 @@
                 am[r] = (Mm4[r] == -INFINITY) ? 0.f : fast_exp2(Mm4[r] - mn);
                 ao[r] = (Mo4[r] == -INFINITY) ? 0.f : fast_exp2(Mo4[r] - mn);
             }
-            const size_t slotg = (size_t)(grp + bag * S) * G + tab.get(bag, kEntSlot);
+            const size_t slotg = (size_t)tab.get(bag, kEntBag) * G + tab.get(bag, kEntSlot);
             if (w == 0 && g == 0 && i16 < P) {
                 const float Mn = fmaxf(M, Mo);
                 const float fm = (M == -INFINITY) ? 0.f : fast_exp2(M - Mn);
@@ -678,6 +679,116 @@
     return best;
 }
 
+namespace {
+struct DealModel {
+    const int64_t* rows;
+    int B, unit_rows, workgroups, reserved_cus;
+    int launched(int S) const {
+        int r = reserved_cus < 0 ? 0 : reserved_cus;
+        r = (r + S - 1) / S * S;
+        if (r > workgroups - S) r = workgroups - S;
+        return workgroups - r;
+    }
+    int64_t bag_cost(int bag, int S) const {
+        const int Gb = launched(S) / S;
+        const int64_t n = rows[bag] > 0 ? rows[bag] : 0, units = (n + unit_rows - 1) / unit_rows;
+        return (units + Gb - 1) / Gb * 10 + 7;
+    }
+    int64_t slowest(const unsigned char* order, int S) const {
+        int64_t worst = 0;
+        for (int g = 0; g < S; ++g) {
+            int64_t c = 0;
+            for (int t = g; t < B; t += S) c += bag_cost(order[t], S);
+            if (c > worst) worst = c;
+        }
+        return worst;
+    }
+};
+
+void by_size(const DealModel& m, int* idx) {
+    for (int i = 0; i < m.B; ++i) idx[i] = i;
+    for (int i = 1; i < m.B; ++i) {
+        const int v = idx[i];
+        int j = i;
+        while (j > 0 && m.rows[idx[j - 1]] < m.rows[v]) { idx[j] = idx[j - 1]; --j; }
+        idx[j] = v;
+    }
+}
+
+void order_of(const int* grp, int B, int S, unsigned char* order) {
+    int filled[256] = {};
+    for (int bag = 0; bag < B; ++bag) order[grp[bag] + (filled[grp[bag]]++) * S] = (unsigned char)bag;
+}
+
+void deal_snake(const DealModel& m, const int* sorted, int S, unsigned char* order) {
+    int grp[256], room[256];
+    for (int g = 0; g < S; ++g) room[g] = (m.B - g + S - 1) / S;
+    int g = 0, dir = 1;
+    for (int i = 0; i < m.B; ++i) {
+        while (room[g] == 0) {
+            if (g + dir < 0 || g + dir >= S) dir = -dir; else g += dir;
+        }
+        grp[sorted[i]] = g;
+        --room[g];
+        if (g + dir < 0 || g + dir >= S) dir = -dir; else g += dir;
+    }
+    order_of(grp, m.B, S, order);
+}
+
+void deal_greedy(const DealModel& m, const int* sorted, int S, unsigned char* order) {
+    int grp[256], room[256];
+    int64_t load[256];
+    for (int g = 0; g < S; ++g) {
+        room[g] = (m.B - g + S - 1) / S;
+        load[g] = 0;
+    }
+    for (int i = 0; i < m.B; ++i) {
+        int best = -1;
+        for (int g = 0; g < S; ++g)
+            if (room[g] > 0 && (best < 0 || load[g] < load[best])) best = g;
+        grp[sorted[i]] = best;
+        --room[best];
+        load[best] += m.bag_cost(sorted[i], S);
+    }
+    order_of(grp, m.B, S, order);
+}
+}
+
+extern "C" int vlsa_batch_deal(const int64_t* rows_host, int B, int reserved_cus, int unit_rows, int workgroups,
+                               unsigned char* order_out) {
+    if (!rows_host || !order_out || B < 1 || B > bt::kMaxBags || unit_rows < 1 || workgroups < 1) return 0;
+    for (int t = 0; t < B; ++t) order_out[t] = (unsigned char)t;
+    const int S0 = vlsa_batch_groups(rows_host, B, reserved_cus);
+    bool equal = true;
+    for (int t = 1; t < B; ++t) equal = equal && rows_host[t] == rows_host[0];
+    if (equal || S0 > workgroups) return S0;
+    const DealModel m{rows_host, B, unit_rows, workgroups, reserved_cus};
+    int sorted[256];
+    by_size(m, sorted);
+    int best = S0;
+    int64_t best_cost = m.slowest(order_out, S0);
+    unsigned char cand[256];
+    for (int S = min_groups(B); S <= 256 && S <= B && S <= workgroups; S *= 2) {
+        for (int how = 0; how < 2; ++how) {
+            if (how == 0) deal_snake(m, sorted, S, cand); else deal_greedy(m, sorted, S, cand);
+            const int64_t c = m.slowest(cand, S);
+            if (c < best_cost) {
+                best_cost = c;
+                best = S;
+                for (int t = 0; t < B; ++t) order_out[t] = cand[t];
+            }
+        }
+    }
+    return best;
+}
+
+extern "C" double vlsa_batch_deal_cost(const int64_t* rows_host, int B, int reserved_cus, int unit_rows, int workgroups, int groups,
+                                       const unsigned char* order) {
+    DealOrder o;
+    if (!rows_host || unit_rows < 1 || groups < 1 || groups > B || groups > workgroups || !deal_order(order, B, &o)) return -1.0;
+    return (double)DealModel{rows_host, B, unit_rows, workgroups, reserved_cus}.slowest(o.at, groups) / 10.0;
+}
+
 extern "C" int vlsa_batch_max_bags(void) { return 64; }
 extern "C" int vlsa_batch_forward_max_bags(void) { return bt::kMaxBags; }
 
@@ -687,15 +798,18 @@
 }
 
 int vlsa_launch_partial_f32_batch(const void* bag_desc, int B, const float* qeff, const float* qmeta, int P, float* pm,
-                                  float* pl, float* pacc, int S, int workgroups, const void* scores_desc, hipStream_t s);
-
-extern "C" int vlsa_vlfan_partial_batch_scores(const void* bag_desc, int B, int x_dtype, int D, const void* qprep, int P,
-                                               void* workspace, int reserved_cus, int groups, const void* scores_desc,
-                                               void* stream) {
+                                  float* pl, float* pacc, int S, int workgroups, const void* scores_desc, const DealOrder& order,
+                                  hipStream_t s);
+
+extern "C" int vlsa_vlfan_partial_batch_scores_dealt(const void* bag_desc, int B, int x_dtype, int D, const void* qprep, int P,
+                                                     void* workspace, int reserved_cus, int groups, const unsigned char* order,
+                                                     const void* scores_desc, void* stream) {
     if (!bag_desc || !qprep || !workspace) return VLSA_EINVAL;
     if (B < 1 || B > bt::kMaxBags || P < 1 || P > VLSA_MAX_P) return VLSA_EINVAL;
     if (x_dtype != VLSA_DT_BF16 && x_dtype != VLSA_DT_F32) return VLSA_EINVAL;
     if (D != 512) return VLSA_EUNSUPPORTED;
+    DealOrder dealt;
+    if (!deal_order(order, B, &dealt)) return VLSA_EINVAL;
     const int S = resolve_groups(B, groups);
     const int WG = batch_workgroups(S, reserved_cus);
     const int G = WG / S;
@@ -707,7 +821,7 @@
         const unsigned char* qp = static_cast<const unsigned char*>(qprep);
         return vlsa_launch_partial_f32_batch(bag_desc, B, reinterpret_cast<const float*>(qp + L.qeff),
                                              reinterpret_cast<const float*>(qp + L.qnorm), P, pm, pl, pacc, S, WG, scores_desc,
-                                             (hipStream_t)stream);
+                                             dealt, (hipStream_t)stream);
     }
     const __bf16* qsplit = reinterpret_cast<const __bf16*>(static_cast<const unsigned char*>(qprep) + L.qsplit);
 #ifdef VLSA_TIMING
@@ -718,12 +832,19 @@
     if (!scores_desc)
         launch_lds<k_vlfan_partial_dma_batch<false>>(dim3(WG), dim3(512), bt::kLdsBytes, (hipStream_t)stream,
                                                      static_cast<const vlsa_bag_desc*>(bag_desc), B, qsplit, P, pm, pl, pacc, S | (xm << 8),
-                                                     static_cast<const vlsa_rows_desc*>(nullptr));
+                                                     static_cast<const vlsa_rows_desc*>(nullptr), dealt);
     else
         launch_lds<k_vlfan_partial_dma_batch<true>>(dim3(WG), dim3(512), bt::kLdsBytes, (hipStream_t)stream,
                                                     static_cast<const vlsa_bag_desc*>(bag_desc), B, qsplit, P, pm, pl, pacc, S,
-                                                    static_cast<const vlsa_rows_desc*>(scores_desc));
+                                                    static_cast<const vlsa_rows_desc*>(scores_desc), dealt);
     return launch_status();
+}
+
+extern "C" int vlsa_vlfan_partial_batch_scores(const void* bag_desc, int B, int x_dtype, int D, const void* qprep, int P,
+                                               void* workspace, int reserved_cus, int groups, const void* scores_desc,
+                                               void* stream) {
+    return vlsa_vlfan_partial_batch_scores_dealt(bag_desc, B, x_dtype, D, qprep, P, workspace, reserved_cus, groups, nullptr, scores_desc,
+                                                 stream);
 }
 
 extern "C" int vlsa_vlfan_partial_batch_ex(const void* bag_desc, int B, int x_dtype, int D, const void* qprep, int P,
@@ -748,19 +869,20 @@
     return vlsa_vlfan_partial_batch_ex(bag_desc, B, x_dtype, D, qprep, P, workspace, 0, 0, stream);
 }
 
-extern "C" int vlsa_vlfan_forward_batch_attn(const void* bag_desc, int B, int x_dtype, int D, const void* qprep, int P,
-                                             int pool_mode, const float* pool_w, const float* W, const float* b,
-                                             const float* That, int K, const float* logit_scale, void* workspace, float* m2,
-                                             float* l, float* out, float* pooled, float* v, float* vhat, float* vnorm,
-                                             float* logits, float* incidence, int reserved_cus, int groups,
-                                             const void* scores_desc, const void* attn_desc, int64_t max_N, void* stream) {
+extern "C" int vlsa_vlfan_forward_batch_attn_dealt(const void* bag_desc, int B, int x_dtype, int D, const void* qprep, int P,
+                                                   int pool_mode, const float* pool_w, const float* W, const float* b,
+                                                   const float* That, int K, const float* logit_scale, void* workspace, float* m2,
+                                                   float* l, float* out, float* pooled, float* v, float* vhat, float* vnorm,
+                                                   float* logits, float* incidence, int reserved_cus, int groups,
+                                                   const unsigned char* order, const void* scores_desc, const void* attn_desc,
+                                                   int64_t max_N, void* stream) {
     if (!That || !logit_scale || !m2 || !l || !out || !pooled || !v || !vhat || !vnorm || !logits) return VLSA_EINVAL;
     if (K < 1 || K > VLSA_MAX_K) return VLSA_EINVAL;
     if ((scores_desc == nullptr) != (attn_desc == nullptr)) return VLSA_EINVAL;
     if (pool_mode < VLSA_POOL_MEAN || pool_mode > VLSA_POOL_WEIGHT) return VLSA_EINVAL;
     if (pool_mode == VLSA_POOL_WEIGHT && !pool_w) return VLSA_EINVAL;
-    const int rc = vlsa_vlfan_partial_batch_scores(bag_desc, B, x_dtype, D, qprep, P, workspace, reserved_cus, groups, scores_desc,
-                                                   stream);
+    const int rc = vlsa_vlfan_partial_batch_scores_dealt(bag_desc, B, x_dtype, D, qprep, P, workspace, reserved_cus, groups, order,
+                                                         scores_desc, stream);
     if (rc != VLSA_OK) return rc;
     hipStream_t s = (hipStream_t)stream;
     const int G = vlsa_batch_partials_per_bag_ex(B, reserved_cus, groups);
@@ -778,6 +900,17 @@
     return vlsa_attn_normalise_batch(bag_desc, B, P, max_N, scores_desc, m2, l, attn_desc, stream);
 }
 
+extern "C" int vlsa_vlfan_forward_batch_attn(const void* bag_desc, int B, int x_dtype, int D, const void* qprep, int P,
+                                             int pool_mode, const float* pool_w, const float* W, const float* b,
+                                             const float* That, int K, const float* logit_scale, void* workspace, float* m2,
+                                             float* l, float* out, float* pooled, float* v, float* vhat, float* vnorm,
+                                             float* logits, float* incidence, int reserved_cus, int groups,
+                                             const void* scores_desc, const void* attn_desc, int64_t max_N, void* stream) {
+    return vlsa_vlfan_forward_batch_attn_dealt(bag_desc, B, x_dtype, D, qprep, P, pool_mode, pool_w, W, b, That, K, logit_scale,
+                                               workspace, m2, l, out, pooled, v, vhat, vnorm, logits, incidence, reserved_cus, groups,
+                                               nullptr, scores_desc, attn_desc, max_N, stream);
+}
+
 extern "C" int vlsa_vlfan_forward_batch(const void* bag_desc, int B, int x_dtype, int D, const void* qprep, int P,
                                         int pool_mode, const float* pool_w, const float* W, const float* b,
                                         const float* That, int K, const float* logit_scale, void* workspace, float* m2,
diff --git a/vlsa_amd/csrc/vlfan_batch_f32.hip b/vlsa_amd/csrc/vlfan_batch_f32.hip
--- a/vlsa_amd/csrc/vlfan_batch_f32.hip
+++ b/vlsa_amd/csrc/vlfan_batch_f32.hip
@@ -27,7 +27,8 @@
                                                                      const float* __restrict__ qeff, const float* __restrict__ qmeta, int P,
                                                                      float* __restrict__ pm, float* __restrict__ pl,
                                                                      float* __restrict__ pacc, int S,
-                                                                     const vlsa_rows_desc* __restrict__ sdesc, const vlsa_bag_desc one) {
+                                                                     const vlsa_rows_desc* __restrict__ sdesc, const vlsa_bag_desc one,
+                                                                     const DealOrder order) {
     using namespace bf;
     constexpr int D = 512;
     extern __shared__ __attribute__((aligned(16))) unsigned char smem[];
@@ -44,11 +45,12 @@
 
     const int nloc = grp < B ? (B - grp + S - 1) / S : 0;
     if (tid < nloc) {
-        const int bag_id = grp + tid * S;
+        const int bag_id = deal_at<64>(order, grp + tid * S);
         const vlsa_bag_desc d = bags ? bags[bag_id] : one;
         const unsigned int vb = (unsigned int)((b + tid * 37) % G);
         int_ma* e = tab.entry(tid);
         const long long rbeg = stream_split<5, 4, kTile>(d, G, vb, true, e);
+        e[kEntBag] = bag_id;
         if constexpr (kScores) {
             const vlsa_rows_desc sd = sdesc[bag_id];
             const unsigned long long sp = sd.ptr ? reinterpret_cast<unsigned long long>(sd.ptr + rbeg) : 0ull;
@@ -284,7 +286,7 @@
                 am[r] = (Mm4[r] == -INFINITY) ? 0.f : fast_exp2(Mm4[r] - mn);
                 ao[r] = (Mo4[r] == -INFINITY) ? 0.f : fast_exp2(Mo4[r] - mn);
             }
-            const size_t slotg = (size_t)(grp + bag * S) * G + tab.get(bag, kEntSlot);
+            const size_t slotg = (size_t)tab.get(bag, kEntBag) * G + tab.get(bag, kEntSlot);
             if (w == 0 && g == 0 && i16 < P) {
                 const float Mn = fmaxf(M, Mo);
                 const float fm = (M == -INFINITY) ? 0.f : fast_exp2(M - Mn);
@@ -321,21 +323,25 @@
 using namespace vlsa;
 
 int vlsa_launch_partial_f32_batch(const void* bag_desc, int B, const float* qeff, const float* qmeta, int P, float* pm,
-                                  float* pl, float* pacc, int S, int workgroups, const void* scores_desc, hipStream_t s) {
+                                  float* pl, float* pacc, int S, int workgroups, const void* scores_desc, const DealOrder& order,
+                                  hipStream_t s) {
     if (!scores_desc)
         launch_lds<k_vlfan_partial_f32_batch<false>>(dim3(workgroups), dim3(512), bf::kLdsBytes, s,
                                                      static_cast<const vlsa_bag_desc*>(bag_desc), B, qeff, qmeta, P, pm, pl, pacc, S,
-                                                     static_cast<const vlsa_rows_desc*>(nullptr), vlsa_bag_desc{nullptr, 0, 0});
+                                                     static_cast<const vlsa_rows_desc*>(nullptr), vlsa_bag_desc{nullptr, 0, 0}, order);
     else
         launch_lds<k_vlfan_partial_f32_batch<true>>(dim3(workgroups), dim3(512), bf::kLdsBytes, s,
                                                     static_cast<const vlsa_bag_desc*>(bag_desc), B, qeff, qmeta, P, pm, pl, pacc, S,
-                                                    static_cast<const vlsa_rows_desc*>(scores_desc), vlsa_bag_desc{nullptr, 0, 0});
+                                                    static_cast<const vlsa_rows_desc*>(scores_desc), vlsa_bag_desc{nullptr, 0, 0}, order);
     return launch_status();
 }
 
 int vlsa_launch_partial_f32_one(const float* X, int64_t N, int64_t ldx, const float* qeff, const float* qmeta, int P, float* pm,
                                 float* pl, float* pacc, int G, hipStream_t s) {
+    DealOrder one_bag;
+    (void)deal_order(nullptr, 1, &one_bag);
     launch_lds<k_vlfan_partial_f32_batch<false>>(dim3(G), dim3(512), bf::kLdsBytes, s, static_cast<const vlsa_bag_desc*>(nullptr), 1,
-                                                 qeff, qmeta, P, pm, pl, pacc, 1, static_cast<const vlsa_rows_desc*>(nullptr), vlsa_bag_desc{X, N, ldx});
+                                                 qeff, qmeta, P, pm, pl, pacc, 1, static_cast<const vlsa_rows_desc*>(nullptr), vlsa_bag_desc{X, N, ldx},
+                                                 one_bag);
     return launch_status();
 }
diff --git a/vlsa_amd/csrc/vlfan_stream.h b/vlsa_amd/csrc/vlfan_stream.h
--- a/vlsa_amd/csrc/vlfan_stream.h
+++ b/vlsa_amd/csrc/vlfan_stream.h
@@ -30,6 +30,7 @@
     kEntScoreLo,
     kEntScoreHi,
     kEntScorePitch,
+    kEntBag,
 };
 
 template <int kInts>
diff --git a/vlsa_amd/csrc/vlsa_common.h b/vlsa_amd/csrc/vlsa_common.h
--- a/vlsa_amd/csrc/vlsa_common.h
+++ b/vlsa_amd/csrc/vlsa_common.h
@@ -38,6 +38,24 @@
 constexpr float kLog2e = 1.4426950408889634f;
 constexpr float kNormEps = 1e-12f;
 constexpr int kPStride = 16;
+
+struct DealOrder {
+    union {
+        unsigned char at[256];
+        unsigned int w[64];
+    };
+};
+
+template <int kWords>
+__device__ __forceinline__ int deal_at(const DealOrder& order, int pos) {
+    unsigned int mine = 0;
+#pragma unroll
+    for (int d = 0; d < kWords; ++d) {
+        const unsigned int wd = order.w[d];
+        if ((pos >> 2) == d) mine = wd;
+    }
+    return (int)((mine >> (8 * (pos & 3))) & 0xffu);
+}
 
 __device__ __forceinline__ float wave_sum(float v) {
 #pragma unroll
diff --git a/vlsa_amd/functional.py b/vlsa_amd/functional.py
--- a/vlsa_amd/functional.py
+++ b/vlsa_amd/functional.py
@@ -605,6 +605,28 @@
     return g
 
 
+_DEAL_CACHE: dict = {}
+
+
+def choose_deal(sizes, reserved_cus: int = 0, dt: Optional[int] = None):
+    unit = 32 if dt == nat.DT_F32 else 64
+    key = (tuple(sizes), int(reserved_cus), unit)
+    d = _DEAL_CACHE.get(key)
+    if d is None:
+        B = len(sizes)
+        arr = (ctypes.c_int64 * B)(*[int(n) for n in sizes])
+        order = (ctypes.c_ubyte * B)()
+        S = int(nat.load().vlsa_batch_deal(arr, B, int(reserved_cus), unit, 256, order))
+        if S < 1:
+            raise nat.VlsaNativeError(f"vlsa_batch_deal refused a batch of {B} bags")
+        order = bytes(order)
+        d = (S, None if order == bytes(range(B)) else order)
+        if len(_DEAL_CACHE) > 4096:
+            _DEAL_CACHE.clear()
+        _DEAL_CACHE[key] = d
+    return d
+
+
 class AttnBuffers:
 
     @staticmethod
@@ -658,7 +680,7 @@
             self.rows, self.D = bag_rows(self), D
         self.sizes = tuple(int(n) for n in self.rows[:, 1])
         self.dt = _dt(self[0]) if len(self) else nat.DT_BF16
-        self._chunks, self._groups, self._desc = {}, {}, None
+        self._chunks, self._groups, self._deals, self._desc = {}, {}, {}, None
 
     def take(self, indices) -> "BagSet":
         idx = [int(i) for i in indices]
@@ -677,6 +699,12 @@
         if g is None:
             g = self._groups[reserved_cus] = choose_groups(self.sizes, reserved_cus)
         return g
+
+    def deal(self, reserved_cus: int = 0):
+        d = self._deals.get(reserved_cus)
+        if d is None:
+            d = self._deals[reserved_cus] = choose_deal(self.sizes, reserved_cus, self.dt)
+        return d
 
     def desc(self) -> torch.Tensor:
         if self._desc is None:
@@ -724,6 +752,9 @@
     def groups(self, reserved_cus: int = 0) -> int:
         return self._fixed_groups
 
+    def deal(self, reserved_cus: int = 0):
+        return self._fixed_groups, None
+
     def follow(self, indices) -> None:
         idx = [int(i) for i in indices]
         if len(idx) != self.batch:
@@ -734,6 +765,7 @@
         self.sizes = tuple(int(n) for n in self.rows[:, 1])
         self._chunks.clear()
         self._groups.clear()
+        self._deals.clear()
         self.__dict__.pop("_plans", None)
 
     def gather(self, order: torch.Tensor, L: int, cursor: torch.Tensor, status: torch.Tensor) -> None:
@@ -766,6 +798,9 @@
     def groups(self, reserved_cus: int = 0) -> int:
         return self.bags.groups(reserved_cus) if isinstance(self.bags, BagSet) else choose_groups(self.sizes, reserved_cus)
 
+    def deal(self, reserved_cus: int = 0):
+        return self.bags.deal(reserved_cus) if isinstance(self.bags, BagSet) else choose_deal(self.sizes, reserved_cus, self.dt)
+
 
 class _VlfanBatchAggregateFn(torch.autograd.Function):
 
@@ -777,9 +812,9 @@
         qp = prepare_queries(Q, gated, coattn_scale)
         P = qp.P
         ws = torch.empty(lib.vlsa_batch_workspace_bytes(B, P, D), dtype=torch.uint8, device=dev)
-        groups = table.groups(0)
-        nat.check(lib.vlsa_vlfan_partial_batch_scores(_p(table.desc), B, table.dt, D, _p(qp.buf), P, _p(ws), 0, groups,
-                                                      None if attn is None else _p(attn.desc), s),
+        groups, order = table.deal(0)
+        nat.check(lib.vlsa_vlfan_partial_batch_scores_dealt(_p(table.desc), B, table.dt, D, _p(qp.buf), P, _p(ws), 0, groups, order,
+                                                            None if attn is None else _p(attn.desc), s),
                   "vlsa_vlfan_partial_batch")
         G = int(lib.vlsa_batch_partials_per_bag_ex(B, 0, groups))
         wf = ws.view(torch.float32)
@@ -793,7 +828,7 @@
             nat.check(lib.vlsa_attn_normalise_batch(_p(table.desc), B, P, attn.max_n, _p(attn.desc), _p(m2), _p(l), _p(attn.desc), s),
                       "vlsa_attn_normalise_batch")
         ctx.save_for_backward(out, m2, l, qp.buf)
-        ctx.table = table
+        ctx.table, ctx.deal = table, (groups, order)
         ctx.xshapes = [tuple(x.shape) for x in bag_tensors]
         ctx.meta = (qp.nq, P, D, bool(gated), float(coattn_scale))
         return out
@@ -813,9 +848,10 @@
         pacc = torch.empty(G, P, D, dtype=torch.float32, device=dev)
         prep = torch.empty(lib.vlsa_bwd_batch_prep_bytes(B, D), dtype=torch.uint8, device=dev)
         if persistent:
-            nat.check(lib.vlsa_vlfan_backward_batch(_p(table.desc), B, table.dt, D, _p(qbuf), P, scale, _p(dout), _p(out),
-                                                    _p(m2), _p(l), _p(prep), _p(pm), _p(pl), _p(pacc),
-                                                    table.groups(0), s),
+            groups, order = ctx.deal
+            nat.check(lib.vlsa_vlfan_backward_batch_dealt(_p(table.desc), B, table.dt, D, _p(qbuf), P, scale, _p(dout), _p(out),
+                                                          _p(m2), _p(l), _p(prep), _p(pm), _p(pl), _p(pacc),
+                                                          groups, order, s),
                       "vlsa_vlfan_backward_batch")
         else:
             nat.check(lib.vlsa_vlfan_backward_bags(_p(table.desc), B, table.dt, D, _p(qbuf), P, scale, _p(dout), _p(out), _p(m2),
@@ -1691,21 +1727,32 @@
         self.want_attn, self.attn = bool(want_attn), None
         self.dt = nat.DT_BF16
         self.groups = 0
+        self.order = None
         self._desc_np = self.desc_host.numpy()
         self._desc_ev = None
         self._c = {k: _p(getattr(self, k)) for k in ("desc", "ws", "qprep", "That", "tnorm", "m2", "l", "out", "pooled", "v",
                                                      "vhat", "vnorm", "logits", "incidence")}
 
+    @property
+    def groups(self) -> int:
+        return self._groups
+
+    @groups.setter
+    def groups(self, S: int) -> None:
+        self._groups, self.order = int(S), None
+
     def set_bags(self, bags, validated: bool = False):
         if len(bags) != self.B:
             raise ValueError(f"expected {self.B} bags, got {len(bags)}")
         if isinstance(bags, BagSet) and bags.D == self.D:
-            keep, rows, sizes, self.dt, self.groups = bags, bags.rows, bags.sizes, bags.dt, bags.groups(self.reserved_cus)
+            keep, rows, sizes, self.dt, deal = bags, bags.rows, bags.sizes, bags.dt, bags.deal(self.reserved_cus)
         else:
             keep = list(bags) if validated else checked_bags(bags, self.D, _BATCH_BAGS)
             rows = bag_rows(keep, self.D)
             sizes = tuple(rows[:, 1].tolist())
-            self.dt, self.groups = _dt(keep[0]), choose_groups(sizes, self.reserved_cus)
+            self.dt = _dt(keep[0])
+            deal = choose_deal(sizes, self.reserved_cus, self.dt)
+        self._groups, self.order = deal
         if self._desc_ev is not None:
             self._desc_ev.synchronize()
         self._desc_np[:] = rows
@@ -1737,12 +1784,12 @@
         if own_That is not None:
             own_That.copy_(self.That)
         ad = _p(self.attn.desc) if self.want_attn else None
-        c(lib.vlsa_vlfan_forward_batch_attn(k["desc"], self.B, self.dt, self.D, k["qprep"], self.P, self.pool,
-                                            _p(pool_w), None if self.identity_head else _p(W),
-                                            None if self.identity_head else _p(b), k["That"], self.K, _p(logit_scale),
-                                            k["ws"], k["m2"], k["l"], k["out"], k["pooled"], k["v"], k["vhat"], k["vnorm"],
-                                            k["logits"], k["incidence"], self.reserved_cus, self.groups, ad, ad,
-                                            self.attn.max_n if self.want_attn else 0, s), "vlfan_forward_batch")
+        c(lib.vlsa_vlfan_forward_batch_attn_dealt(k["desc"], self.B, self.dt, self.D, k["qprep"], self.P, self.pool,
+                                                  _p(pool_w), None if self.identity_head else _p(W),
+                                                  None if self.identity_head else _p(b), k["That"], self.K, _p(logit_scale),
+                                                  k["ws"], k["m2"], k["l"], k["out"], k["pooled"], k["v"], k["vhat"], k["vnorm"],
+                                                  k["logits"], k["incidence"], self.reserved_cus, self.groups, self.order, ad, ad,
+                                                  self.attn.max_n if self.want_attn else 0, s), "vlfan_forward_batch")
         return outs["logits"] if outs and "logits" in outs else self.logits
 
     def capture(self, Q, T, logit_scale, W=None, b=None, pool_w=None):
@@ -1758,9 +1805,9 @@
         return g
 
     def run_partial_only(self):
-        nat.check(self.lib.vlsa_vlfan_partial_batch_scores(_p(self.desc), self.B, self.dt, self.D, _p(self.qprep), self.P,
-                                                           _p(self.ws), self.reserved_cus, self.groups,
-                                                           _p(self.attn.desc) if self.want_attn else None, _stream()),
+        nat.check(self.lib.vlsa_vlfan_partial_batch_scores_dealt(_p(self.desc), self.B, self.dt, self.D, _p(self.qprep), self.P,
+                                                                 _p(self.ws), self.reserved_cus, self.groups, self.order,
+                                                                 _p(self.attn.desc) if self.want_attn else None, _stream()),
                   "vlfan_partial_batch")
 
 
@@ -1774,8 +1821,9 @@
         Pk = qp.P
         sc = AttnBuffers(table.sizes, Pk, dev, bag_desc=table.desc)
         ws = torch.empty(lib.vlsa_batch_workspace_bytes(B, Pk, table.D), dtype=torch.uint8, device=dev)
-        nat.check(lib.vlsa_vlfan_partial_batch_scores(_p(table.desc), B, table.dt, table.D, _p(qp.buf), Pk, _p(ws), 0,
-                                                      table.groups(0), _p(sc.desc), s), "vlsa_vlfan_partial_batch_scores")
+        groups, order = table.deal(0)
+        nat.check(lib.vlsa_vlfan_partial_batch_scores_dealt(_p(table.desc), B, table.dt, table.D, _p(qp.buf), Pk, _p(ws), 0,
+                                                            groups, order, _p(sc.desc), s), "vlsa_vlfan_partial_batch_scores")
         part = torch.empty(B, Pk, dtype=torch.float32, device=dev)
         if want_idx:
             idx = torch.empty(B, Pk, kk, dtype=torch.int32, device=dev) if kk else None
```
